# mountain/qingdai

Hardware: AMD Instinct MI355X
Metric: simulated planet-days/sec at 721x1440 f64 (higher is better)
Workload: dtype f64; 1 GPU; 721x1440 seed-42 planet, dt=300 s: forcing + time_step(Teq, dt, albedo) with QD_ENERGY_W=1 QD_CLOUD_COUPLE=1 + slab-ocean coupling + driver-side precipitation/cloud/albedo diagnostics (run_simulation.py:1766-1934,2063-2146) (BASELINE configs[2]; loop order of benchmark_jax.py:124-158); ocean_n_sub=13, parallelism=lat-bands x1

## Files before the change

qingdai_amd/csrc/qd_atmos.hip:

```cpp
#include "qd_internal.h"
#include "qd_pointwise.h"
#include "qd_device.h"
#include "qd_saf.h"

#include "qd_fluxes.h"
#include "qd_fused.h"

struct QdColPtrs {
    const double *u, *v, *Teq, *isr, *albedo, *csmap;
    double *h, *Ts, *q, *cloud, *hice;
    double *E, *Pcond, *LH, *LHrel, *olr, *cloud_eff;
    const uint8_t* land;
    const double* pref;
    unsigned long long* npos;
};

struct QdColIn { double cloud, isr, albedo, teq; };

template <int PHASE, bool HAS_ALB>
__device__ __forceinline__ void qd_column_cell(const QdColP& P, const QdColPtrs& A, size_t o, const QdColIn* IN, int i, int nlat) {
    const double u = A.u[o], v = A.v[o], h = A.h[o], Ts = A.Ts[o];
    const double hice = A.hice[o];
    const bool land = (A.land[o] == 1);
    const bool ocean = !land;
    const double T_a = 288.0 + P.ga * h;
    const double qsat_air = qd_qsat(T_a, P.p0);

    const QdHum Hm = qd_humidity_column(P, u, v, Ts, A.q[o], qsat_air, land, hice);
    const double q = Hm.q, E = Hm.E, Pc = Hm.Pc, LH = Hm.LH, LHrel = Hm.LHrel;
    if (PHASE == 1) { A.Pcond[o] = Pc; return; }
    A.q[o] = q; A.LH[o] = LH;
    if (PHASE != 2) A.Pcond[o] = Pc;
    if (P.write_diag) { A.E[o] = E; A.LHrel[o] = LHrel; }

    const double Teq = IN ? IN->teq : A.Teq[o];
    const double olr_old = P.sigma * qd_pow4(Ts);
    const double net_old = P.sigma * qd_pow4(Teq) + P.gfs * qd_pow4(T_a) - olr_old;
    const double Ts_newton = Ts + (net_old / P.c_sfc_safe) * P.dt;

    double Ts_new, h_new = h;
    QdFlux F;
    if (HAS_ALB) {
        const double cloud = IN ? IN->cloud : A.cloud[o];
        double cloud_eff;
        if (P.couple) {
            const double RH = qd_clip(q / qd_max(1e-12, qsat_air), 0.0, 1.5);
            const double rh_excess = qd_max(0.0, RH - P.rh0);
            const double P_ref = *A.pref;
            const double p_term = qd_tanh(P_ref > 0 ? Pc / P_ref : 0.0);
            cloud_eff = qd_clip(cloud + P.k_q * rh_excess + P.k_p * p_term, 0.0, 1.0);
        } else cloud_eff = cloud;
        A.cloud_eff[o] = cloud_eff;
        F = qd_surface_fluxes(P, IN ? IN->isr : A.isr[o], IN ? IN->albedo : A.albedo[o], cloud_eff, Ts, T_a, u, v, land, hice);
        double Ts_energy;
        if (P.seaice) {
            double Q = F.SW_sfc - F.LW_sfc - F.SH - LH;
            double Tn = Ts, hi = hice;
            if (hi > 0.0 && ocean && Q > 0.0) {
                const double dh_melt = (Q * P.dt) / P.rhoiLf;
                const double dh_cap = qd_min(dh_melt, hi);
                hi -= dh_cap;
                Q = Q - (dh_cap * P.rho_i * P.L_f) / P.dt;
            }
            if (ocean && Q < 0.0 && Tn <= (P.t_freeze + 0.5)) {
                hi += (-Q * P.dt) / P.rhoiLf;
                Q = 0.0;
                Tn = qd_min(Tn, P.t_freeze);
            }
            double Cs = land ? P.Cs_land : (hi > 0.0 ? P.Cs_ice : P.Cs_ocean);
            Cs = (isfinite(Cs) && Cs > 1e3) ? Cs : 1e3;
            Tn = Tn + (Q / Cs) * P.dt;
            if ((i == 0 && P.fix_s) || (i == nlat - 1 && P.fix_n)) {
                if (ocean && Q < 0.0 && Tn > P.t_freeze) Tn = P.t_freeze;
            }
            if (hi > 0.0 && ocean) Tn = qd_min(Tn, P.t_freeze);
            Tn = qd_max(P.t_floor, Tn);
            Ts_energy = qd_nn(Tn);
            { const double hn_ = qd_nn(hi); if (__double_as_longlong(hn_) != __double_as_longlong(hice)) A.hice[o] = hn_; }
        } else {
            const double net = F.SW_sfc - F.LW_sfc - F.SH - LH;
            double Cs;
            if (P.has_csmap) { const double cm = A.csmap[o]; Cs = (isfinite(cm) && cm > 1e3) ? cm : 1e3; }
            else Cs = P.c_sfc_safe;
            Ts_energy = qd_nn(qd_max(P.t_floor, Ts + (net / Cs) * P.dt));
        }
        if (P.write_diag) A.olr[o] = F.OLR;
        Ts_new = (1.0 - P.w_energy) * Ts_newton + P.w_energy * Ts_energy;
    } else {
        if (P.write_diag) A.olr[o] = olr_old;
        Ts_new = Ts_newton;
    }
    A.Ts[o] = Ts_new;

    const double h_eq = P.h_eq_fac * Teq;
    h_new = h + ((h_eq - h) / P.tau_rad) * P.dt;
    if (HAS_ALB && P.atm_couple) {
        const double F_atm = F.SW_atm + F.LW_atm + F.SH + LHrel;
        h_new = qd_nn(h_new + P.atm_w * (F_atm / P.atm_denom) * P.dt);
    }
    A.h[o] = h_new;
}

template <int PHASE, bool HAS_ALB>
__global__ void __launch_bounds__(QD_BLOCK)
k_column(QdGeom G, QdColP P, QdColPtrs A) {
    const QdTile tl = qd_tile();
    const int j = tl.seg * QD_BLOCK + threadIdx.x;
    if (j >= G.nlon) return;
    const int i = G.row0 + tl.row;
    qd_column_cell<PHASE, HAS_ALB>(P, A, (size_t)qd_lrow(G, i) * G.nlon + j, nullptr, i, G.nlat);
}

__global__ void __launch_bounds__(QD_BLOCK)
k_saf_column2(QdSafArgs K, QdColP P, QdColPtrs A) {
    const QdTile tl = qd_tile();
    const int j = tl.seg * QD_BLOCK + threadIdx.x;
    if (j >= K.G.nlon) return;
    const int i = K.G.row0 + tl.row;
    const size_t o = (size_t)qd_lrow(K.G, i) * K.G.nlon + j;
    const QdSafOut s = qd_saf_cell(K, i, j, o, K.write_diag != 0);
    const QdColIn in{s.cloud, s.isr, s.albedo, s.teq};
    qd_column_cell<2, true>(P, A, o, &in, i, K.G.nlat);
}

struct QdMomP { double g, a, dt, dlat, dlon, f_min; int primitive; };

__global__ void __launch_bounds__(QD_BLOCK)
k_momentum(QdGeom G, QdTabs T, QdMomP P, const double* __restrict__ h, const double* __restrict__ fric,
           double* __restrict__ u, double* __restrict__ v) {
    const QdTile tl = qd_tile();
    const int j = tl.seg * QD_BLOCK + threadIdx.x;
    if (j >= G.nlon) return;
    const int i = G.row0 + tl.row;
    const int n = G.nlat, m = G.nlon;
    const size_t b = (size_t)qd_lrow(G, i) * m;
    const size_t o = b + j;
    double dh_dlon;
    if (j == 0) dh_dlon = (h[b + 1] - h[b]) / P.dlon;
    else if (j == m - 1) dh_dlon = (h[b + m - 1] - h[b + m - 2]) / P.dlon;
    else dh_dlon = (h[b + j + 1] - h[b + j - 1]) / (2.0 * P.dlon);
    double dh_dlat;
    if (i == 0) dh_dlat = (h[(size_t)qd_lrow(G, 1) * m + j] - h[o]) / P.dlat;
    else if (i == n - 1) dh_dlat = (h[o] - h[(size_t)qd_lrow(G, n - 2) * m + j]) / P.dlat;
    else dh_dlat = (h[(size_t)qd_lrow(G, i + 1) * m + j] - h[(size_t)qd_lrow(G, i - 1) * m + j]) / (2.0 * P.dlat);
    const double cosc = T.cos6[i];
    const double f = T.fcor[i];
    const double r = fric[o];
    const double u0 = u[o], v0 = v[o];
    if (P.primitive) {
        const double PGF_x = -(P.g / (P.a * cosc)) * dh_dlon;
        const double PGF_y = -(P.g / P.a) * dh_dlat;
        const double du = (PGF_x + f * v0 - r * u0) * P.dt;
        const double dv = (PGF_y - f * u0 - r * v0) * P.dt;
        u[o] = qd_clip(u0 + du, -200.0, 200.0);
        v[o] = qd_clip(v0 + dv, -200.0, 200.0);
    } else {
        const double sgn = (f >= 0.0) ? 1.0 : -1.0;
        const double f_safe = (fabs(f) < P.f_min) ? sgn * P.f_min : f;
        const double u_g = qd_clip(-(P.g / (f_safe * P.a * cosc)) * dh_dlat, -200.0, 200.0);
        const double v_g = qd_clip((P.g / (f_safe * P.a)) * dh_dlon, -200.0, 200.0);
        double un = u0 * 0.8 + u_g * 0.2;
        double vn = v0 * 0.8 + v_g * 0.2;
        un = un + (-r * un) * P.dt;
        vn = vn + (-r * vn) * P.dt;
        u[o] = un; v[o] = vn;
    }
}

__global__ void __launch_bounds__(QD_BLOCK)
k_final(QdGeom G, const double* __restrict__ cosl, double dt, double a, double dlat, double dlon,
        double* __restrict__ u, double* __restrict__ v, double* __restrict__ h, double* __restrict__ Ts,
        double* __restrict__ q, const double* __restrict__ cloud_in, double* __restrict__ cloud_out,
        double decay, double dfac) {
    const QdTile tl = qd_tile();
    const int j = tl.seg * QD_BLOCK + threadIdx.x;
    if (j >= G.nlon) return;
    const int i = G.row0 + tl.row;
    const size_t o = (size_t)qd_lrow(G, i) * G.nlon + j;
    const double uu = u[o], vv = v[o];
    const QdBilin b = qd_departure(G, i, j, uu, vv, dt, a, cosl[i], dlat, dlon);
    double c = qd_gather(cloud_in, G, b);
    c = c * decay;
    cloud_out[o] = qd_nn(c * dfac);
    u[o] = qd_nn(uu * dfac);
    v[o] = qd_nn(vv * dfac);
    h[o] = qd_nn(h[o] * dfac);
    q[o] = qd_nn(q[o] * dfac);
    Ts[o] = qd_nn(Ts[o]);
}

__global__ void __launch_bounds__(QD_BLOCK)
k_forcing(QdGeom G, QdTabs T, QdForcingP P, double* __restrict__ isrA, double* __restrict__ isrB, double* __restrict__ isr,
          const double* __restrict__ albedo, double* __restrict__ Teq, double* __restrict__ eday, double eday_dt) {
    const QdTile tl = qd_tile();
    const int j = tl.seg * QD_BLOCK + threadIdx.x;
    if (j >= G.nlon) return;
    const int i = G.row0 + tl.row;
    const size_t o = (size_t)qd_lrow(G, i) * G.nlon + j;
    qd_forcing_cell(T, P, i, j, o, P.with_teq ? albedo[o] : 0.0, isrA, isrB, isr, Teq, eday, eday_dt);
}

int qd_forcing_impl(qd_ctx* c, const double* sa, const double* sb, double theta, int with_teq) {
    QdScope sc(c, "forcing");
    QdStar A{sa[0], std::sin(sa[1]), std::cos(sa[1]), sa[2]};
    QdStar B{sb[0], std::sin(sb[1]), std::cos(sb[1]), sb[2]};
    const int m = with_teq ? qd_plan(c, {QD_IN(c->f[QD_F_ALBEDO], 0)}) : c->geo.halo;
    if (m < 0) return -1;
    const QdForcingP FP{A, B, theta, 5.670374e-8, with_teq};
    QD_ROWS(c, m, G, hipLaunchKernelGGL(k_forcing, qd_grid2d(G), dim3(QD_BLOCK), 0, c->stream, G, c->tabs, FP,
                                        c->f[QD_F_ISR_A], c->f[QD_F_ISR_B], c->f[QD_F_ISR],
                                        c->f[QD_F_ALBEDO], c->f[QD_F_TEQ], c->eco.eday_dt > 0 ? c->f[QD_F_ECO_EDAY] : (double*)nullptr,
                                        c->eco.eday_dt));
    c->eco.eday_dt = 0;
    qd_mark(c, {c->f[QD_F_ISR_A], c->f[QD_F_ISR_B], c->f[QD_F_ISR]}, m);
    if (with_teq) qd_mark(c, {c->f[QD_F_TEQ]}, m);
    return 0;
}

__global__ void __launch_bounds__(QD_BLOCK)
k_simple_albedo(QdGeom G, const uint8_t* __restrict__ land, const double* __restrict__ base, double ocean_albedo,
                double* __restrict__ albedo) {
    const QdTile tl = qd_tile();
    const int j = tl.seg * QD_BLOCK + threadIdx.x;
    if (j >= G.nlon) return;
    const size_t o = (size_t)qd_lrow(G, G.row0 + tl.row) * G.nlon + j;
    albedo[o] = (land[o] == 0) ? ocean_albedo : base[o];
}

int qd_simple_albedo_impl(qd_ctx* c, double ocean_albedo) {
    const int m = c->geo.full ? 0 : c->geo.halo;
    QD_ROWS(c, m, G, hipLaunchKernelGGL(k_simple_albedo, qd_grid2d(G), dim3(QD_BLOCK), 0, c->stream, G, c->land,
                                        c->f[QD_F_BASE_ALBEDO], ocean_albedo, c->f[QD_F_ALBEDO]));
    qd_mark(c, {c->f[QD_F_ALBEDO]}, m);
    return 0;
}

static inline bool qd_isset(double x) { return !(x != x); }

QdColP qd_make_colp(const qd_ctx* c, double dt) {
    const qd_params& p = c->p;
    QdColP P;
    P.ga = p.g / 1004.0;
    P.M_col = std::max(1e-6, p.rho_a * p.h_mbl);
    P.tau_c = std::max(1e-6, p.tau_cond);
    P.L_v = p.L_v; P.p0 = p.p0; P.rhoCE = p.rho_a * p.C_E;
    P.s_ocean = p.ocean_evap_scale; P.s_land = p.land_evap_scale; P.s_ice = p.ice_evap_scale;
    P.sigma = 5.670374e-8;
    P.gfs = p.greenhouse_factor * P.sigma;
    P.c_sfc_safe = std::max(1e-12, p.c_sfc);
    P.dt = dt;
    P.rh0 = p.rh0; P.k_q = p.k_q; P.k_p = p.k_p;
    P.sw_a0 = p.sw_a0; P.sw_kc = p.sw_kc; P.lw_eps0 = p.lw_eps0; P.lw_kc = p.lw_kc;
    P.eps_clear = std::min(std::max(p.lw_eps0, 0.0), 1.0);
    P.tau0 = p.lw_tau0; P.k_tau = p.lw_ktau;
    P.hice_ref_safe = std::max(1e-6, p.hice_ref);
    P.eps_ocean = p.eps_ocean; P.eps_land = p.eps_land; P.eps_ice = p.eps_ice; P.eps_default = p.eps_default;
    P.g_lw = p.gh_factor_lw;
    P.rhocpch = p.rho_a * p.cp_a * p.ch;
    P.t_freeze = p.t_freeze; P.rho_i = p.rho_i; P.L_f = p.L_f; P.rhoiLf = p.rho_i * p.L_f;
    P.Cs_ocean = p.Cs_ocean; P.Cs_land = p.Cs_land; P.Cs_ice = p.Cs_ice; P.t_floor = p.t_floor;
    P.w_energy = std::min(1.0, std::max(0.0, p.energy_w));
    P.h_eq_fac = 287.0 / p.g;
    P.tau_rad = p.tau_rad;
    const double H_atm = qd_isset(p.atm_h) ? p.atm_h : p.h_mbl;
    P.atm_denom = std::max(1e-6, p.rho_a) * std::max(1.0, H_atm) * p.g;
    P.atm_w = p.energy_w;
    P.atm_couple = (p.energy_w > 0.0) ? 1 : 0;
    P.couple = p.cloud_couple; P.lw_v2 = p.lw_v2; P.gh_lock = p.gh_lock; P.seaice = p.seaice_enabled;
    P.fix_s = p.polar_freeze_fix_s; P.fix_n = p.polar_freeze_fix_n; P.has_csmap = p.has_csmap;
    P.write_diag = c->diag_write;
    return P;
}

__global__ void k_set_scalar(double* p, double v) { if (threadIdx.x == 0 && blockIdx.x == 0) *p = v; }
__global__ void k_zero_count(unsigned long long* p) { if (threadIdx.x == 0 && blockIdx.x == 0) *p = 0ull; }

static QdColPtrs qd_col_ptrs(qd_ctx* c) {
    double** F = c->f;
    QdColPtrs A;
    A.u = F[QD_F_U]; A.v = F[QD_F_V]; A.Teq = F[QD_F_TEQ]; A.isr = F[QD_F_ISR];
    A.albedo = F[QD_F_ALBEDO]; A.csmap = F[QD_F_CSMAP];
    A.h = F[QD_F_H]; A.Ts = F[QD_F_TS]; A.q = F[QD_F_Q]; A.cloud = F[QD_F_CLOUD]; A.hice = F[QD_F_HICE];
    A.E = F[QD_F_EFLUX]; A.Pcond = F[QD_F_PCOND]; A.LH = F[QD_F_LH]; A.LHrel = F[QD_F_LHREL];
    A.olr = F[QD_F_OLR]; A.cloud_eff = F[QD_F_CLOUD_EFF];
    A.land = c->land; A.pref = c->dscal + QD_S_PREF; A.npos = c->dcount;
    return A;
}

int qd_pcond_phase1(qd_ctx* c, double dt) {
    hipLaunchKernelGGL((k_column<1, true>), qd_grid2d(c->geo), dim3(QD_BLOCK), 0, c->stream, c->geo, qd_make_colp(c, dt), qd_col_ptrs(c));
    return 0;
}
int qd_pcond_median_side(qd_ctx* c, double dt) {
    QD_HIP(c, hipEventRecord(c->med_fork, c->stream));
    QD_HIP(c, hipStreamWaitEvent(c->side_stream, c->med_fork, 0));
    std::swap(c->stream, c->side_stream);
    c->med_side_active = true;
    const QdColP P = qd_make_colp(c, dt);
    const QdColPtrs A = qd_col_ptrs(c);
    hipLaunchKernelGGL((k_column<1, true>), qd_grid2d(c->geo), dim3(QD_BLOCK), 0, c->stream, c->geo, P, A);
    const int r = qd_median_positive_dev(c, c->f[QD_F_PCOND], 1e-6, QD_S_PREF, 0, 0.0, 1);
    c->med_side_active = false;
    std::swap(c->stream, c->side_stream);
    if (r) return -1;
    QD_HIP(c, hipEventRecord(c->med_done, c->side_stream));
    c->pcond_ahead = 2;
    return 0;
}

int qd_atmos_step_impl(qd_ctx* c, double dt, int has_albedo) {
    const qd_params& p = c->p;
    const QdGeom& G0 = c->geo;
    const dim3 blk(QD_BLOCK);
    double** F = c->f;
    QdColP P = qd_make_colp(c, dt);
    const int R = qd_adv_reach(c, dt, 250.0);

    if (c->saf_pending && !(has_albedo && p.cloud_couple && !qd_isset(p.pcond_ref) && c->pcond_ahead == 3) && qd_saf_flush(c)) return -1;
    {
        QdScope sc(c, "column");
        int m = has_albedo
            ? qd_plan(c, {QD_IN(F[QD_F_U], 0), QD_IN(F[QD_F_V], 0), QD_IN(F[QD_F_H], 0), QD_IN(F[QD_F_TS], 0), QD_IN(F[QD_F_Q], 0),
                          QD_IN(F[QD_F_CLOUD], 0), QD_IN(F[QD_F_HICE], 0), QD_IN(F[QD_F_TEQ], 0), QD_IN(F[QD_F_ISR], 0),
                          QD_IN(F[QD_F_ALBEDO], 0)})
            : qd_plan(c, {QD_IN(F[QD_F_U], 0), QD_IN(F[QD_F_V], 0), QD_IN(F[QD_F_H], 0), QD_IN(F[QD_F_TS], 0), QD_IN(F[QD_F_Q], 0),
                          QD_IN(F[QD_F_HICE], 0), QD_IN(F[QD_F_TEQ], 0)});
        if (m < 0) return -1;
        QdColPtrs A;
        A.u = F[QD_F_U]; A.v = F[QD_F_V]; A.Teq = F[QD_F_TEQ]; A.isr = F[QD_F_ISR];
        A.albedo = F[QD_F_ALBEDO]; A.csmap = F[QD_F_CSMAP];
        A.h = F[QD_F_H]; A.Ts = F[QD_F_TS]; A.q = F[QD_F_Q]; A.cloud = F[QD_F_CLOUD]; A.hice = F[QD_F_HICE];
        A.E = F[QD_F_EFLUX]; A.Pcond = F[QD_F_PCOND]; A.LH = F[QD_F_LH]; A.LHrel = F[QD_F_LHREL];
        A.olr = F[QD_F_OLR]; A.cloud_eff = F[QD_F_CLOUD_EFF];
        A.land = c->land; A.pref = c->dscal + QD_S_PREF; A.npos = c->dcount;
        if (!has_albedo) {
            QD_ROWS(c, m, G, hipLaunchKernelGGL((k_column<0, false>), qd_grid2d(G), blk, 0, c->stream, G, P, A));
        } else if (!p.cloud_couple || qd_isset(p.pcond_ref)) {
            hipLaunchKernelGGL(k_set_scalar, dim3(1), dim3(1), 0, c->stream, c->dscal + QD_S_PREF,
                               qd_isset(p.pcond_ref) ? p.pcond_ref : 1e-6);
            QD_ROWS(c, m, G, hipLaunchKernelGGL((k_column<0, true>), qd_grid2d(G), blk, 0, c->stream, G, P, A));
        } else {
            const int ahead = c->pcond_ahead;
            c->pcond_ahead = 0;
            if (!ahead) QD_ROWS(c, m, G, hipLaunchKernelGGL((k_column<1, true>), qd_grid2d(G), blk, 0, c->stream, G, P, A));
            if (ahead == 2) QD_HIP(c, hipStreamWaitEvent(c->stream, c->med_done, 0));
            else if (ahead != 3 && qd_median_positive_dev(c, F[QD_F_PCOND], 1e-6, QD_S_PREF, 0, 0.0, 1)) return -1;
            if (c->saf_pending && ahead == 3 && c->geo.full) {
                QdSafArgs* K = (QdSafArgs*)c->saf_pending;
                c->saf_pending = nullptr;
                hipLaunchKernelGGL(k_saf_column2, qd_grid2d(K->G), blk, 0, c->stream, *K, P, A);
                delete K;
            } else {
                if (qd_saf_flush(c)) return -1;
                QD_ROWS(c, m, G, hipLaunchKernelGGL((k_column<2, true>), qd_grid2d(G), blk, 0, c->stream, G, P, A));
            }
        }
        qd_mark(c, {F[QD_F_H], F[QD_F_TS], F[QD_F_Q], F[QD_F_EFLUX], F[QD_F_PCOND], F[QD_F_LH], F[QD_F_LHREL], F[QD_F_OLR]}, m);
        if (has_albedo) { qd_mark(c, {F[QD_F_HICE], F[QD_F_CLOUD_EFF]}, m); c->cloud_eff_valid = 1; }
    }
    c->atm_counter += 1;
    const int64_t sc_ = c->atm_counter;

    {
        QdScope sc(c, "advect_tsq");
        const int m = qd_plan(c, {QD_IN(F[QD_F_TS], R), QD_IN(F[QD_F_Q], R), QD_IN(F[QD_F_U], 0), QD_IN(F[QD_F_V], 0)});
        if (m < 0) return -1;
        double* oT = qd_scratch(c, 0); double* oq = qd_scratch(c, 1);
        qd_launch_advect(c, F[QD_F_U], F[QD_F_V], c->tabs.cos6, dt, F[QD_F_TS], oT, F[QD_F_Q], oq, 0.2, 1, m);
        qd_swap(c, QD_F_TS, 0); qd_swap(c, QD_F_Q, 1);
    }
    const int ft = p.filter_type;
    const bool do_diff = p.diff_enable && (ft == 0 || ft == 1) && (sc_ % std::max(1, p.diff_every) == 0);
    const double f_min = 2.0 * p.omega * std::sin(5.0 * (M_PI / 180.0));
    if (do_diff) { int rc = qd_build_k4_tables(c, dt, false, 0.0); if (rc) return rc; }
    const double ov[5] = {p.k4_u, p.k4_v, p.k4_h, p.k4_q, p.k4_cloud};
    if (do_diff && c->use_fused && p.k4_nsub == 1) {
        const int m = qd_plan(c, {QD_IN(F[QD_F_H], 5), QD_IN(F[QD_F_U], 4), QD_IN(F[QD_F_V], 4), QD_IN(F[QD_F_FRICTION], 4),
                                  QD_IN(F[QD_F_Q], 4), QD_IN(F[QD_F_CLOUD], 4)});
        if (m < 0) return -1;
        QdDynArgs D;
        D.u = F[QD_F_U]; D.v = F[QD_F_V]; D.h = F[QD_F_H]; D.fric = F[QD_F_FRICTION];
        D.q = F[QD_F_Q]; D.cloud = F[QD_F_CLOUD];
        D.uo = qd_scratch(c, 0); D.vo = qd_scratch(c, 1); D.ho = qd_scratch(c, 2); D.qo = qd_scratch(c, 3); D.co = qd_scratch(c, 4);
        for (int f = 0; f < 5; ++f) {
            const bool sc1 = qd_isset(ov[f]);
            D.k4row[f] = sc1 ? nullptr : c->k4_atm + (size_t)f * G0.nlat;
            D.k4s[f] = sc1 ? ov[f] : 0.0;
            D.skip[f] = c->k4_atm_skip[f];
        }
        D.g = p.g; D.a = p.a; D.dt = dt; D.dlat = c->dlat; D.dlon = c->dlon; D.f_min = f_min; D.primitive = p.mom_scheme == 1;
        D.inv_dlon = 1.0 / c->dlon; D.inv_2dlon = 1.0 / (2.0 * c->dlon); D.inv_dlat = 1.0 / c->dlat; D.inv_2dlat = 1.0 / (2.0 * c->dlat);
        D.pgf_y = -(p.g / p.a);
        if (qd_launch_dyn_hyper(c, D, m)) return -1;
        qd_mark(c, {D.uo, D.vo, D.ho, D.qo, D.co}, m);
        qd_swap(c, QD_F_U, 0); qd_swap(c, QD_F_V, 1); qd_swap(c, QD_F_H, 2); qd_swap(c, QD_F_Q, 3); qd_swap(c, QD_F_CLOUD, 4);
    } else {
        {
            QdScope sc(c, "momentum");
            const int m = qd_plan(c, {QD_IN(F[QD_F_H], 1), QD_IN(F[QD_F_U], 0), QD_IN(F[QD_F_V], 0), QD_IN(F[QD_F_FRICTION], 0)});
            if (m < 0) return -1;
            QdMomP M;
            M.g = p.g; M.a = p.a; M.dt = dt; M.dlat = c->dlat; M.dlon = c->dlon; M.f_min = f_min;
            M.primitive = p.mom_scheme == 1;
            QD_ROWS(c, m, G, hipLaunchKernelGGL(k_momentum, qd_grid2d(G), blk, 0, c->stream, G, c->tabs, M, F[QD_F_H],
                                                F[QD_F_FRICTION], F[QD_F_U], F[QD_F_V]));
            qd_mark(c, {F[QD_F_U], F[QD_F_V]}, m);
        }
        if (do_diff) {
            QdScope sc(c, "hyperdiffusion");
            const int ns = std::max(1, p.k4_nsub);
            const int m3 = qd_plan(c, {QD_IN(F[QD_F_U], 4 * ns), QD_IN(F[QD_F_V], 4 * ns), QD_IN(F[QD_F_H], 4 * ns)});
            const int m2 = qd_plan(c, {QD_IN(F[QD_F_Q], 4), QD_IN(F[QD_F_CLOUD], 4)});
            if (m3 < 0 || m2 < 0) return -1;
            double* fl[5] = {F[QD_F_U], F[QD_F_V], F[QD_F_H], F[QD_F_Q], F[QD_F_CLOUD]};
            int skip3[5] = {c->k4_atm_skip[0], c->k4_atm_skip[1], c->k4_atm_skip[2], 1, 1};
            int skip2[5] = {1, 1, 1, c->k4_atm_skip[3], c->k4_atm_skip[4]};
            qd_hyperdiffuse_fields(c, fl, 5, c->k4_atm, skip3, ov, dt, ns, c->tabs.cos02, m3);
            qd_hyperdiffuse_fields(c, fl, 5, c->k4_atm, skip2, ov, dt, 1, c->tabs.cos02, m2);
            F[QD_F_U] = fl[0]; F[QD_F_V] = fl[1]; F[QD_F_H] = fl[2]; F[QD_F_Q] = fl[3]; F[QD_F_CLOUD] = fl[4];
        }
    }
    if ((ft == 0 || ft == 1 || ft == 2) && p.shapiro_every > 0 && (sc_ % p.shapiro_every == 0)) {
        QdScope sc(c, "shapiro");
        const int np_ = std::max(1, p.shapiro_n);
        const int m = qd_plan(c, {QD_IN(F[QD_F_U], np_), QD_IN(F[QD_F_V], np_), QD_IN(F[QD_F_H], np_)});
        if (m < 0) return -1;
        double* fl[3] = {F[QD_F_U], F[QD_F_V], F[QD_F_H]};
        qd_shapiro_fields(c, fl, 3, np_, m);
        F[QD_F_U] = fl[0]; F[QD_F_V] = fl[1]; F[QD_F_H] = fl[2];
        const int n1 = std::max(1, p.shapiro_n - 1);
        if (p.diff_q) {
            const int mq = qd_plan(c, {QD_IN(F[QD_F_Q], n1)}); if (mq < 0) return -1;
            double* g1[1] = {F[QD_F_Q]}; qd_shapiro_fields(c, g1, 1, n1, mq); F[QD_F_Q] = g1[0];
        }
        if (p.diff_cloud) {
            const int mc = qd_plan(c, {QD_IN(F[QD_F_CLOUD], n1)}); if (mc < 0) return -1;
            double* g1[1] = {F[QD_F_CLOUD]}; qd_shapiro_fields(c, g1, 1, n1, mc); F[QD_F_CLOUD] = g1[0];
        }
    }
    if ((ft == 0 || ft == 3) && p.spec_every > 0 && (sc_ % p.spec_every == 0)) {
        QdScope sc(c, "zonal_filter");
        const int m = qd_plan(c, {QD_IN(F[QD_F_U], 0), QD_IN(F[QD_F_V], 0), QD_IN(F[QD_F_H], 0)});
        if (m < 0) return -1;
        double* fl[3] = {F[QD_F_U], F[QD_F_V], F[QD_F_H]};
        if (qd_zonal_filter_fields(c, fl, 3, p.spec_cutoff, p.spec_damp, m)) return -1;
    }
    {
        QdScope sc(c, "final");
        const int m = qd_plan(c, {QD_IN(F[QD_F_CLOUD], R), QD_IN(F[QD_F_U], 0), QD_IN(F[QD_F_V], 0), QD_IN(F[QD_F_H], 0),
                                  QD_IN(F[QD_F_TS], 0), QD_IN(F[QD_F_Q], 0)});
        if (m < 0) return -1;
        const double decay = 1 - dt / (2.0 * 24 * 3600);
        if (c->defer_final && c->geo.full) {
            c->final_pending.on = 1; c->final_pending.dt = dt; c->final_pending.decay = decay; c->final_pending.dfac = p.diff_factor;
            return 0;
        }
        double* oc = qd_scratch(c, 0);
        QD_ROWS(c, m, G, hipLaunchKernelGGL(k_final, qd_grid2d(G), blk, 0, c->stream, G, c->tabs.cos6, dt, p.a, c->dlat, c->dlon,
                                            F[QD_F_U], F[QD_F_V], F[QD_F_H], F[QD_F_TS], F[QD_F_Q], F[QD_F_CLOUD], oc, decay,
                                            p.diff_factor));
        qd_mark(c, {F[QD_F_U], F[QD_F_V], F[QD_F_H], F[QD_F_TS], F[QD_F_Q], oc}, m);
        qd_swap(c, QD_F_CLOUD, 0);
    }
    return 0;
}
```

qingdai_amd/csrc/qd_ocean.hip:

```cpp
#include <cstdlib>
#include <atomic>
#include <chrono>
#include "qd_internal.h"
#include "qd_device.h"
#include "qd_wave.h"

#include "qd_fluxes.h"
#include "qd_fused.h"
#include "qd_ocntail.h"
#include "qd_band.h"
#include "qd_blockred.h"

QdColP qd_make_colp(const qd_ctx* c, double dt);

__global__ void __launch_bounds__(QD_BLOCK)
k_qnet(QdGeom G, QdColP P, const double* __restrict__ isr, const double* __restrict__ albedo,
       const double* __restrict__ cloud, const double* __restrict__ Ts, const double* __restrict__ h,
       const double* __restrict__ u, const double* __restrict__ v, const uint8_t* __restrict__ land,
       const double* __restrict__ hice, const double* __restrict__ LH, double* __restrict__ qnet,
       uint8_t* __restrict__ icemask) {
    const QdTile tl = qd_tile();
    const int j = tl.seg * QD_BLOCK + threadIdx.x;
    if (j >= G.nlon) return;
    const size_t o = (size_t)qd_lrow(G, G.row0 + tl.row) * G.nlon + j;
// ... 225 lines not shown
    const double du = (f * v0 - P.g * gx + taux[o] / P.rhoH - P.r_bot * u0);
    const double dv = (-f * u0 - P.g * gy + tauy[o] / P.rhoH - P.r_bot * v0);
    double un = u0 + P.sub_dt * du;
    double vn = v0 + P.sub_dt * dv;
    if (land[o] == 1) { un = 0.0; vn = 0.0; }
    const double rx = T.r_extra[i];
    un = un - P.sub_dt * rx * un;
    vn = vn - P.sub_dt * rx * vn;
    uo[o] = un; vo[o] = vn;
}

__global__ void __launch_bounds__(QD_BLOCK)
k_continuity(QdGeom G, QdTabs T, double a, double dlat, double dlon, double msdtH, const double* __restrict__ uo,
             const double* __restrict__ vo, const uint8_t* __restrict__ land, double* __restrict__ eta,
             double* __restrict__ partial) {
    __shared__ double sm[QD_BLOCK / 64];
    const int i = G.row0 + blockIdx.y;
    const size_t b = (size_t)qd_lrow(G, i) * G.nlon;
    const double w = T.warea[i];
    double acc = 0.0;
    for (int j = threadIdx.x; j < G.nlon; j += QD_BLOCK) {
        const size_t o = b + j;
        const double div = qd_divvort_point(G, T, uo, vo, i, j, a, dlat, dlon, 0);
        double e = eta[o] + msdtH * div;
        const bool island = land[o] == 1;
        if (island) e = 0.0;
        eta[o] = e;
        acc += e * (island ? 0.0 : w);
    }
    acc = qd_wave_sum(acc);
    const int lane = threadIdx.x & 63, wv = threadIdx.x >> 6;
    if (lane == 0) sm[wv] = acc;
    __syncthreads();
    if (threadIdx.x == 0) {
        double r = sm[0];
        for (int k = 1; k < QD_BLOCK / 64; ++k) r += sm[k];
        partial[blockIdx.y] = r;
    }
}

__global__ void __launch_bounds__(QD_BLOCK)
k_eta_mean(const double* __restrict__ partial, int n, double wsum, double* __restrict__ out, double seq = 0.0) {
    __shared__ double sm[QD_BLOCK / 64];
    double acc = 0.0;
    for (int k = threadIdx.x; k < n; k += QD_BLOCK) acc += partial[k];
    acc = qd_wave_sum(acc);
    const int lane = threadIdx.x & 63, wv = threadIdx.x >> 6;
    if (lane == 0) sm[wv] = acc;
    __syncthreads();
    if (threadIdx.x == 0) {
        double r = sm[0];
        for (int k = 1; k < QD_BLOCK / 64; ++k) r += sm[k];
        *out = (wsum < 0.0) ? r : r / (wsum + 1e-15);
        if (seq != 0.0) __hip_atomic_store(&out[1], seq, __ATOMIC_RELEASE, __HIP_MEMORY_SCOPE_SYSTEM);
    }
}

__global__ void __launch_bounds__(QD_BLOCK)
k_cont_sstadv(QdGeom G, QdTabs T, double a, double dlat, double dlon, double msdtH, double sub_dt, double alpha,
              const double* __restrict__ uo, const double* __restrict__ vo, const uint8_t* __restrict__ land,
              double* __restrict__ eta, const double* __restrict__ Ts, double* __restrict__ Ts_out,
              int own0, int own1, double* __restrict__ partial, unsigned long long* ticket, double wsum,
              double* __restrict__ eta_mean) {
    __shared__ double sm[QD_BLOCK / 64];
    __shared__ int s_last;
    const int i = G.row0 + blockIdx.y;
    const size_t b = (size_t)qd_lrow(G, i) * G.nlon;
    const double w = (i >= own0 && i < own1) ? T.warea[i] : 0.0;
    const double cosl = T.cos05[i];
    const int pidx = blockIdx.y * gridDim.x + blockIdx.x, pcount = gridDim.x * gridDim.y;
    double acc = 0.0;
    for (int j = blockIdx.x * QD_BLOCK + threadIdx.x; j < G.nlon; j += gridDim.x * QD_BLOCK) {
        const size_t o = b + j;
        const double div = qd_divvort_point(G, T, uo, vo, i, j, a, dlat, dlon, 0);
        double e = eta[o] + msdtH * div;
        const bool island = land[o] == 1;
        if (island) e = 0.0;
        eta[o] = e;
        acc += e * (island ? 0.0 : w);
        const QdBilin bl = qd_departure(G, i, j, uo[o], vo[o], sub_dt, a, cosl, dlat, dlon);
        Ts_out[o] = (1.0 - alpha) * Ts[o] + alpha * qd_gather(Ts, G, bl);
    }
    acc = qd_wave_sum(acc);
    const int lane = threadIdx.x & 63, wv = threadIdx.x >> 6;
    if (lane == 0) sm[wv] = acc;
    __syncthreads();
    if (threadIdx.x == 0) {
        double r = sm[0];
        for (int k = 1; k < QD_BLOCK / 64; ++k) r += sm[k];
        if (!ticket) partial[pidx] = r;
        else {
            __hip_atomic_store(&partial[pidx], r, __ATOMIC_RELAXED, __HIP_MEMORY_SCOPE_AGENT);
            asm volatile("s_waitcnt vmcnt(0)" ::: "memory");
            const unsigned long long t = atomicAdd(ticket, 1ull);
            s_last = (t == (unsigned long long)pcount - 1ull) ? 1 : 0;
        }
    }
    if (!ticket) return;
    __syncthreads();
    if (!s_last) return;
    double a2 = 0.0;
    for (int k = threadIdx.x; k < pcount; k += QD_BLOCK)
        a2 += __hip_atomic_load(&partial[k], __ATOMIC_RELAXED, __HIP_MEMORY_SCOPE_AGENT);
    a2 = qd_wave_sum(a2);
    __syncthreads();
    if (lane == 0) sm[wv] = a2;
    __syncthreads();
    if (threadIdx.x == 0) {
        double r = sm[0];
        for (int k = 1; k < QD_BLOCK / 64; ++k) r += sm[k];
        *eta_mean = r / (wsum + 1e-15);
        __hip_atomic_store(ticket, 0ull, __ATOMIC_RELAXED, __HIP_MEMORY_SCOPE_AGENT);
    }
}

__global__ void __launch_bounds__(QD_BLOCK)
k_sst_advect(QdGeom G, const double* __restrict__ cos05, double sub_dt, double a, double dlat, double dlon,
             const double* __restrict__ uo, const double* __restrict__ vo, const double* __restrict__ Ts,
             double* __restrict__ Ts_out, double alpha, double* __restrict__ eta, const double* __restrict__ eta_mean,
             int has_ocean) {
    const QdTile tl = qd_tile();
    const int j = tl.seg * QD_BLOCK + threadIdx.x;
    if (j >= G.nlon) return;
    const int i = G.row0 + tl.row;
    const size_t o = (size_t)qd_lrow(G, i) * G.nlon + j;
    if (has_ocean) eta[o] = eta[o] - *eta_mean;
    const QdBilin b = qd_departure(G, i, j, uo[o], vo[o], sub_dt, a, cos05[i], dlat, dlon);
    const double adv = qd_gather(Ts, G, b);
    Ts_out[o] = (1.0 - alpha) * Ts[o] + alpha * adv;
}

struct QdHeatP { double sub_dt, K_h, rcH, ice_qfac; int use_q, has_ice; };

__global__ void __launch_bounds__(QD_BLOCK)
k_sst_diffuse_heat(QdGeom G, const double* __restrict__ cos05, double dlat, double dlon, double a, QdHeatP P,
                   const double* __restrict__ Ts1, double* __restrict__ Ts_out, const double* __restrict__ qnet,
                   const uint8_t* __restrict__ land, const uint8_t* __restrict__ ice) {
    const QdTile tl = qd_tile();
    const int j = tl.seg * QD_BLOCK + threadIdx.x;
    if (j >= G.nlon) return;
    const int i = G.row0 + tl.row;
    const size_t o = (size_t)qd_lrow(G, i) * G.nlon + j;
    double T = Ts1[o];
    if (P.K_h > 0.0) T = qd_nn(T) + P.sub_dt * P.K_h * qd_lap_point<true>(Ts1, G, cos05, i, j, dlat, dlon, a);
    if (P.use_q) {
        const double heat = qnet[o] / P.rcH;
        const bool ocean = land[o] == 0;
        if (P.has_ice) {
            const bool ic = ice[o] != 0;
            if (ocean && !ic) T = T + P.sub_dt * heat;
            if (P.ice_qfac > 0.0 && ocean && ic) T = T + P.sub_dt * P.ice_qfac * heat;
        } else if (ocean) T = T + P.sub_dt * heat;
    }
    Ts_out[o] = qd_nn(T);
}

__global__ void __launch_bounds__(QD_BLOCK)
k_outlier(QdGeom G, const double* __restrict__ uo, const double* __restrict__ vo, double* __restrict__ uo_out,
          double* __restrict__ vo_out, double* __restrict__ eta, double cap, double eta_cap, int mean4) {
    const QdTile tl = qd_tile();
    const int j = tl.seg * QD_BLOCK + threadIdx.x;
    if (j >= G.nlon) return;
    const int i = G.row0 + tl.row;
    const size_t b = (size_t)qd_lrow(G, i) * G.nlon;
    const size_t o = b + j;
    double u = qd_nn(uo[o]), v = qd_nn(vo[o]);
    const double speed = sqrt(u * u + v * v);
    if (mean4) {
        if (speed > cap) {
            const size_t bn = (size_t)qd_lrow(G, i + 1) * G.nlon, bs = (size_t)qd_lrow(G, i - 1) * G.nlon;
            const int je = qd_wrapc(j + 1, G.nlon), jw = qd_wrapc(j - 1, G.nlon);
            u = 0.25 * (qd_nn(uo[bn + j]) + qd_nn(uo[bs + j]) + qd_nn(uo[b + je]) + qd_nn(uo[b + jw]));
            v = 0.25 * (qd_nn(vo[bn + j]) + qd_nn(vo[bs + j]) + qd_nn(vo[b + je]) + qd_nn(vo[b + jw]));
        }
        const double sp2 = sqrt(u * u + v * v);
        const double sc2 = (sp2 > cap) ? cap / (sp2 + 1e-12) : 1.0;
        u = u * sc2; v = v * sc2;
    } else {
        const double sc = (speed > cap) ? cap / (speed + 1e-12) : 1.0;
        u = u * sc; v = v * sc;
    }
    uo_out[o] = u; vo_out[o] = v;
    eta[o] = qd_clip(qd_nn(eta[o]), -eta_cap, eta_cap);
}

__global__ void __launch_bounds__(QD_BLOCK)
k_sst_outlier_fused(QdGeom G, QdTabs T, double dlat, double dlon, double a, QdHeatP P,
                    const double* __restrict__ Ts1, double* __restrict__ Ts_out, const double* __restrict__ qnet,
                    const uint8_t* __restrict__ land, const uint8_t* __restrict__ ice,
                    const double* __restrict__ uo, const double* __restrict__ vo, double* __restrict__ uo_out,
                    double* __restrict__ vo_out, double* __restrict__ eta, double cap, double eta_cap, int mean4,
                    const double* __restrict__ eta_mean, const double* __restrict__ partial, int pcount, double wsum,
                    double* __restrict__ mean_out) {
    if (mean_out && blockIdx.x == 0 && blockIdx.y == 0) {
        __shared__ double smm[QD_BLOCK / 64];
        double acc = 0.0;
        for (int k = threadIdx.x; k < pcount; k += QD_BLOCK) acc += partial[k];
        acc = qd_wave_sum(acc);
        if ((threadIdx.x & 63) == 0) smm[threadIdx.x >> 6] = acc;
        __syncthreads();
        if (threadIdx.x == 0) {
            double r = smm[0];
            for (int k = 1; k < QD_BLOCK / 64; ++k) r += smm[k];
            *mean_out = r / (wsum + 1e-15);
        }
    }
    const QdTile tl = qd_tile();
    const int j = tl.seg * QD_BLOCK + threadIdx.x;
    if (j >= G.nlon) return;
    const int i = G.row0 + tl.row;
    const size_t b = (size_t)qd_lrow(G, i) * G.nlon;
    const size_t o = b + j;
    double Tv = Ts1[o];
    if (P.K_h > 0.0) Tv = qd_nn(Tv) + P.sub_dt * P.K_h * qd_lap_point_fast<true>(Ts1, G, T, 1, i, j, dlat, dlon, a);
    if (P.use_q) {
        const double heat = qnet[o] / P.rcH;
        const bool ocean = land[o] == 0;
        if (P.has_ice) {
            const bool ic = ice[o] != 0;
            if (ocean && !ic) Tv = Tv + P.sub_dt * heat;
            if (P.ice_qfac > 0.0 && ocean && ic) Tv = Tv + P.sub_dt * P.ice_qfac * heat;
        } else if (ocean) Tv = Tv + P.sub_dt * heat;
    }
    Ts_out[o] = qd_nn(Tv);
    double u = qd_nn(uo[o]), v = qd_nn(vo[o]);
    const double speed = sqrt(u * u + v * v);
    if (mean4) {
        if (speed > cap) {
            const size_t bn = (size_t)qd_lrow(G, i + 1) * G.nlon, bs = (size_t)qd_lrow(G, i - 1) * G.nlon;
            const int je = qd_wrapc(j + 1, G.nlon), jw = qd_wrapc(j - 1, G.nlon);
            u = 0.25 * (qd_nn(uo[bn + j]) + qd_nn(uo[bs + j]) + qd_nn(uo[b + je]) + qd_nn(uo[b + jw]));
            v = 0.25 * (qd_nn(vo[bn + j]) + qd_nn(vo[bs + j]) + qd_nn(vo[b + je]) + qd_nn(vo[b + jw]));
        }
        const double sp2 = sqrt(u * u + v * v);
        const double sc2 = (sp2 > cap) ? cap / (sp2 + 1e-12) : 1.0;
        u = u * sc2; v = v * sc2;
    } else {
        const double sc = (speed > cap) ? cap / (speed + 1e-12) : 1.0;
        u = u * sc; v = v * sc;
    }
    uo_out[o] = u; vo_out[o] = v;
    if (mean_out) return;
    const double e = eta_mean ? eta[o] - (pcount < 0 ? *eta_mean / (wsum + 1e-15) : *eta_mean) : eta[o];
    eta[o] = qd_clip(qd_nn(e), -eta_cap, eta_cap);
}


__device__ __forceinline__ double qd_block_sum_ocn(double x, double* sm) {
    x = qd_wave_sum(x);
    const int lane = threadIdx.x & 63, wv = threadIdx.x >> 6;
    __syncthreads();
    if (lane == 0) sm[wv] = x;
    __syncthreads();
    double r = sm[0];
    for (int k = 1; k < QD_BLOCK / 64; ++k) r += sm[k];
    return r;
}

__device__ __forceinline__ void qd_polar_fill_row(const QdGeom& G, const QdTabs& T, const uint8_t* __restrict__ land, double* __restrict__ Ts,
                                                  double* __restrict__ uo, double* __restrict__ vo, bool north, double* sm) {
    const int i = north ? G.nlat - 1 : 0;
    const size_t b = (size_t)qd_lrow(G, i) * G.nlon;
    double cnt = 0, sT = 0, s0 = 0, s1 = 0;
    for (int j = threadIdx.x; j < G.nlon; j += QD_BLOCK) {
        if (land[b + j] != 0) continue;
        cnt += 1.0;
        sT += Ts[b + j];
        const double sl = T.sin_lon[j], cl = T.cos_lon[j];
        const double u = uo[b + j], v = vo[b + j];
        const double nx = north ? -cl : cl, ny = north ? -sl : sl;
        s0 += (-sl) * u + nx * v;
        s1 += cl * u + ny * v;
    }
    cnt = qd_block_sum_ocn(cnt, sm);
    sT = qd_block_sum_ocn(sT, sm);
    s0 = qd_block_sum_ocn(s0, sm);
    s1 = qd_block_sum_ocn(s1, sm);
    if (cnt <= 0.0) return;
    const double mT = sT / cnt, m0 = s0 / cnt, m1 = s1 / cnt;
    for (int j = threadIdx.x; j < G.nlon; j += QD_BLOCK) {
        if (land[b + j] != 0) continue;
        const double sl = T.sin_lon[j], cl = T.cos_lon[j];
        const double nx = north ? -cl : cl, ny = north ? -sl : sl;
        Ts[b + j] = mT;
        uo[b + j] = (-sl) * m0 + cl * m1;
        vo[b + j] = nx * m0 + ny * m1;
    }
}

__global__ void __launch_bounds__(QD_BLOCK)
k_polar_fill(QdGeom G, QdTabs T, const uint8_t* __restrict__ land, double* __restrict__ Ts, double* __restrict__ uo,
             double* __restrict__ vo) {
    __shared__ double sm[QD_BLOCK / 64];
    const bool north = blockIdx.x == 1;
    const int i = north ? G.nlat - 1 : 0;
    if (i < G.row0 || i >= G.row0 + G.nrows) return;
    qd_polar_fill_row(G, T, land, Ts, uo, vo, north, sm);
}

__device__ __forceinline__ void qd_sst_clamp_cell(size_t o, double* __restrict__ sst, double tmin, double tmax, int inject,
                                                  const uint8_t* __restrict__ land, const uint8_t* __restrict__ ice, int has_ice,
                                                  double* __restrict__ Ts_atm, double* __restrict__ eta, const double* __restrict__ eta_mean,
                                                  double eta_cap) {
    if (eta) eta[o] = qd_clip(qd_nn(eta[o] - *eta_mean), -eta_cap, eta_cap);
    const double t0 = sst[o];
    const double t = qd_clip(t0, tmin, tmax);
    if (__double_as_longlong(t) != __double_as_longlong(t0)) sst[o] = t;
    if (inject && land[o] == 0 && !(has_ice && ice[o] != 0)) Ts_atm[o] = t;
}

__global__ void __launch_bounds__(QD_BLOCK)
k_sst_clamp_inject(QdGeom G, double* __restrict__ sst, double tmin, double tmax, int inject,
                   const uint8_t* __restrict__ land, const uint8_t* __restrict__ ice, int has_ice,
                   double* __restrict__ Ts_atm, double* __restrict__ eta, const double* __restrict__ eta_mean, double eta_cap) {
    const QdTile tl = qd_tile();
    const int j = tl.seg * QD_BLOCK + threadIdx.x;
    if (j >= G.nlon) return;
    const size_t o = (size_t)qd_lrow(G, G.row0 + tl.row) * G.nlon + j;
    qd_sst_clamp_cell(o, sst, tmin, tmax, inject, land, ice, has_ice, Ts_atm, eta, eta_mean, eta_cap);
}

#define QD_PF_CH 6
__global__ void __launch_bounds__(QD_BLOCK)
k_polar_clamp_inject(QdGeom G, QdTabs T, double* __restrict__ sst, double* __restrict__ uo, double* __restrict__ vo, double tmin, double tmax,
                     int inject, const uint8_t* __restrict__ land, const uint8_t* __restrict__ ice, int has_ice,
                     double* __restrict__ Ts_atm, double* __restrict__ eta, const double* __restrict__ eta_mean, double eta_cap) {
    __shared__ double sm[4][QD_BLOCK / 64];
    const QdTile tl = qd_tile();
    const int i = G.row0 + tl.row;
    if (i == 0 || i == G.nlat - 1) {
        if (tl.seg != 0) return;
        const bool north = i != 0;
        const size_t b = (size_t)qd_lrow(G, i) * G.nlon;
        if (G.nlon > QD_PF_CH * QD_BLOCK) {
            qd_polar_fill_row(G, T, land, sst, uo, vo, north, &sm[0][0]);
            __syncthreads();
            for (int j = threadIdx.x; j < G.nlon; j += QD_BLOCK)
                qd_sst_clamp_cell(b + j, sst, tmin, tmax, inject, land, ice, has_ice, Ts_atm, eta, eta_mean, eta_cap);
            return;
        }
        double t_[QD_PF_CH], u_[QD_PF_CH], v_[QD_PF_CH], sl_[QD_PF_CH], cl_[QD_PF_CH]; int ld_[QD_PF_CH];
#pragma unroll
        for (int k = 0; k < QD_PF_CH; ++k) {
            const int j = threadIdx.x + k * QD_BLOCK;
            const int jj = j < G.nlon ? j : G.nlon - 1;
            ld_[k] = j < G.nlon ? (int)land[b + jj] : 1;
            t_[k] = sst[b + jj]; u_[k] = uo[b + jj]; v_[k] = vo[b + jj]; sl_[k] = T.sin_lon[jj]; cl_[k] = T.cos_lon[jj];
        }
        double cnt = 0, sT = 0, s0 = 0, s1 = 0;
#pragma unroll
        for (int k = 0; k < QD_PF_CH; ++k) {
            if (ld_[k] != 0) continue;
            cnt += 1.0;
            sT += t_[k];
            const double nx = north ? -cl_[k] : cl_[k], ny = north ? -sl_[k] : sl_[k];
            s0 += (-sl_[k]) * u_[k] + nx * v_[k];
            s1 += cl_[k] * u_[k] + ny * v_[k];
        }
        cnt = qd_wave_sum(cnt); sT = qd_wave_sum(sT); s0 = qd_wave_sum(s0); s1 = qd_wave_sum(s1);
        const int lane = threadIdx.x & 63, wv = threadIdx.x >> 6;
        if (lane == 0) { sm[0][wv] = cnt; sm[1][wv] = sT; sm[2][wv] = s0; sm[3][wv] = s1; }
        __syncthreads();
        cnt = sm[0][0]; sT = sm[1][0]; s0 = sm[2][0]; s1 = sm[3][0];
        for (int k = 1; k < QD_BLOCK / 64; ++k) { cnt += sm[0][k]; sT += sm[1][k]; s0 += sm[2][k]; s1 += sm[3][k]; }
        const bool any = cnt > 0.0;
        const double mT = sT / cnt, m0 = s0 / cnt, m1 = s1 / cnt;
#pragma unroll
        for (int k = 0; k < QD_PF_CH; ++k) {
            const int j = threadIdx.x + k * QD_BLOCK;
            if (j >= G.nlon) continue;
            const size_t o = b + j;
            double tv = t_[k];
            if (any && ld_[k] == 0) {
                const double nx = north ? -cl_[k] : cl_[k], ny = north ? -sl_[k] : sl_[k];
                tv = mT;
                uo[o] = (-sl_[k]) * m0 + cl_[k] * m1;
                vo[o] = nx * m0 + ny * m1;
            }
            if (eta) eta[o] = qd_clip(qd_nn(eta[o] - *eta_mean), -eta_cap, eta_cap);
            const double t = qd_clip(tv, tmin, tmax);
            sst[o] = t;
            if (inject && ld_[k] == 0 && !(has_ice && ice[o] != 0)) Ts_atm[o] = t;
        }
        return;
    }
    const int j = tl.seg * QD_BLOCK + threadIdx.x;
    if (j >= G.nlon) return;
    qd_sst_clamp_cell((size_t)qd_lrow(G, i) * G.nlon + j, sst, tmin, tmax, inject, land, ice, has_ice, Ts_atm, eta, eta_mean, eta_cap);
}

__global__ void __launch_bounds__(256) k_eta_mean_tail(const double* __restrict__ partial, int n, double wsum, double* __restrict__ out) {
    __shared__ double sm[4];
    double a = 0.0;
    for (int k = threadIdx.x; k < n; k += 256) a += partial[k];
#pragma unroll
    for (int o = 32; o > 0; o >>= 1) a += __shfl_down(a, o, 64);
    if ((threadIdx.x & 63) == 0) sm[threadIdx.x >> 6] = a;
    __syncthreads();
    if (threadIdx.x == 0) *out = (((sm[0] + sm[1]) + sm[2]) + sm[3]) / (wsum + 1e-15);
}

__global__ void k_eta_mean_post(double* s, double wsum) { if (threadIdx.x == 0 && blockIdx.x == 0) *s = *s / (wsum + 1e-15); }

__global__ void k_host_flag(double* flag, double seq) {
    if (threadIdx.x == 0 && blockIdx.x == 0) __hip_atomic_store(flag, seq, __ATOMIC_RELEASE, __HIP_MEMORY_SCOPE_SYSTEM);
}
int qd_ocean_step_impl(qd_ctx* c, double dt, int compute_qnet, int use_ice_mask, int inject_sst) {
    const qd_params& p = c->p;
    const QdGeom& G0 = c->geo;
    const dim3 blk(QD_BLOCK);
    double** F = c->f;
    const bool band = !G0.full;
    c->ocn_counter += 1;
    const int64_t step = c->ocn_counter;
    const double H = p.H_ocean;
    const QdGeom Gown = qd_segments(c, 0).g[0];
    const dim3 rows(1, Gown.nrows);

    auto launch_qnet = [&]() -> int {
        QdScope sc(c, "ocean_qnet");
        QdColP P = qd_make_colp_driver(c, dt);
        double*& cl = c->cloud_eff_valid ? F[QD_F_CLOUD_EFF] : F[QD_F_CLOUD];
        const int m = qd_plan(c, {QD_IN(F[QD_F_ISR], 0), QD_IN(F[QD_F_ALBEDO], 0), QD_IN(cl, 0), QD_IN(F[QD_F_TS], 0),
                                  QD_IN(F[QD_F_H], 0), QD_IN(F[QD_F_U], 0), QD_IN(F[QD_F_V], 0), QD_IN(F[QD_F_HICE], 0),
                                  QD_IN(F[QD_F_LH], 0)});
        if (m < 0) return -1;
        QD_ROWS(c, m, G, hipLaunchKernelGGL(k_qnet, qd_grid2d(G), blk, 0, c->stream, G, P, F[QD_F_ISR], F[QD_F_ALBEDO], cl,
                                            F[QD_F_TS], F[QD_F_H], F[QD_F_U], F[QD_F_V], c->land, F[QD_F_HICE], F[QD_F_LH],
                                            F[QD_F_QNET], c->icemask));
        qd_mark(c, {F[QD_F_QNET], c->icemask}, m);
        use_ice_mask = 1;
        return 0;
    };
    if (compute_qnet && band && launch_qnet()) return -1;
    double*& taux = c->scratch[14];
    double*& tauy = c->scratch[15];
    int n_sub;
    bool band_fix_stats = false;
    {
        QdScope sc(c, "ocean_stress");
        const int m = qd_plan(c, {QD_IN(F[QD_F_U], 0), QD_IN(F[QD_F_V], 0), QD_IN(F[QD_F_UO], 0), QD_IN(F[QD_F_VO], 0)});
        if (m < 0) return -1;
        QdSegs S = qd_segments(c, m);
        double maxVa = 0.0, maxUo = 0.0;
        if (!band) {
            const QdGeom& G = S.g[0];
            c->eta_seq += 1.0;
            bool merged_final = false;
            if (c->final_pending.on) {
                if (!compute_qnet) return qd_fail(c, "ocean step: a deferred k_final needs compute_qnet");
                c->final_pending.on = 0;
                QdFqsArgs A;
                A.cosl = c->tabs.cos6; A.dt = c->final_pending.dt; A.a = p.a; A.dlat = c->dlat; A.dlon = c->dlon;
                A.decay = c->final_pending.decay; A.dfac = c->final_pending.dfac;
                A.u = F[QD_F_U]; A.v = F[QD_F_V]; A.h = F[QD_F_H]; A.Ts = F[QD_F_TS]; A.q = F[QD_F_Q];
                A.cloud_in = F[QD_F_CLOUD]; A.cloud_out = qd_scratch(c, 0);
                A.isr = F[QD_F_ISR]; A.albedo = F[QD_F_ALBEDO]; A.cloud_eff = c->cloud_eff_valid ? F[QD_F_CLOUD_EFF] : nullptr;
                A.hice = F[QD_F_HICE]; A.LH = F[QD_F_LH]; A.land = c->land; A.qnet = F[QD_F_QNET]; A.icemask = c->icemask;
                A.uo = F[QD_F_UO]; A.vo = F[QD_F_VO]; A.vcap = p.vcap; A.rhoCD = p.rho_a_ocean * p.CD; A.tau_scale = p.tau_scale;
                A.taux = taux; A.tauy = tauy;
                A.dev_wg = c->wgmax; A.n_wg = c->n_wgmax;
                merged_final = true;
                hipLaunchKernelGGL(k_final_qnet_stress, qd_grid2d(G), blk, 0, c->stream, G, qd_make_colp_driver(c, dt), A);
                hipLaunchKernelGGL(k_max2_publish, dim3(1), dim3(1024), 0, c->stream, c->wgmax, c->n_wgmax, c->hpin + 58, c->fix_count);
                qd_swap(c, QD_F_CLOUD, 0);
                use_ice_mask = 1;
            } else {
            hipLaunchKernelGGL(k_stress_max, dim3(1, G.nrows), blk, 0, c->stream, G, F[QD_F_U], F[QD_F_V], F[QD_F_UO],
                               F[QD_F_VO], p.vcap, p.rho_a_ocean * p.CD, p.tau_scale, taux, tauy, c->hpin_rows,
                               c->hpin_rows + (size_t)2 * G0.lrows(), c->eta_seq);
            qd_mark(c, {taux, tauy}, m);
            if (compute_qnet && launch_qnet()) return -1;
            }
            if (c->before_cfl_wait) {
                std::function<int()> fn = std::move(c->before_cfl_wait);
                c->before_cfl_wait = nullptr;
                if (c->side_stream_on && c->timing != 1 && !c->ocn_fused) {
                    QD_HIP(c, hipEventRecord(c->side_fork, c->stream));
                    QD_HIP(c, hipStreamWaitEvent(c->side_stream, c->side_fork, 0));
                    std::swap(c->stream, c->side_stream);
                    const int r = fn();
                    std::swap(c->stream, c->side_stream);
                    if (r) return -1;
                    QD_HIP(c, hipEventRecord(c->side_done, c->side_stream));
                    c->side_pending = true;
                } else if (fn()) return -1;
            }
            if (merged_final) {
                if (qd_wait_host_nonneg(c, c->hpin + 58, &maxVa, "ocean step: the CFL maxima never arrived") ||
                    qd_wait_host_nonneg(c, c->hpin + 59, &maxUo, "ocean step: the CFL maxima never arrived")) return -1;
                { const double avg = c->hpin[57]; c->hpin[57] = -1.0; if (avg >= 0.0) c->fix_avg = avg; }
            } else {
            for (int k = 0; k < G.nrows; ++k)
                if (qd_wait_host_flag(c, c->hpin_rows + (size_t)2 * G0.lrows() + k, c->eta_seq, "ocean step: the CFL maxima never arrived")) return -1;
            for (int k = 0; k < G.nrows; ++k) { maxVa = std::max(maxVa, c->hpin_rows[k]); maxUo = std::max(maxUo, c->hpin_rows[G.nrows + k]); }
            }
        } else {
        const bool hooked = qd_peer_hooks(c) && !qd_has_host_ring(c) && S.n <= 3;
        for (int k = 0; k < S.n; ++k) {
            const QdGeom& G = S.g[k];
            hipLaunchKernelGGL(k_stress_max, dim3(1, G.nrows), blk, 0, c->stream, G, F[QD_F_U], F[QD_F_V], F[QD_F_UO],
                               F[QD_F_VO], p.vcap, p.rho_a_ocean * p.CD, p.tau_scale, taux, tauy,
                               c->red_partial + (size_t)k * 2 * G0.lrows(), (double*)nullptr, 0.0);
            if (!hooked)
            hipLaunchKernelGGL(k_max2_finish, dim3(1), blk, 0, c->stream, c->red_partial + (size_t)k * 2 * G0.lrows(), G.nrows,
                               c->dscal + QD_S_TMP0 + 2 * k, k == S.n - 1 ? 2 * (3 - S.n) : 0);
        }
        qd_mark(c, {taux, tauy}, m);
        if (hooked) {
            QdPeerHook H; H.pre = 3; H.partial = c->red_partial; H.pstride = (size_t)2 * G0.lrows(); H.nseg = S.n;
            for (int k = 0; k < S.n; ++k) H.nsegrows[k] = S.g[k].nrows;
            c->allreduces++;
            c->pub_seq += 1.0;
            H.fixstat = (c->tail_fix && c->fix_count) ? c->fix_count : nullptr;
            if (qd_peer_allreduce_hooked(c, c->dscal + QD_S_TMP0, H.fixstat ? 7 : 6, 1, H, c->hpin, c->pub_seq)) return -1;
            if (qd_wait_host_flag(c, c->hpin + 61, c->pub_seq, "reduced scalars never reached the host")) return -1;
            if (c->hpin[60] != 0.0) return qd_fail(c, "peer exchange: a rank did not arrive within the deadline");
            if (H.fixstat && c->hpin[6] >= 0.0) c->fix_avg = c->hpin[6];
            band_fix_stats = H.fixstat != nullptr;
        } else if (qd_has_host_ring(c)) {
            QD_HIP(c, hipMemcpyAsync(c->hpin, c->dscal + QD_S_TMP0, 6 * sizeof(double), hipMemcpyDeviceToHost, c->stream));
            QD_HIP(c, hipStreamSynchronize(c->stream));
            if (qd_host_allreduce(c, c->hpin, 6, 1)) return -1;
        } else {
        if (qd_allreduce_fetch(c, c->dscal + QD_S_TMP0, 6, 1, c->hpin)) return -1;
        }
        for (int k = 0; k < 3; ++k) { maxVa = std::max(maxVa, c->hpin[2 * k]); maxUo = std::max(maxUo, c->hpin[2 * k + 1]); }
        }
        const double dx_lat = p.a * c->dlat;
        const double min_cos = 0.5;
        const double dx_lon_min = p.a * c->dlon * std::max(1e-3, min_cos);
        const double dx_min = std::min(dx_lat, dx_lon_min);
        const double cg = std::sqrt(p.g_ocean * H);
        double uadv = std::max(maxUo, maxVa);
        const double target = std::max(1e-3, p.ocean_cfl);
        const double v = std::ceil(std::max(cg, uadv) * (dt / std::max(1e-12, dx_min)) / target);
        n_sub = (v != v) ? 1 : (v > 500.0 ? 500 : (v < 1.0 ? 1 : (int)v));
        c->last_nsub = n_sub;
        c->form_note(QD_SF_LAST_NSUB, n_sub); c->form_note(QD_SF_LAST_TAIL_KERNEL, 0); c->form_note(QD_SF_LAST_OCN_FORM, 0);
    }
    bool fix_now = c->tail_fix && c->fix_count && (!band || band_fix_stats);
    if (fix_now) {
        if (c->fix_avg <= c->fix_dense) c->fix_probe_every = 32;
        else if (step >= c->fix_probe_at) {
            c->fix_probe_at = step + c->fix_probe_every;
            c->fix_probe_every = std::min(256, c->fix_probe_every * 2);
        } else fix_now = false;
    }
    const double sub_dt = dt / n_sub;
    QdOcnP OP{p.a, p.g_ocean, c->dlat, c->dlon, sub_dt, p.rho_w * H, p.r_bot};
    QdHeatP HP{sub_dt, p.K_h, p.rho_w * p.cp_w * H, p.ocean_ice_qfac, p.ocean_use_qnet ? 1 : 0, use_ice_mask ? 1 : 0};
    const bool do_diff = (p.ocean_diff_every > 0) && (step % p.ocean_diff_every == 0);
    const bool do_shap = (p.ocean_shapiro_n > 0) && (p.ocean_shapiro_every > 0) && (step % p.ocean_shapiro_every == 0);
    if (do_diff) { int rc = qd_build_k4_tables(c, dt, true, sub_dt); if (rc) return rc; }
    const double ov[3] = {p.ocean_k4_u, p.ocean_k4_v, p.ocean_k4_eta};
    const int Ro = qd_adv_reach(c, sub_dt, 4.0);

    const bool can_defer = do_diff && c->use_fused && p.ocean_k4_nsub == 1 && !do_shap && c->wsum_ocean > 0.0;
    const bool band_defer = band && can_defer && qd_has_host_ring(c);
    const bool band_tail = band && can_defer && !band_defer && c->ocn_tail == 1 && c->tail_acc && c->band_tail && G0.nlon >= 64 &&
                           G0.halo >= std::max(7, Ro + 2);
    const bool defer_eta = (!band && can_defer) || band_defer || band_tail;
    double* const mean_ptr = band_defer ? c->hpin + 42 : c->dscal + QD_S_ETA_MEAN;
    struct CoRefresh { qd_ctx* c; ~CoRefresh() { c->corefresh.clear(); } } corefresh_guard{c};
    if (band) c->corefresh = {QD_IN(F[QD_F_UO], 0), QD_IN(F[QD_F_VO], 0), QD_IN(F[QD_F_ETA], 0), QD_IN(F[QD_F_SST], 0), QD_IN(taux, 0),
                              QD_IN(tauy, 0), QD_IN(F[QD_F_QNET], 0), QD_IN8(c->icemask, 0)};
    const bool use_tail = c->use_fused && (!band || band_tail) && defer_eta && qd_ocn_tail_ok(G0) && c->ocn_tail;
    const bool tail_acc = use_tail && c->tail_acc;
    const bool use_fused1 = use_tail && !band && c->ocn_fused && c->ocn_tail == 1 && tail_acc && c->fused_fast == 1 && do_diff &&
                            p.ocean_k4_nsub == 1 && !do_shap && HP.use_q && HP.K_h > 0.0 && qd_ocn_fused_ok(c) &&
                            !c->k4_ocn_skip[0] && !c->k4_ocn_skip[1] && !c->k4_ocn_skip[2];
    const bool mean_form_ok = c->mean_in_momentum && !band && G0.full && tail_acc && !use_fused1 && do_diff && c->use_fused && n_sub > 1 &&
                              p.ocean_k4_nsub == 1 && !do_shap && qd_ocn_tail_is_fast(c) && qd_ocn_stream_ok(c, 0);
    if (mean_form_ok) fix_now = false;
    const bool mean_next_ok = mean_form_ok;
    c->form_note(QD_SF_LAST_USE_TAIL, use_tail); c->form_note(QD_SF_LAST_TAIL_ACC, tail_acc); c->form_note(QD_SF_LAST_USE_FUSED1, use_fused1);
    c->form_note(QD_SF_LAST_MEAN_FORM, mean_form_ok); c->form_note(QD_SF_LAST_FIX_NOW, fix_now);
    unsigned long long* acc_pending = nullptr;
    for (int s = 0; s < n_sub; ++s) {
        if (use_fused1) {
            QdOcnArgs O;
            O.uo = F[QD_F_UO]; O.vo = F[QD_F_VO]; O.eta = F[QD_F_ETA]; O.taux = taux; O.tauy = tauy; O.land = c->land;
            O.uo_out = qd_scratch(c, 0); O.vo_out = qd_scratch(c, 1); O.eta_out = qd_scratch(c, 6);
            for (int f = 0; f < 3; ++f) {
                const bool sc1 = !(ov[f] != ov[f]);
                O.k4row[f] = sc1 ? nullptr : c->k4_ocn + (size_t)f * G0.nlat;
                O.k4s[f] = sc1 ? ov[f] : 0.0;
                O.skip[f] = c->k4_ocn_skip[f];
            }
            O.a = p.a; O.g = p.g_ocean; O.dlat = c->dlat; O.dlon = c->dlon; O.sub_dt = sub_dt; O.rhoH = p.rho_w * H; O.r_bot = p.r_bot;
            O.inv_2dlon = 1.0 / (2.0 * c->dlon); O.inv_2dlat = 1.0 / (2.0 * c->dlat); O.inv_a = 1.0 / p.a; O.inv_rhoH = 1.0 / (p.rho_w * H);
            O.eta_mean = s > 0 ? mean_ptr : nullptr;
            O.eta_cap = p.eta_cap;
            QdTailArgs A;
            A.uo = O.uo_out; A.vo = O.vo_out; A.eta_in = O.eta_out; A.Ts = F[QD_F_SST]; A.qnet = F[QD_F_QNET]; A.land = c->land; A.ice = c->icemask;
            A.eta = qd_scratch(c, 2); A.Ts_out = qd_scratch(c, 3); A.uo_out = qd_scratch(c, 12); A.vo_out = qd_scratch(c, 13); A.partial = c->red_partial;
            A.a = p.a; A.dlat = c->dlat; A.dlon = c->dlon; A.sub_dt = sub_dt; A.msdtH = -sub_dt * H; A.alpha = p.ocean_adv_alpha;
            A.K_h = HP.K_h; A.rcH = HP.rcH; A.ice_qfac = HP.ice_qfac; A.cap = p.ocean_max_u;
            A.use_q = HP.use_q; A.has_ice = HP.has_ice; A.mean4 = p.ocean_outlier == 0 ? 1 : 0;
            A.r_a = 1.0 / p.a; A.r_dlon = 1.0 / c->dlon; A.r_dlat = 1.0 / c->dlat; A.r_2dlon = 1.0 / (2 * c->dlon); A.r_2dlat = 1.0 / (2 * c->dlat);
            A.r_rcH = 1.0 / HP.rcH;
            A.acc = c->eta_acc; A.mean_out = c->dscal + QD_S_ETA_MEAN; A.wsum = c->wsum_ocean;
            if (qd_launch_ocn_fused(c, O, A)) return -1;
            qd_swap(c, QD_F_UO, 12); qd_swap(c, QD_F_VO, 13); qd_swap(c, QD_F_ETA, 2); qd_swap(c, QD_F_SST, 3);
            continue;
        }
        if (do_diff && c->use_fused && p.ocean_k4_nsub == 1) {
            const QdUse narrow[5] = {QD_IN(F[QD_F_ETA], 5), QD_IN(F[QD_F_UO], 4), QD_IN(F[QD_F_VO], 4), QD_IN(taux, 4), QD_IN(tauy, 4)};
            bool pending = false;
            int m_old = 0;
            if (band_tail) {
                const QdUse wide[8] = {QD_IN(F[QD_F_ETA], 7), QD_IN(F[QD_F_UO], 6), QD_IN(F[QD_F_VO], 6), QD_IN(taux, 6), QD_IN(tauy, 6),
                                       QD_IN(F[QD_F_SST], Ro + 2), QD_IN(F[QD_F_QNET], 0), QD_IN8(c->icemask, 0)};
                if (qd_plan_begin(c, wide, 8, &pending) < 0) return -1;
                if (pending) m_old = qd_plan_peek(c, narrow, 5);
            }
            QdOcnArgs O;
            O.uo = F[QD_F_UO]; O.vo = F[QD_F_VO]; O.eta = F[QD_F_ETA]; O.taux = taux; O.tauy = tauy; O.land = c->land;
            O.uo_out = qd_scratch(c, 0); O.vo_out = qd_scratch(c, 1); O.eta_out = qd_scratch(c, 2);
            for (int f = 0; f < 3; ++f) {
                const bool sc1 = !(ov[f] != ov[f]);
                O.k4row[f] = sc1 ? nullptr : c->k4_ocn + (size_t)f * G0.nlat;
                O.k4s[f] = sc1 ? ov[f] : 0.0;
                O.skip[f] = c->k4_ocn_skip[f];
            }
            O.a = p.a; O.g = p.g_ocean; O.dlat = c->dlat; O.dlon = c->dlon; O.sub_dt = sub_dt; O.rhoH = p.rho_w * H; O.r_bot = p.r_bot;
            O.inv_2dlon = 1.0 / (2.0 * c->dlon); O.inv_2dlat = 1.0 / (2.0 * c->dlat); O.inv_a = 1.0 / p.a; O.inv_rhoH = 1.0 / (p.rho_w * H);
            O.eta_mean = (defer_eta && s > 0) ? mean_ptr : nullptr;
            O.eta_cap = p.eta_cap;
            if (acc_pending) { O.acc_read = acc_pending; O.acc_partial = c->red_partial; O.acc_n = qd_ocn_tail_tiles(c, Gown); O.acc_wsum = c->wsum_ocean; }
            int m_int = 0;
            bool split = false;
            if (pending) {
                m_int = m_old >= 0 ? m_old : -12;
                const QdSegList Si = qd_segments_rows(c, c->own_row0 - m_int, c->own_nrows + 2 * m_int);
                if (c->own_nrows + 2 * m_int >= 12 && qd_ocn_stream_ok_list(c, Si)) {
                    if (qd_launch_ocn_stream_list(c, O, Si)) return -1;
                    split = true;
                    c->form_count(QD_SF_CNT_SPLIT);
                }
                if (qd_plan_end(c)) return -1;
            }
            const int m = qd_plan(c, narrow, 5);
            if (m < 0) return -1;
            if (qd_allreduce_flush(c)) return -1;
            if (split && m > m_int) {
                QdSegList Sb = qd_segments_rows(c, c->own_row0 - m, m - m_int);
                Sb = qd_segments_rows(c, c->own_row0 + c->own_nrows + m_int, m - m_int, Sb);
                if (!qd_ocn_stream_ok_list(c, Sb)) {
                    c->form_count(QD_SF_CNT_SPLIT_REDO);
                    if (qd_launch_ocn_hyper(c, O, m)) return -1;
                } else if (qd_launch_ocn_stream_list(c, O, Sb)) return -1;
            } else if (!split) {
                if (qd_launch_ocn_hyper(c, O, m)) return -1;
            }
            qd_mark(c, {O.uo_out, O.vo_out, O.eta_out}, m);
            qd_swap(c, QD_F_UO, 0); qd_swap(c, QD_F_VO, 1); qd_swap(c, QD_F_ETA, 2);
        } else {
            {
                QdScope sc(c, "ocean_momentum");
                const int m = qd_plan(c, {QD_IN(F[QD_F_ETA], 1), QD_IN(F[QD_F_UO], 0), QD_IN(F[QD_F_VO], 0), QD_IN(taux, 0),
                                          QD_IN(tauy, 0)});
                if (m < 0) return -1;
                QD_ROWS(c, m, G, hipLaunchKernelGGL(k_ocean_momentum, qd_grid2d(G), blk, 0, c->stream, G, c->tabs, OP,
                                                    F[QD_F_ETA], taux, tauy, c->land, F[QD_F_UO], F[QD_F_VO]));
                qd_mark(c, {F[QD_F_UO], F[QD_F_VO]}, m);
            }
            if (do_diff) {
                QdScope sc(c, "ocean_hyperdiffusion");
                const int ns = std::max(1, p.ocean_k4_nsub);
                const int m = qd_plan(c, {QD_IN(F[QD_F_UO], 4 * ns), QD_IN(F[QD_F_VO], 4 * ns), QD_IN(F[QD_F_ETA], 4 * ns)});
                if (m < 0) return -1;
                double* fl[3] = {F[QD_F_UO], F[QD_F_VO], F[QD_F_ETA]};
                c->lap_tag = "ocean_k_laplacian"; c->hyp_tag = "ocean_k_hyper_apply";
                qd_hyperdiffuse_fields(c, fl, 3, c->k4_ocn, c->k4_ocn_skip, ov, sub_dt, ns, c->tabs.cos05, m);
                c->lap_tag = "k_laplacian"; c->hyp_tag = "k_hyper_apply";
                F[QD_F_UO] = fl[0]; F[QD_F_VO] = fl[1]; F[QD_F_ETA] = fl[2];
            }
        }
        if (do_shap) {
            const int np_ = p.ocean_shapiro_n;
            const int m = qd_plan(c, {QD_IN(F[QD_F_UO], np_), QD_IN(F[QD_F_VO], np_), QD_IN(F[QD_F_ETA], np_)});
            if (m < 0) return -1;
            double* fl[3] = {F[QD_F_UO], F[QD_F_VO], F[QD_F_ETA]};
            qd_shapiro_fields(c, fl, 3, np_, m);
// ... 201 lines not shown
```

qingdai_amd/csrc/qd_physics.hip:

```cpp
#include "qd_internal.h"
#include "qd_band.h"
#include "qd_pointwise.h"
#include "qd_device.h"
#include "qd_saf.h"
#include "qd_fluxes.h"
#include "qd_blockred.h"
QdColP qd_make_colp(const qd_ctx* c, double dt);


template <bool SLAB>
__global__ void __launch_bounds__(QD_BLOCK)
k_precip_raw(QdGeom G, QdTabs T, const double* __restrict__ u, const double* __restrict__ v,
             const double* __restrict__ pcond, double a, double dlat, double dlon, double D_crit, double beta,
             const double* __restrict__ scale_p, const unsigned long long* __restrict__ sel_state,
             double* __restrict__ praw, double* __restrict__ pos_out, double* __restrict__ partial,
             const double* __restrict__ orog) {
    __shared__ double sm[2][QD_BLOCK / 64];
    const int i = G.row0 + blockIdx.y;
    const size_t b = (size_t)qd_lrow(G, i) * G.nlon;
    const double w = T.warea[i];
    const bool anypos = sel_state[0] > 0;
    const double scale = qd_max(*scale_p, 1e-12);
    double s_num = 0.0, s_den = 0.0;
    for (int j = threadIdx.x; j < G.nlon; j += QD_BLOCK) {
        const double div = SLAB ? u[b + j] : qd_divvort_point(G, T, u, v, i, j, a, dlat, dlon, 0);
        const double pos = qd_max(0.0, -(div - D_crit));
        const double F_div = anypos ? qd_clip(pos / scale, 0.0, 5.0) : 0.0;
        const double Pq = qd_max(0.0, pcond[b + j]);
        const double F_orog = orog ? qd_clip(orog[b + j], 1.0, 3.0) : 1.0;
        const double F = (1.0 + beta * F_div) * F_orog;
        const double pr = Pq * F;
        praw[b + j] = pr;
        if (!SLAB) pos_out[b + j] = pos;
        s_num += Pq * w;
        s_den += pr * w;
    }
    s_num = qd_wave_sum(s_num); s_den = qd_wave_sum(s_den);
    const int lane = threadIdx.x & 63, wv = threadIdx.x >> 6;
    if (lane == 0) { sm[0][wv] = s_num; sm[1][wv] = s_den; }
    __syncthreads();
    if (threadIdx.x == 0) {
        for (int k = 1; k < QD_BLOCK / 64; ++k) { s_num += sm[0][k]; s_den += sm[1][k]; }
        partial[blockIdx.y] = s_num;
        partial[gridDim.y + blockIdx.y] = s_den;
    }
}

__global__ void __launch_bounds__(QD_BLOCK)
k_orog_factor(QdGeom G, QdTabs T, const double* __restrict__ elev, const double* __restrict__ u, const double* __restrict__ v,
              double a, double dlat, double dlon, double k_orog, double cap, double* __restrict__ out) {
    const QdTile tl = qd_tile();
    const int j = tl.seg * QD_BLOCK + threadIdx.x;
    if (j >= G.nlon) return;
    const int i = G.row0 + tl.row, n = G.nlat;
    const size_t b = (size_t)qd_lrow(G, i) * G.nlon;
    const int jp = qd_wrapc(j + 1, G.nlon), jm = qd_wrapc(j - 1, G.nlon);
    const double dx = a * T.cos6[i] * dlon, dy = a * dlat;
    const double dHdx = (elev[b + jp] - elev[b + jm]) / (2.0 * dx);
    double dHdy = 0.0;
    if (i != 0 && i != n - 1)
        dHdy = (elev[(size_t)qd_lrow(G, i + 1) * G.nlon + j] - elev[(size_t)qd_lrow(G, i - 1) * G.nlon + j]) / (2.0 * dy);
    const double gn = sqrt(dHdx * dHdx + dHdy * dHdy);
    const double nxh = gn > 1e-12 ? dHdx / (gn + 1e-12) : 0.0;
    const double nyh = gn > 1e-12 ? dHdy / (gn + 1e-12) : 0.0;
    out[b + j] = qd_clip(1.0 + k_orog * qd_max(0.0, u[b + j] * nxh + v[b + j] * nyh), 1.0, cap);
}

__global__ void __launch_bounds__(QD_BLOCK)
k_precip_scalars(const double* __restrict__ partial, int n, double wsum, double pq_min, double p_blend, int use_fb,
                 double* __restrict__ out) {
    qd_precip_scalars_wg(partial, n, wsum, pq_min, p_blend, use_fb, out);
}

__global__ void __launch_bounds__(QD_BLOCK)
k_scale_field(QdGeom G, const double* __restrict__ in, const double* __restrict__ s, double k, double* __restrict__ out) {
    const QdTile tl = qd_tile();
    const int j = tl.seg * QD_BLOCK + threadIdx.x;
    if (j >= G.nlon) return;
    const size_t o = (size_t)qd_lrow(G, G.row0 + tl.row) * G.nlon + j;
    out[o] = s ? in[o] * (*s) : k * in[o];
}

__global__ void __launch_bounds__(QD_BLOCK)
k_precip_blend(QdGeom G, const double* __restrict__ P, const double* __restrict__ Pdyn, const double* __restrict__ sc,
               double* __restrict__ out) {
    const QdTile tl = qd_tile();
    const int j = tl.seg * QD_BLOCK + threadIdx.x;
    if (j >= G.nlon) return;
    const size_t o = (size_t)qd_lrow(G, G.row0 + tl.row) * G.nlon + j;
    const double al = sc[1];
    double p = P[o];
    if (al != 0.0) p = (1.0 - al) * p + al * Pdyn[o];
    out[o] = qd_max(p, 0.0);
}

__global__ void __launch_bounds__(QD_BLOCK)
k_cloud_from_p(QdGeom G, const double* __restrict__ precip, const double* __restrict__ pref, double cmax,
               double* __restrict__ out) {
    const QdTile tl = qd_tile();
    const int j = tl.seg * QD_BLOCK + threadIdx.x;
    if (j >= G.nlon) return;
    const size_t o = (size_t)qd_lrow(G, G.row0 + tl.row) * G.nlon + j;
    out[o] = cmax * qd_tanh(precip[o] / (*pref + 1e-12));
}


__device__ __forceinline__ double qd_tanh01(double x) {
    double t = 0.0;
    if (!(x <= 0.0)) t = qd_tanh_nonneg(x);
    return qd_clip(t, 0.0, 1.0);
}

__device__ __forceinline__ double qd_cloud_source_cell(const QdGeom& G, const QdTabs& T, const double* __restrict__ u, const double* __restrict__ v,
                                                       const double* __restrict__ Ts, double a, double dlat, double dlon, int i, int j);

__global__ void __launch_bounds__(QD_BLOCK)
k_cloud_source(QdGeom G, QdTabs T, const double* __restrict__ u, const double* __restrict__ v,
               const double* __restrict__ Ts, double a, double dlat, double dlon, double* __restrict__ out) {
    const QdTile tl = qd_tile();
    const int j = tl.seg * QD_BLOCK + threadIdx.x;
    if (j >= G.nlon) return;
    const int i = G.row0 + tl.row;
    out[(size_t)qd_lrow(G, i) * G.nlon + j] = qd_cloud_source_cell(G, T, u, v, Ts, a, dlat, dlon, i, j);
}

__global__ void __launch_bounds__(QD_BLOCK)
k_cloud_fromp_source(QdGeom G, QdTabs T, const double* __restrict__ precip, const double* __restrict__ pref, double cmax,
                     const double* __restrict__ u, const double* __restrict__ v, const double* __restrict__ Ts, double a, double dlat,
                     double dlon, double* __restrict__ cfp, double* __restrict__ src) {
    const QdTile tl = qd_tile();
    const int j = tl.seg * QD_BLOCK + threadIdx.x;
    if (j >= G.nlon) return;
    const int i = G.row0 + tl.row;
    const size_t o = (size_t)qd_lrow(G, i) * G.nlon + j;
    cfp[o] = cmax * qd_tanh(precip[o] / (*pref + 1e-12));
    src[o] = qd_cloud_source_cell(G, T, u, v, Ts, a, dlat, dlon, i, j);
}

__device__ __forceinline__ double qd_cloud_source_cell(const QdGeom& G, const QdTabs& T, const double* __restrict__ u, const double* __restrict__ v,
                                                       const double* __restrict__ Ts, double a, double dlat, double dlon, int i, int j) {
    const size_t b = (size_t)qd_lrow(G, i) * G.nlon;
    const size_t o = b + j;
    const double T0 = Ts[o];
    double src = 0.0;
    src = src + 0.5 * qd_tanh01((T0 - 285.0) / 12.0);
    const double vort = qd_divvort_point(G, T, v, u, i, j, a, dlat, dlon, 1);
    const double rel = vort / (T.fcor[i] + 1e-12);
    src = src + 0.4 * qd_tanh01((rel - 0.5) / 2.0);
    const double dx = dlon * a * T.cos6[i];
    const double dy = dlat * a;
    const int jp = qd_wrapc(j + 1, G.nlon), jm = qd_wrapc(j - 1, G.nlon);
    const double gx = (Ts[b + jp] - Ts[b + jm]) / (2 * dx);
    const double gy = (Ts[(size_t)qd_lrow(G, i + 1) * G.nlon + j] - Ts[(size_t)qd_lrow(G, i - 1) * G.nlon + j]) / (2 * dy);
    const double tadv = -(u[o] * gx + v[o] * gy);
    src = src + 0.3 * qd_tanh01(fabs(tadv) / 2e-5);
    return src;
}

struct QdBlendP { double w_mem, w_p, w_src, tend, c_floor; };

__global__ void __launch_bounds__(QD_BLOCK)
k_cloud_blend(QdGeom G, QdBlendP P, const double* __restrict__ cfp, const double* __restrict__ src,
              double* __restrict__ cloud) {
    const QdTile tl = qd_tile();
    const int j = tl.seg * QD_BLOCK + threadIdx.x;
    if (j >= G.nlon) return;
    const size_t o = (size_t)qd_lrow(G, G.row0 + tl.row) * G.nlon + j;
    const double c0 = cloud[o], cp = cfp[o];
    const double tendency = src[o] * P.tend;
    double c = (P.w_mem * c0 + P.w_p * cp + P.w_src * qd_clip(c0 + tendency, 0.0, 1.0));
    if (P.c_floor > 0.0) c = qd_max(c, qd_clip(P.c_floor * cp, 0.0, 1.0));
    cloud[o] = qd_clip(c, 0.0, 1.0);
}

__global__ void __launch_bounds__(QD_BLOCK)
k_cloud_albedo(QdGeom G, QdAlbP P, const double* __restrict__ adv, double* __restrict__ cloud,
               const double* __restrict__ cloud_eff, const double* __restrict__ hice,
               const double* __restrict__ base, const uint8_t* __restrict__ land, const double* __restrict__ csnow,
               const double* __restrict__ eco_alpha, const double* __restrict__ glacier, const double* __restrict__ banded,
               const double* __restrict__ water, double* __restrict__ albedo) {
    const QdTile tl = qd_tile();
    const int j = tl.seg * QD_BLOCK + threadIdx.x;
    if (j >= G.nlon) return;
    const size_t o = (size_t)qd_lrow(G, G.row0 + tl.row) * G.nlon + j;
    double c = cloud[o];
    if (P.do_adv) { c = qd_clip((1.0 - P.alpha) * c + P.alpha * adv[o], 0.0, 1.0); cloud[o] = c; }
    const int landv = land[o];
    const double cs = (P.snow && landv == 1) ? csnow[o] : 0.0;
    const double gl = (P.eco && landv == 1) ? glacier[o] : 0.0;
    albedo[o] = qd_albedo_cell(P, o, c, cloud_eff, hice, base, landv, cs, gl, eco_alpha, banded, water);
}

__global__ void k_precip_scalars_post(const double* raw, double wsum, double pq_min, double p_blend, int use_fb, double* out) {
    if (threadIdx.x == 0 && blockIdx.x == 0) {
        const double a = raw[0], b = raw[1];
        const double den = b + 1e-20;
        out[0] = den > 0 ? a / den : 1.0;
        const double pq_mean = a / (wsum + 1e-15);
        out[1] = (use_fb && pq_mean < pq_min) ? p_blend : 0.0;
    }
}
__global__ void __launch_bounds__(QD_BLOCK)
k_precip_rawsums(const double* __restrict__ partial, int n, double* __restrict__ out) {
    __shared__ double sm[2][QD_BLOCK / 64];
    double a = 0.0, b = 0.0;
    for (int k = threadIdx.x; k < n; k += QD_BLOCK) { a += partial[k]; b += partial[n + k]; }
    a = qd_wave_sum(a); b = qd_wave_sum(b);
    const int lane = threadIdx.x & 63, wv = threadIdx.x >> 6;
    if (lane == 0) { sm[0][wv] = a; sm[1][wv] = b; }
    __syncthreads();
    if (threadIdx.x == 0) {
        for (int k = 1; k < QD_BLOCK / 64; ++k) { a += sm[0][k]; b += sm[1][k]; }
        out[0] = a; out[1] = b;
    }
}

__global__ void __launch_bounds__(QD_BLOCK)
k_snow_provisional(QdGeom G, QdTabs T, QdSnowP P, const double* __restrict__ precip, const double* __restrict__ h,
                   const double* __restrict__ S_snow, const double* __restrict__ elev, const uint8_t* __restrict__ land,
                   double* __restrict__ P_rain, double* __restrict__ S_next, double* __restrict__ melt,
                   double* __restrict__ C_snow, double* __restrict__ glacier) {
    const QdTile tl = qd_tile();
    const int j = tl.seg * QD_BLOCK + threadIdx.x;
    if (j >= G.nlon) return;
    const int i = G.row0 + tl.row;
    const size_t o = (size_t)qd_lrow(G, i) * G.nlon + j;
    const QdSnowOut r = qd_snow_cell(T, P, i, land[o] == 1, h[o], S_snow[o], elev[o], precip[o]);
    P_rain[o] = r.Pr; S_next[o] = r.Sn; melt[o] = r.melt; C_snow[o] = r.Cs; glacier[o] = r.gl;
}

__global__ void __launch_bounds__(QD_BLOCK)
k_snow_albedo_forcing(QdSafArgs K) {
    const QdTile tl = qd_tile();
    const int j = tl.seg * QD_BLOCK + threadIdx.x;
    if (j >= K.G.nlon) return;
    const int i = K.G.row0 + tl.row;
    qd_saf_cell(K, i, j, (size_t)qd_lrow(K.G, i) * K.G.nlon + j, true);
}
int qd_saf_launch(qd_ctx* c, const QdSafArgs& K) {
    hipLaunchKernelGGL(k_snow_albedo_forcing, qd_grid2d(K.G), dim3(QD_BLOCK), 0, c->stream, K);
    return 0;
}
void qd_saf_drop(qd_ctx* c) { delete (QdSafArgs*)c->saf_pending; c->saf_pending = nullptr; }
int qd_saf_flush(qd_ctx* c) {
    if (!c->saf_pending) return 0;
    QdSafArgs* K = (QdSafArgs*)c->saf_pending;
    c->saf_pending = nullptr;
    const int r = qd_saf_launch(c, *K);
    delete K;
    return r;
}

struct QdBucketP { double dt, tau_s, cap; };

__global__ void __launch_bounds__(QD_BLOCK)
k_hydro_commit(QdGeom G, QdBucketP P, const double* __restrict__ P_rain, const double* __restrict__ melt,
               const double* __restrict__ glacier, const double* __restrict__ E, const uint8_t* __restrict__ land,
               const double* __restrict__ S_next, double* __restrict__ S_snow, double* __restrict__ W_land,
               double* __restrict__ runoff) {
    const QdTile tl = qd_tile();
    const int j = tl.seg * QD_BLOCK + threadIdx.x;
    if (j >= G.nlon) return;
    const size_t o = (size_t)qd_lrow(G, G.row0 + tl.row) * G.nlon + j;
    const double L = land[o] == 1 ? 1.0 : 0.0;
    const double gl = glacier[o];
    const double non_gl = (L != 0.0 && gl == 0.0) ? 1.0 : 0.0;
    const double ml = melt[o];
    const double P_in = (P_rain[o] * L + ml) * non_gl;
    const double E_l = (E[o] * L) * non_gl;
    const double W = W_land[o];
    const double R_base = W / P.tau_s;
    double Wn = qd_max(0.0, W + (P_in - E_l - R_base) * P.dt);
    double R_fast = 0.0;
    if (P.cap > 0.0) {
        const double over = qd_max(0.0, Wn - P.cap);
        Wn = Wn - over;
        R_fast = (P.dt > 0) ? over / P.dt : 0.0;
    }
    W_land[o] = qd_nn(Wn);
    runoff[o] = qd_nn(R_base + R_fast) + ml * gl;
    S_snow[o] = S_next[o];
}

int qd_hydrology_commit_impl(qd_ctx* c, double dt) {
    const qd_params& p = c->p;
    double** F = c->f;
    QdScope sc(c, "hydrology");
    const int m = qd_plan(c, {QD_IN(F[QD_F_P_RAIN], 0), QD_IN(F[QD_F_MELT], 0), QD_IN(F[QD_F_GLACIER], 0), QD_IN(F[QD_F_EFLUX], 0),
                              QD_IN(F[QD_F_S_SNOW_NEXT], 0), QD_IN(F[QD_F_W_LAND], 0)});
    if (m < 0) return -1;
    QdBucketP B{dt, std::max(1.0, p.runoff_tau_days * 86400.0), (p.wland_cap_mm == p.wland_cap_mm && p.wland_cap_mm > 0) ? p.wland_cap_mm : -1.0};
    QD_ROWS(c, m, G, hipLaunchKernelGGL(k_hydro_commit, qd_grid2d(G), dim3(QD_BLOCK), 0, c->stream, G, B, F[QD_F_P_RAIN], F[QD_F_MELT],
                                        F[QD_F_GLACIER], F[QD_F_EFLUX], c->land, F[QD_F_S_SNOW_NEXT], F[QD_F_S_SNOW], F[QD_F_W_LAND],
                                        F[QD_F_RUNOFF]));
    qd_mark(c, {F[QD_F_S_SNOW], F[QD_F_W_LAND], F[QD_F_RUNOFF]}, m);
    return 0;
}

int qd_driver_physics_impl(qd_ctx* c, double dt, const QdForcingCall* fc, int part) {
    const qd_params& p = c->p;
    const QdGeom& G0 = c->geo;
    const dim3 blk(QD_BLOCK);
    double** F = c->f;
    const bool band = !G0.full;
    const QdGeom Gown = qd_segments(c, 0).g[0];
    auto isset = [](double x) { return !(x != x); };
    double*& praw = c->scratch[4];
    double*& pos = c->scratch[5];
    double*& tmp = c->scratch[6];
    double*& pdyn = c->scratch[7];
    const int R1 = qd_gauss_radius(1.0);
    const int Rc = qd_adv_reach(c, dt, 250.0);
    double* const rp = (c->side_stream_on && c->red_partial_b) ? c->red_partial_b : c->red_partial;
    if (part == 2 && qd_side_join(c)) return -1;
    const bool pcond_side = part != 1 && c->want_pcond_ahead && c->med_side && c->side_stream && c->geo.full && p.cloud_couple && !isset(p.pcond_ref) &&
                            c->timing != 1;
    if (pcond_side && qd_pcond_median_side(c, dt)) return -1;
    const bool pcond_pair = part != 1 && !pcond_side && c->want_pcond_ahead && c->med_pair && c->hist_b && c->geo.full && p.cloud_couple &&
                            !isset(p.pcond_ref) && !(isset(p.pref) && p.pref != 0.0);
    if (part != 2) {
        QdScope sc(c, "phys_precip");
        int m = qd_plan(c, {QD_IN(F[QD_F_U], 1), QD_IN(F[QD_F_V], 1), QD_IN(F[QD_F_PCOND], 0)});
        if (m < 0) return -1;
        qd_launch_divvort(c, F[QD_F_U], F[QD_F_V], tmp, 0, m);
        if (qd_median_positive_dev(c, tmp, 1e-12, QD_S_PSCALE, 1, p.D_crit, 2)) return -1;
        const double* orog = nullptr;
        if (p.orog_enable && c->has_elevation) {
            double*& of = c->scratch[8];
            const int mo = qd_plan(c, {QD_IN(F[QD_F_U], 0), QD_IN(F[QD_F_V], 0), QD_IN(F[QD_F_ELEVATION], 1)});
            if (mo < 0) return -1;
            QD_ROWS(c, mo, G, hipLaunchKernelGGL(k_orog_factor, qd_grid2d(G), blk, 0, c->stream, G, c->tabs, F[QD_F_ELEVATION],
                                                 F[QD_F_U], F[QD_F_V], p.a, c->dlat, c->dlon, p.orog_k, 2.0, of));
            qd_mark(c, {of}, mo);
            const int mb = qd_plan(c, {QD_IN(of, R1)});
            if (mb < 0) return -1;
            if (qd_gaussian_swap(c, of, tmp, 1.0, 0, mb)) return -1;
            orog = of;
            m = qd_plan(c, {QD_IN(F[QD_F_U], 1), QD_IN(F[QD_F_V], 1), QD_IN(F[QD_F_PCOND], 0), QD_IN(c->scratch[8], 0)});
            if (m < 0) return -1;
        }
        if (band && m > 0) {
            QdSegs S = qd_segments(c, m);
            const int own0 = c->own_row0, own1 = c->own_row0 + c->own_nrows;
            for (int k = 0; k < S.n; ++k) {
                const QdGeom& G = S.g[k];
                auto run = [&](int r0, int r1) {
                    if (r1 <= r0) return;
                    QdGeom g2 = G; g2.row0 = r0; g2.nrows = r1 - r0;
                    hipLaunchKernelGGL(k_precip_raw<false>, dim3(1, g2.nrows), blk, 0, c->stream, g2, c->tabs, F[QD_F_U], F[QD_F_V],
                                       F[QD_F_PCOND], p.a, c->dlat, c->dlon, p.D_crit, p.p_betadiv, c->dscal + QD_S_PSCALE,
                                       c->dcount, praw, pos, rp + (size_t)2 * G0.lrows(), orog);
                };
                const int a0 = G.row0, a1 = G.row0 + G.nrows;
                if (a1 <= own0 || a0 >= own1) run(a0, a1);
                else { run(a0, std::max(a0, own0)); run(std::min(a1, own1), a1); }
            }
        }
        const bool fold = !band && !orog && qd_gauss_pair_ok(c, 1.0);
        if (fold)
            hipLaunchKernelGGL(k_precip_raw<true>, dim3(1, Gown.nrows), blk, 0, c->stream, Gown, c->tabs, tmp, (const double*)nullptr,
                               F[QD_F_PCOND], p.a, c->dlat, c->dlon, p.D_crit, p.p_betadiv, c->dscal + QD_S_PSCALE, c->dcount, praw,
                               (double*)nullptr, rp, orog);
        else
        hipLaunchKernelGGL(k_precip_raw<false>, dim3(1, Gown.nrows), blk, 0, c->stream, Gown, c->tabs, F[QD_F_U], F[QD_F_V],
                           F[QD_F_PCOND], p.a, c->dlat, c->dlon, p.D_crit, p.p_betadiv, c->dscal + QD_S_PSCALE, c->dcount, praw,
                           pos, rp, orog);
        if (fold) qd_mark(c, {praw}, m); else qd_mark(c, {praw, pos}, m);
        if (band && qd_peer_hooks(c)) {
            QdPeerHook H; H.pre = 2; H.partial = rp; H.n = Gown.nrows;
            H.post = 1; H.wsum = c->wsum_all; H.pq_min = p.pq_min; H.p_blend = p.p_blend; H.use_fb = p.p_hybrid_fallback; H.out = c->dscal + QD_S_RENORM;
            c->allreduces++;
            if (qd_peer_allreduce_hooked(c, c->dscal + QD_S_TMP0, 2, 0, H)) return -1;
        } else if (band) {
            hipLaunchKernelGGL(k_precip_rawsums, dim3(1), blk, 0, c->stream, rp, Gown.nrows, c->dscal + QD_S_TMP0);
            if (qd_allreduce_f64(c, c->dscal + QD_S_TMP0, 2, 0)) return -1;
            hipLaunchKernelGGL(k_precip_scalars_post, dim3(1), dim3(64), 0, c->stream, c->dscal + QD_S_TMP0, c->wsum_all, p.pq_min,
                               p.p_blend, p.p_hybrid_fallback, c->dscal + QD_S_RENORM);
        } else if (!fold) {
            hipLaunchKernelGGL(k_precip_scalars, dim3(1), blk, 0, c->stream, rp, Gown.nrows, c->wsum_all, p.pq_min,
                               p.p_blend, p.p_hybrid_fallback, c->dscal + QD_S_RENORM);
        }
        if (fold) {
            const int mg = qd_plan(c, {QD_IN(praw, R1), QD_IN(tmp, R1)});
            if (mg < 0) return -1;
            const QdPrecipFold PF{rp, Gown.nrows, c->wsum_all, p.pq_min, p.p_blend, p.p_hybrid_fallback, p.D_crit, c->dscal + QD_S_RENORM};
            if (qd_gaussian_pair(c, praw, tmp, 1.0, 0, nullptr, 1.0, p.k_precip, nullptr, 1, nullptr, nullptr, nullptr,
                                 F[QD_F_PRECIP], mg, &PF)) return -1;
            qd_mark(c, {F[QD_F_PRECIP]}, mg);
        } else if (qd_gauss_pair_ok(c, 1.0)) {
            const int mg = qd_plan(c, {QD_IN(praw, R1), QD_IN(pos, R1)});
            if (mg < 0) return -1;
            if (qd_gaussian_pair(c, praw, pos, 1.0, 0, c->dscal + QD_S_RENORM, 1.0, p.k_precip, c->dscal + QD_S_RENORM, 1, nullptr,
                                 nullptr, nullptr, F[QD_F_PRECIP], mg)) return -1;
            qd_mark(c, {F[QD_F_PRECIP]}, mg);
        } else if (qd_gauss_can_fuse(c, 1.0)) {
            const int mg = qd_plan(c, {QD_IN(praw, R1), QD_IN(pos, R1)});
            if (mg < 0) return -1;
            if (qd_gaussian_swap(c, praw, tmp, 1.0, 0, mg, 0, c->dscal + QD_S_RENORM)) return -1;
            if (qd_gaussian(c, pos, pdyn, nullptr, 1.0, 0, mg, 0, nullptr, p.k_precip)) return -1;
            QD_ROWS(c, mg, G, hipLaunchKernelGGL(k_precip_blend, qd_grid2d(G), blk, 0, c->stream, G, praw, pdyn,
                                                 c->dscal + QD_S_RENORM, F[QD_F_PRECIP]));
            qd_mark(c, {F[QD_F_PRECIP]}, mg);
        } else {
        QD_ROWS(c, m, G, hipLaunchKernelGGL(k_scale_field, qd_grid2d(G), blk, 0, c->stream, G, praw, c->dscal + QD_S_RENORM, 0.0, praw));
        QD_ROWS(c, m, G, hipLaunchKernelGGL(k_scale_field, qd_grid2d(G), blk, 0, c->stream, G, pos, (const double*)nullptr,
                                            p.k_precip, pdyn));
        qd_mark(c, {pdyn}, m);
        const int mg = qd_plan(c, {QD_IN(praw, R1), QD_IN(pdyn, R1)});
        if (mg < 0) return -1;
        if (qd_gaussian_swap(c, praw, tmp, 1.0, 0, mg)) return -1;
        if (qd_gaussian_swap(c, pdyn, tmp, 1.0, 0, mg)) return -1;
        QD_ROWS(c, mg, G, hipLaunchKernelGGL(k_precip_blend, qd_grid2d(G), blk, 0, c->stream, G, praw, pdyn,
                                             c->dscal + QD_S_RENORM, F[QD_F_PRECIP]));
        qd_mark(c, {F[QD_F_PRECIP]}, mg);
        }
    }
    if (part == 1) return 0;
    {
        QdScope sc(c, "phys_cloud");
        if (isset(p.pref) && p.pref != 0.0) {
            hipMemcpyAsync(c->dscal + QD_S_MED_OUT, &p.pref, sizeof(double), hipMemcpyHostToDevice, c->stream);
        } else if (pcond_pair) {
            if (c->med_fold && qd_median_pair_ready(c, 3, 1)) {
                if (qd_median_pair_pcond_dev(c, F[QD_F_PRECIP], 1e-6, QD_S_MED_OUT, 0, 0.0, 3, qd_make_colp(c, dt), 1e-6, QD_S_PREF, 1)) return -1;
            } else {
                if (qd_pcond_phase1(c, dt)) return -1;
                if (qd_median_pair_dev(c, F[QD_F_PRECIP], 1e-6, QD_S_MED_OUT, 0, 0.0, 3, F[QD_F_PCOND], 1e-6, QD_S_PREF, 0, 0.0, 1)) return -1;
            }
            c->pcond_ahead = 3;
        } else {
            if (qd_median_positive_dev(c, F[QD_F_PRECIP], 1e-6, QD_S_MED_OUT, 0, 0.0, 3)) return -1;
        }
        double*& cfp = F[QD_F_CLOUD_FROM_P];
        double*& src = F[QD_F_CLOUD_SRC];
        int m = qd_plan(c, {QD_IN(F[QD_F_PRECIP], 0)});
        if (m < 0) return -1;
        int ms = qd_plan(c, {QD_IN(F[QD_F_U], 1), QD_IN(F[QD_F_V], 1), QD_IN(F[QD_F_TS], 1)});
        if (ms < 0) return -1;
        if (c->merge_pointwise) {
            m = ms = std::min(m, ms);
            QD_ROWS(c, m, G, hipLaunchKernelGGL(k_cloud_fromp_source, qd_grid2d(G), blk, 0, c->stream, G, c->tabs, F[QD_F_PRECIP],
                                                c->dscal + QD_S_MED_OUT, p.cmax, F[QD_F_U], F[QD_F_V], F[QD_F_TS], p.a, c->dlat, c->dlon, cfp, src));
        } else {
        QD_ROWS(c, m, G, hipLaunchKernelGGL(k_cloud_from_p, qd_grid2d(G), blk, 0, c->stream, G, F[QD_F_PRECIP],
                                            c->dscal + QD_S_MED_OUT, p.cmax, cfp));
        QD_ROWS(c, ms, G, hipLaunchKernelGGL(k_cloud_source, qd_grid2d(G), blk, 0, c->stream, G, c->tabs, F[QD_F_U], F[QD_F_V],
                                             F[QD_F_TS], p.a, c->dlat, c->dlon, src));
        }
        qd_mark(c, {cfp}, m);
        qd_mark(c, {src}, ms);
        const int mg = qd_plan(c, {QD_IN(cfp, R1), QD_IN(src, R1), QD_IN(F[QD_F_CLOUD], 0)});
        if (mg < 0) return -1;
        double wm = p.w_mem, wp = p.w_p, ws = p.w_src, wsum = wm + wp + ws;
        if (wsum <= 0) { wm = 0.5; wp = 0.4; ws = 0.1; wsum = 1.0; }
        wm /= wsum; wp /= wsum; ws /= wsum;
        QdBlendP B{wm, wp, ws, dt / (6 * 3600), p.cloud_from_p_floor};
        if (qd_gauss_pair_ok(c, 1.0)) {
            double*& oa = c->scratch[6]; double*& ob = c->scratch[7];
            const double b5[5] = {B.w_mem, B.w_p, B.w_src, B.tend, B.c_floor};
            if (qd_gaussian_pair(c, cfp, src, 1.0, 0, nullptr, 1.0, 1.0, nullptr, 2, b5, oa, ob, F[QD_F_CLOUD], mg)) return -1;
            std::swap(cfp, oa); std::swap(src, ob);
            qd_mark(c, {cfp, src, F[QD_F_CLOUD]}, mg);
        } else {
        if (qd_gaussian_swap(c, cfp, tmp, 1.0, 0, mg, 1)) return -1;
        if (qd_gaussian_swap(c, src, tmp, 1.0, 0, mg, 1)) return -1;
        QD_ROWS(c, mg, G, hipLaunchKernelGGL(k_cloud_blend, qd_grid2d(G), blk, 0, c->stream, G, B, cfp, src, F[QD_F_CLOUD]));
        qd_mark(c, {F[QD_F_CLOUD]}, mg);
        }
    }
    {
        QdScope sc(c, "phys_albedo");
        double*& adv = c->scratch[7];
        int m;
        if (p.cloud_advect) {
            const int ma = qd_plan(c, {QD_IN(F[QD_F_CLOUD], Rc), QD_IN(F[QD_F_U], 0), QD_IN(F[QD_F_V], 0)});
            if (ma < 0) return -1;
            qd_launch_advect(c, F[QD_F_U], F[QD_F_V], c->tabs.cos05, dt, F[QD_F_CLOUD], adv, nullptr, nullptr, 1.0, 0, ma);
            if (p.cloud_smooth_sigma > 0.0) {
                const int rs = qd_gauss_radius(p.cloud_smooth_sigma);
                const int mb = qd_plan(c, {QD_IN(adv, rs)});
                if (mb < 0) return -1;
                if (qd_gaussian_swap(c, adv, tmp, p.cloud_smooth_sigma, 1, mb)) return -1;
            }
            m = qd_plan(c, {QD_IN(adv, 0), QD_IN(F[QD_F_CLOUD], 0), QD_IN(F[QD_F_HICE], 0)});
        } else {
            m = qd_plan(c, {QD_IN(F[QD_F_CLOUD], 0), QD_IN(F[QD_F_HICE], 0)});
        }
        if (m < 0) return -1;
        if (c->cloud_eff_valid) { const int me = qd_plan(c, {QD_IN(F[QD_F_CLOUD_EFF], 0)}); if (me < 0) return -1; m = std::min(m, me); }
        const QdEco& E = c->eco;
        QdAlbP A{p.cloud_adv_alpha, std::max(1e-6, p.hice_ref), p.alpha_ice, p.alpha_cloud, p.alpha_water, p.snow_albedo_fresh, E.p.w_lai,
                 p.cloud_advect ? 1 : 0, p.use_topo_albedo ? 1 : 0, p.swe_enable ? 1 : 0,
                 (E.configured && E.p.albedo_couple && E.alpha_valid) ? 1 : 0, (E.configured && E.p.bands_couple && E.banded_valid) ? 1 : 0,
                 ((E.configured && E.p.water_couple && E.water_valid) || qd_phyto_daily_couples(c)) ? 1 : 0,
                 (E.configured && E.p.map_f32) ? 1 : 0};
        if (A.eco) { const int me = qd_plan(c, {QD_IN(F[QD_F_ECO_ALPHA], 0)}); if (me < 0) return -1; m = std::min(m, me); }
        if (A.banded) { const int me = qd_plan(c, {QD_IN(F[QD_F_ECO_ALPHA_BANDED], 0)}); if (me < 0) return -1; m = std::min(m, me); }
        if (A.water) { const int me = qd_plan(c, {QD_IN(F[QD_F_WATER_ALPHA], 0)}); if (me < 0) return -1; m = std::min(m, me); }
        {
            const int msn = qd_plan(c, {QD_IN(F[QD_F_PRECIP], 0), QD_IN(F[QD_F_H], 0), QD_IN(F[QD_F_S_SNOW], 0), QD_IN(F[QD_F_ELEVATION], 0)});
            if (msn < 0) return -1;
            QdSnowP S;
            S.dt = dt; S.ga = 9.81 / 1004.0; S.rho_snow_safe = std::max(p.rho_snow, 1e-6); S.polar_lat = p.polar_lat_thresh;
            S.ice_max = p.polar_ice_thick_max_m; S.elev_max = p.land_elev_max_m; S.gamma = p.lapse_k_kpm; S.lapse = p.lapse_enable;
            S.t_thresh = p.snow_thresh_K; S.dT = std::max(1e-6, p.snow_t_band_K); S.mode = p.snow_melt_mode;
            S.ddf_s = p.snow_ddf_mm_per_k_day / 86400.0; S.tref = p.snow_melt_tref_K; S.rate_s = p.snow_melt_rate_mm_day / 86400.0;
            S.swe_max = (p.swe_max_mm == p.swe_max_mm && p.swe_max_mm > 0) ? p.swe_max_mm : -1.0;
            S.swe_ref_safe = std::max(1e-6, p.swe_ref_mm); S.gl_frac = p.glacier_frac; S.gl_swe = p.glacier_swe_mm; S.swe = p.swe_enable;
            if (fc) {
                const QdForcingP Fo{QdStar{fc->sa[0], std::sin(fc->sa[1]), std::cos(fc->sa[1]), fc->sa[2]},
                                    QdStar{fc->sb[0], std::sin(fc->sb[1]), std::cos(fc->sb[1]), fc->sb[2]}, fc->theta, 5.670374e-8, 1};
                const int mm = std::min(m, msn);
                QdSafArgs K;
                K.T = c->tabs; K.S = S; K.A = A; K.Fo = Fo;
                K.precip = F[QD_F_PRECIP]; K.h = F[QD_F_H]; K.S_snow = F[QD_F_S_SNOW]; K.elev = F[QD_F_ELEVATION]; K.land = c->land;
                K.P_rain = F[QD_F_P_RAIN]; K.S_next = F[QD_F_S_SNOW_NEXT]; K.melt = F[QD_F_MELT]; K.C_snow = F[QD_F_C_SNOW]; K.glacier = F[QD_F_GLACIER];
                K.adv = adv; K.cloud = F[QD_F_CLOUD]; K.cloud_eff = c->cloud_eff_valid ? F[QD_F_CLOUD_EFF] : (const double*)nullptr;
                K.hice = F[QD_F_HICE]; K.base = F[QD_F_BASE_ALBEDO]; K.eco_alpha = F[QD_F_ECO_ALPHA]; K.banded = F[QD_F_ECO_ALPHA_BANDED];
                K.water = F[QD_F_WATER_ALPHA]; K.albedo = F[QD_F_ALBEDO]; K.isrA = F[QD_F_ISR_A]; K.isrB = F[QD_F_ISR_B]; K.isr = F[QD_F_ISR];
                K.Teq = F[QD_F_TEQ]; K.eday = c->eco.eday_dt > 0 ? F[QD_F_ECO_EDAY] : (double*)nullptr; K.eday_dt = c->eco.eday_dt;
                K.write_diag = c->diag_write;
                K.col1 = (c->want_pcond_ahead && !pcond_side && !pcond_pair && c->geo.full && p.cloud_couple && !isset(p.pcond_ref)) ? 1 : 0;
                K.P = qd_make_colp(c, dt);
                K.u = F[QD_F_U]; K.v = F[QD_F_V]; K.Ts = F[QD_F_TS]; K.q = F[QD_F_Q]; K.Pcond = F[QD_F_PCOND];
                if (pcond_pair && c->merge_saf && c->pcond_ahead == 3 && c->geo.full) {
                    K.G = c->geo;
                    delete (QdSafArgs*)c->saf_pending;
                    c->saf_pending = new QdSafArgs(K);
                } else
                QD_ROWS(c, mm, G, K.G = G; hipLaunchKernelGGL(k_snow_albedo_forcing, qd_grid2d(G), blk, 0, c->stream, K));
                c->eco.eday_dt = 0;
                if (K.col1) c->pcond_ahead = 1;
                qd_mark(c, {F[QD_F_P_RAIN], F[QD_F_S_SNOW_NEXT], F[QD_F_MELT], F[QD_F_C_SNOW], F[QD_F_GLACIER]}, mm);
                qd_mark(c, {F[QD_F_CLOUD], F[QD_F_ALBEDO], F[QD_F_ISR_A], F[QD_F_ISR_B], F[QD_F_ISR], F[QD_F_TEQ]}, mm);
                return 0;
            }
            QD_ROWS(c, msn, G, hipLaunchKernelGGL(k_snow_provisional, qd_grid2d(G), blk, 0, c->stream, G, c->tabs, S, F[QD_F_PRECIP],
                                                  F[QD_F_H], F[QD_F_S_SNOW], F[QD_F_ELEVATION], c->land, F[QD_F_P_RAIN],
                                                  F[QD_F_S_SNOW_NEXT], F[QD_F_MELT], F[QD_F_C_SNOW], F[QD_F_GLACIER]));
            qd_mark(c, {F[QD_F_P_RAIN], F[QD_F_S_SNOW_NEXT], F[QD_F_MELT], F[QD_F_C_SNOW], F[QD_F_GLACIER]}, msn);
// ... 67 lines not shown
```

qingdai_amd/csrc/qd_pointwise.h:

```cpp
#pragma once
#include "qd_internal.h"

struct QdSnowP {
    double dt, ga, rho_snow_safe, polar_lat, ice_max, elev_max, gamma, t_thresh, dT, ddf_s, tref, rate_s, swe_max, swe_ref_safe,
           gl_frac, gl_swe;
    int lapse, mode, swe;
};
struct QdSnowOut { double Pr, Sn, melt, Cs, gl; };

__device__ __forceinline__ QdSnowOut qd_snow_cell(const QdTabs& T, const QdSnowP& P, int i, bool is_land, double hval, double S0, double elev,
                                                  double Pf) {
    QdSnowOut r;
    const double T_a = 288.0 + P.ga * hval;
    const double h_snow = is_land ? qd_max(S0, 0.0) / P.rho_snow_safe : 0.0;
    const bool polar = fabs(T.lat_deg[i]) >= P.polar_lat;
    const double h_ice_eff = polar ? qd_min(h_snow, P.ice_max) : h_snow;
    const double H_eff = qd_min(elev + h_ice_eff, P.elev_max);
    const double T_hat = P.lapse ? T_a - P.gamma * (H_eff / 1000.0) : T_a;
    double f_snow = 1.0 / (1.0 + exp((T_hat - P.t_thresh) / P.dT));
    f_snow = qd_clip(f_snow, 0.0, 1.0);
    const double Ps = qd_nn(f_snow * Pf);
    const double Pr = qd_nn((1.0 - f_snow) * Pf);
    r.Pr = Pr;
    if (!P.swe) { r.Sn = S0; r.melt = 0.0; r.Cs = 0.0; r.gl = 0.0; return r; }
    const double Ps_land = Ps * (is_land ? 1.0 : 0.0);
    double melt_flux;
    if (P.mode == 0) melt_flux = P.ddf_s * qd_max(T_hat - P.tref, 0.0);
    else melt_flux = (T_hat >= P.t_thresh) ? P.rate_s : 0.0;
    const double actual = qd_min(qd_max(S0, 0.0), melt_flux * P.dt);
    double Sn = S0 + Ps_land * P.dt - actual;
    if (P.swe_max > 0.0) Sn = qd_min(Sn, P.swe_max);
    Sn = qd_max(0.0, Sn);
    const double melt_out = (P.dt > 0) ? actual / P.dt : 0.0;
    const double Cs = qd_clip(1.0 - exp(-qd_max(Sn, 0.0) / P.swe_ref_safe), 0.0, 1.0);
    Sn = qd_nn(Sn);
    const bool gl = is_land && ((Cs >= P.gl_frac) || (Sn >= P.gl_swe));
    const double Pr_gl = (Pr * (is_land ? 1.0 : 0.0)) * (gl ? 1.0 : 0.0);
    if (Pr_gl != 0.0) Sn = Sn + Pr_gl * P.dt;
    r.Sn = Sn; r.melt = qd_nn(melt_out); r.Cs = Cs; r.gl = gl ? 1.0 : 0.0;
    return r;
}

struct QdAlbP { double alpha, hice_ref_safe, alpha_ice, alpha_cloud, alpha_water, alpha_snow, w_lai; int do_adv, use_topo, snow, eco, banded, water, eco_f32; };

__device__ __forceinline__ double qd_albedo_cell(const QdAlbP& P, size_t o, double c, const double* __restrict__ cloud_eff,
                                                 const double* __restrict__ hice, const double* __restrict__ base, int landv, double cs, double gl,
                                                 const double* __restrict__ eco_alpha, const double* __restrict__ banded,
                                                 const double* __restrict__ water) {
    const double crad = cloud_eff ? cloud_eff[o] : c;
    const double C = qd_clip(crad, 0.0, 1.0);
    const double ice_frac = 1.0 - exp(-qd_max(hice[o], 0.0) / P.hice_ref_safe);
    double fi = qd_clip(ice_frac, 0.0, 1.0);
    fi = fi * ((landv == 0) ? 1.0 : 0.0);
    double b0 = P.use_topo ? base[o] : P.alpha_water;
    if (P.eco && landv == 1 && gl == 0.0) {
        const double ae = P.eco_f32 ? (double)reinterpret_cast<const float*>(eco_alpha)[o] : eco_alpha[o];
        if (fabs(ae) <= DBL_MAX) b0 = (1.0 - P.w_lai) * b0 + P.w_lai * ae;
    }
    if (P.banded && landv == 1) {
        const double ab = P.eco_f32 ? (double)reinterpret_cast<const float*>(banded)[o] : banded[o];
        if (fabs(ab) <= DBL_MAX) b0 = qd_clip(ab, 0.0, 1.0);
    }
    if (P.water && landv == 0) {
        const double aw = water[o];
        if (fabs(aw) <= DBL_MAX) b0 = qd_clip(aw, 0.0, 1.0);
    }
    if (P.snow && landv == 1) b0 = qd_clip((1.0 - cs) * b0 + cs * P.alpha_snow, 0.0, 1.0);
    const double surf = b0 * (1.0 - fi) + P.alpha_ice * fi;
    return qd_clip(surf * (1.0 - C) + P.alpha_cloud * C, 0.0, 1.0);
}

struct QdStar { double flux, sin_d, cos_d, alpha; };
struct QdForcingP { QdStar A, B; double theta, sigma; int with_teq; };

__device__ __forceinline__ void qd_star_insolation(const QdTabs& T, const QdStar& A, const QdStar& B, double theta, int i, int j,
                                                   double& a_, double& b_) {
    const double sl = T.sin_raw[i], cl = T.cos_raw[i], lon = T.lon_rad[j];
    const double hA = theta + lon - A.alpha;
    const double hB = theta + lon - B.alpha;
    const double czA = qd_max(0.0, sl * A.sin_d + cl * A.cos_d * cos(hA));
    const double czB = qd_max(0.0, sl * B.sin_d + cl * B.cos_d * cos(hB));
    a_ = A.flux * czA; b_ = B.flux * czB;
}

struct QdForcingOut { double tot, teq; };
__device__ __forceinline__ QdForcingOut qd_forcing_cell(const QdTabs& T, const QdForcingP& P, int i, int j, size_t o, double alb,
                                                        double* __restrict__ isrA, double* __restrict__ isrB, double* __restrict__ isr,
                                                        double* __restrict__ Teq, double* __restrict__ eday, double eday_dt) {
    double a_, b_;
    qd_star_insolation(T, P.A, P.B, P.theta, i, j, a_, b_);
    const double tot = a_ + b_;
    if (isrA) { isrA[o] = a_; isrB[o] = b_; }
    isr[o] = tot;
    if (eday) eday[o] += qd_nn(tot) * eday_dt;
    QdForcingOut r{tot, 0.0};
    if (P.with_teq) {
        double num = tot * (1 - alb);
        if (num < 0) num = 0;
        r.teq = sqrt(sqrt(num / P.sigma));
        if (Teq) Teq[o] = r.teq;
    }
    return r;
}
```

qingdai_amd/csrc/qd_saf.h:

```cpp
#pragma once
#include "qd_internal.h"
#include "qd_pointwise.h"
#include "qd_fluxes.h"

struct QdSafArgs {
    QdGeom G; QdTabs T; QdSnowP S; QdAlbP A; QdForcingP Fo;
    const double *precip, *h, *S_snow, *elev; const uint8_t* land;
    double *P_rain, *S_next, *melt, *C_snow, *glacier;
    const double* adv; double* cloud; const double *cloud_eff, *hice, *base, *eco_alpha, *banded, *water;
    double *albedo, *isrA, *isrB, *isr, *Teq, *eday; double eday_dt;
    int write_diag, col1; QdColP P; const double *u, *v, *Ts, *q; double* Pcond;
};
struct QdSafOut { double cloud, albedo, isr, teq; };

__device__ __forceinline__ QdSafOut qd_saf_cell(const QdSafArgs& K, int i, int j, size_t o, bool store_teq) {
    const int landv = K.land[o];
    const double hh = K.h[o];
    if (K.col1) {
        const double hi = K.hice[o];
        const double qsat_air = qd_qsat(288.0 + K.P.ga * hh, K.P.p0);
        K.Pcond[o] = qd_humidity_column(K.P, K.u[o], K.v[o], K.Ts[o], K.q[o], qsat_air, landv == 1, hi).Pc;
    }
    const QdSnowOut r = qd_snow_cell(K.T, K.S, i, landv == 1, hh, K.S_snow[o], K.elev[o], K.precip[o]);
    if (K.write_diag) { K.P_rain[o] = r.Pr; K.S_next[o] = r.Sn; K.melt[o] = r.melt; K.C_snow[o] = r.Cs; K.glacier[o] = r.gl; }
    double c = K.cloud[o];
    if (K.A.do_adv) { c = qd_clip((1.0 - K.A.alpha) * c + K.A.alpha * K.adv[o], 0.0, 1.0); K.cloud[o] = c; }
    const double alb = qd_albedo_cell(K.A, o, c, K.cloud_eff, K.hice, K.base, landv, r.Cs, r.gl, K.eco_alpha, K.banded, K.water);
    K.albedo[o] = alb;
    const QdForcingOut f = qd_forcing_cell(K.T, K.Fo, i, j, o, alb, K.write_diag ? K.isrA : nullptr, K.isrB, K.isr, store_teq ? K.Teq : nullptr,
                                           K.eday, K.eday_dt);
    return QdSafOut{c, alb, f.tot, f.teq};
}
```

qingdai_amd/csrc/qd_stencil.hip:

```cpp
#include "qd_internal.h"
#include "qd_device.h"
#include "qd_wave.h"
#include "qd_blockred.h"
#include <cstdlib>

__global__ void __launch_bounds__(QD_BLOCK)
k_laplacian(QdGeom G, QdFieldList fl, const double* __restrict__ cosf, double dphi, double dlam, double a) {
    const QdTile tl = qd_tile();
    const int j = tl.seg * QD_BLOCK + threadIdx.x;
    if (j >= G.nlon) return;
    const int i = G.row0 + tl.row;
    const int f = tl.fld;
    const size_t o = (size_t)qd_lrow(G, i) * G.nlon + j;
    fl.out[f][o] = qd_lap_point<true>(fl.in[f], G, cosf, i, j, dphi, dlam, a);
}

__global__ void __launch_bounds__(QD_BLOCK)
k_hyper_apply(QdGeom G, QdFieldList fl, const double* __restrict__ cosf, double dphi, double dlam, double a,
              double sub_dt) {
    const QdTile tl = qd_tile();
    const int j = tl.seg * QD_BLOCK + threadIdx.x;
    if (j >= G.nlon) return;
    const int i = G.row0 + tl.row;
    const int f = tl.fld;
// ... 98 lines not shown
    const int lane = threadIdx.x & 63, n = G.nlat;
    const int jraw = cs * W - NP + lane;
    const int j = jraw < 0 ? jraw + G.nlon : (jraw >= G.nlon ? jraw - G.nlon : jraw);
    const bool own = lane >= NP && lane < 64 - NP && jraw < G.nlon;
    const unsigned vo = (unsigned)j * 8u, vs = own ? (unsigned)jraw * 8u : QD_BUF_OOB;
    const unsigned slab = (unsigned)(G.lrows_ + QD_PAD_ROWS) * (unsigned)G.nlon * 8u;
    const qd_rsrc src = qd_buf(fl.in[blockIdx.y], slab), dst = qd_buf(fl.out[blockIdx.y], slab);
    int a[NP + 1], b[NP + 1];
    a[NP] = G.row0 + rs * R; b[NP] = min(a[NP] + R, G.row0 + G.nrows) - 1;
#pragma unroll
    for (int p = NP; p > 0; --p) { a[p - 1] = max(0, a[p] - 1); b[p - 1] = min(n - 1, b[p] + 1); }
    const int t0 = a[0], t1 = b[NP] + NP;
    auto row_off = [&](int g) { return (unsigned)min(qd_lrow(G, min(g, n - 1)), G.lrows_ - 1) * (unsigned)G.nlon; };
    double pf[QD_SH_PF], h1[NP], h2[NP];
#pragma unroll
    for (int k = 0; k < QD_SH_PF; ++k) pf[k] = qd_buf_ld(src, row_off(t0 + k), vo);
#pragma unroll
    for (int p = 0; p < NP; ++p) h1[p] = h2[p] = 0.0;
    int t_lo = t0, t_hi = t1;
#pragma unroll
    for (int p = 1; p <= NP; ++p) { t_lo = max(t_lo, a[p] + p); t_hi = min(t_hi, min(min(b[p] + 1, b[p - 1]), n - 1) + (p - 1)); }
    auto tick = [&](int t, double cur) {
        if (t > t1) return;
        if (scrub) cur = qd_nn(cur);
        bool live = false;
#pragma unroll
        for (int p = 1; p <= NP; ++p) {
            const int rp = t - (p - 1);
            live = false;
            if (rp < a[p - 1] || rp > b[p - 1] + (b[p - 1] == n - 1 ? 1 : 0)) continue;
            const double l = rp <= n - 1 ? (qd_west(cur) * 0.25 + cur * 0.5) + qd_east(cur) * 0.25 : h1[p - 1];
            if (rp == a[p - 1]) { h1[p - 1] = l; h2[p - 1] = l; continue; }
            const double o = (h2[p - 1] * 0.25 + h1[p - 1] * 0.5) + l * 0.25;
            h2[p - 1] = h1[p - 1]; h1[p - 1] = l;
            live = rp - 1 >= a[p] && rp - 1 <= b[p];
            if (live) cur = o;
        }
        if (live) qd_buf_st(dst, row_off(t - NP), vs, cur);
    };
    auto tick_all = [&](int t, double cur) {
        cur = scrub ? qd_nn(cur) : cur;
#pragma unroll
        for (int p = 0; p < NP; ++p) {
            const double l = (qd_west(cur) * 0.25 + cur * 0.5) + qd_east(cur) * 0.25;
            const double o = (h2[p] * 0.25 + h1[p] * 0.5) + l * 0.25;
            h2[p] = h1[p]; h1[p] = l;
            cur = o;
        }
        qd_buf_st(dst, row_off(t - NP), vs, cur);
    };
    static_assert(QD_SH_PF == 8, "the tick loop is written as two half-rings of four");
    for (int tb = t0; tb <= t1; tb += QD_SH_PF) {
        if (tb >= t_lo && tb + 3 <= t_hi) {
#pragma unroll
            for (int k = 0; k < 4; ++k) { const double cur = pf[k]; pf[k] = qd_buf_ld(src, row_off(tb + k + QD_SH_PF), vo); tick_all(tb + k, cur); }
        } else {
#pragma unroll
            for (int k = 0; k < 4; ++k) { const double cur = pf[k]; pf[k] = qd_buf_ld(src, row_off(tb + k + QD_SH_PF), vo); tick(tb + k, cur); }
        }
        if (tb + 4 >= t_lo && tb + 7 <= t_hi) {
#pragma unroll
            for (int k = 4; k < 8; ++k) { const double cur = pf[k]; pf[k] = qd_buf_ld(src, row_off(tb + k + QD_SH_PF), vo); tick_all(tb + k, cur); }
        } else {
#pragma unroll
            for (int k = 4; k < 8; ++k) { const double cur = pf[k]; pf[k] = qd_buf_ld(src, row_off(tb + k + QD_SH_PF), vo); tick(tb + k, cur); }
        }
    }
}

static int qd_shapiro_rows(const qd_ctx* c) { return c->tune.shapiro_r > 0 ? c->tune.shapiro_r : 12; }

int qd_shapiro_fields(qd_ctx* c, double** fields, int n, int npass, int m_out) {
    if (npass < 1) npass = 1;
    QdFieldList a; a.n = n;
    if (npass <= 3 && c->geo.nlon >= 64 && c->shapiro_stream) {
        QdScope sc(c, "k_shapiro_stream");
        for (int k = 0; k < n; ++k) { a.in[k] = fields[k]; a.out[k] = qd_scratch(c, k); a.aux[k] = nullptr; a.k4row[k] = nullptr; a.k4s[k] = 0; }
        const int R = qd_shapiro_rows(c), W = 64 - 2 * npass, ntc = (c->geo.nlon + W - 1) / W;
        QD_ROWS(c, m_out, G, {
            const int ns = ((G.nrows + R - 1) / R) * ntc;
            const dim3 grid((ns + QD_SH_WAVES - 1) / QD_SH_WAVES, n), blk(64 * QD_SH_WAVES);
            if (npass == 1) hipLaunchKernelGGL(k_shapiro_stream<1>, grid, blk, 0, c->stream, G, a, 1, R, ntc, ns);
            else if (npass == 2) hipLaunchKernelGGL(k_shapiro_stream<2>, grid, blk, 0, c->stream, G, a, 1, R, ntc, ns);
            else hipLaunchKernelGGL(k_shapiro_stream<3>, grid, blk, 0, c->stream, G, a, 1, R, ntc, ns);
        });
        for (int k = 0; k < n; ++k) { double* t = fields[k]; fields[k] = c->scratch[k]; c->scratch[k] = t; qd_mark(c, {fields[k]}, m_out); }
        return 0;
    }
    QdScope sc(c, "k_shapiro_pass");
    for (int p = 0; p < npass; ++p) {
        for (int k = 0; k < n; ++k) { a.in[k] = fields[k]; a.out[k] = qd_scratch(c, k); a.aux[k] = nullptr; a.k4row[k] = nullptr; a.k4s[k] = 0; }
        const int m = m_out + (npass - 1 - p);
        qd_launch_shapiro_pass(c, a, p == 0, m);
        for (int k = 0; k < n; ++k) { double* t = fields[k]; fields[k] = c->scratch[k]; c->scratch[k] = t; qd_mark(c, {fields[k]}, m); }
    }
    return 0;
}

__global__ void __launch_bounds__(QD_BLOCK)
k_advect(QdGeom G, const double* __restrict__ u, const double* __restrict__ v, const double* __restrict__ cosl,
         double dt, double a, double dlat, double dlon,
         const double* __restrict__ f0, double* __restrict__ o0,
         const double* __restrict__ f1, double* __restrict__ o1, double alpha, int clipq) {
    const QdTile tl = qd_tile();
    const int j = tl.seg * QD_BLOCK + threadIdx.x;
    if (j >= G.nlon) return;
    const int i = G.row0 + tl.row;
    const size_t o = (size_t)qd_lrow(G, i) * G.nlon + j;
    const QdBilin b = qd_departure(G, i, j, u[o], v[o], dt, a, cosl[i], dlat, dlon);
    const bool blend = (alpha != 1.0);
    {
        const double adv = qd_gather(f0, G, b);
        o0[o] = blend ? (1.0 - alpha) * f0[o] + alpha * adv : adv;
    }
    if (f1) {
        const double adv = qd_gather(f1, G, b);
        double x = blend ? (1.0 - alpha) * f1[o] + alpha * adv : adv;
        if (clipq) x = qd_clip(qd_nn(x), 0.0, 0.5);
        o1[o] = x;
    }
}

void qd_launch_advect(qd_ctx* c, const double* u, const double* v, const double* coslat, double dt,
                      const double* f0, double* o0, const double* f1, double* o1, double alpha, int clipq, int m) {
    QD_ROWS(c, m, G, hipLaunchKernelGGL(k_advect, qd_grid2d(G), dim3(QD_BLOCK), 0, c->stream, G, u, v, coslat, dt,
                                        c->p.a, c->dlat, c->dlon, f0, o0, f1, o1, alpha, clipq));
    qd_mark(c, {o0, o1}, m);
}

__global__ void __launch_bounds__(QD_BLOCK)
k_divvort(QdGeom G, QdTabs T, const double* __restrict__ u, const double* __restrict__ v, double* __restrict__ out,
          double a, double dlat, double dlon, int vort) {
    const QdTile tl = qd_tile();
    const int j = tl.seg * QD_BLOCK + threadIdx.x;
    if (j >= G.nlon) return;
    const int i = G.row0 + tl.row;
    out[(size_t)qd_lrow(G, i) * G.nlon + j] =
        vort ? qd_divvort_point(G, T, v, u, i, j, a, dlat, dlon, 1) : qd_divvort_point(G, T, u, v, i, j, a, dlat, dlon, 0);
}

void qd_launch_divvort(qd_ctx* c, const double* u, const double* v, double* out, int vort, int m) {
    QD_ROWS(c, m, G, hipLaunchKernelGGL(k_divvort, qd_grid2d(G), dim3(QD_BLOCK), 0, c->stream, G, c->tabs, u, v, out,
                                        c->p.a, c->dlat, c->dlon, vort));
    qd_mark(c, {out}, m);
}

#define QD_GAUSS_MAXR 24
struct QdGaussW { double w[QD_GAUSS_MAXR + 1]; int r; };

__device__ __forceinline__ int qd_ext(int i, int n, int mode_wrap) {
    if (mode_wrap) { i %= n; return i < 0 ? i + n : i; }
    const int p = 2 * n;
    i %= p; if (i < 0) i += p;
    return i >= n ? p - 1 - i : i;
}

__global__ void __launch_bounds__(QD_BLOCK)
k_gauss_axis(QdGeom G, const double* __restrict__ in, double* __restrict__ out, QdGaussW W, int axis, int mode_wrap) {
    const QdTile tl = qd_tile();
    const int j = tl.seg * QD_BLOCK + threadIdx.x;
    if (j >= G.nlon) return;
    const int i = G.row0 + tl.row;
    const size_t o = (size_t)qd_lrow(G, i) * G.nlon + j;
    double tmp = in[o] * W.w[0];
    if (axis == 0) {
        for (int k = W.r; k >= 1; --k) {
            const double lo = in[(size_t)qd_lrow(G, qd_ext(i - k, G.nlat, mode_wrap)) * G.nlon + j];
            const double hi = in[(size_t)qd_lrow(G, qd_ext(i + k, G.nlat, mode_wrap)) * G.nlon + j];
            tmp += (lo + hi) * W.w[k];
        }
    } else {
        const size_t b = (size_t)qd_lrow(G, i) * G.nlon;
        for (int k = W.r; k >= 1; --k) {
            const double lo = in[b + qd_ext(j - k, G.nlon, mode_wrap)];
            const double hi = in[b + qd_ext(j + k, G.nlon, mode_wrap)];
            tmp += (lo + hi) * W.w[k];
        }
    }
    out[o] = tmp;
}

__global__ void __launch_bounds__(QD_BLOCK) k_clip01_field(QdGeom G, double* __restrict__ x) {
    const QdTile tl = qd_tile();
    const int j = tl.seg * QD_BLOCK + threadIdx.x;
    if (j >= G.nlon) return;
    const size_t o = (size_t)qd_lrow(G, G.row0 + tl.row) * G.nlon + j;
    x[o] = qd_clip(x[o], 0.0, 1.0);
}

__global__ void __launch_bounds__(QD_BLOCK)
k_gauss_fused(QdGeom G, const double* __restrict__ in, double* __restrict__ out, QdGaussW W, int mode_wrap, int clip01,
              const double* __restrict__ scale_p, double scale_k) {
    __shared__ double sm[QD_BLOCK + 2 * QD_GAUSS_MAXR];
    const QdTile tl = qd_tile();
    const int i = G.row0 + tl.row;
    const int jbase = tl.seg * QD_BLOCK;
    const int r = W.r;
    for (int s = threadIdx.x; s < QD_BLOCK + 2 * r; s += QD_BLOCK) {
        const int jj = jbase - r + s;
        if (jj >= G.nlon + r) break;
        const int j = qd_ext(jj, G.nlon, mode_wrap);
        const double sc = scale_p ? *scale_p : scale_k;
        double tmp = (in[(size_t)qd_lrow(G, i) * G.nlon + j] * sc) * W.w[0];
        for (int k = r; k >= 1; --k) {
            const double lo = in[(size_t)qd_lrow(G, qd_ext(i - k, G.nlat, mode_wrap)) * G.nlon + j] * sc;
            const double hi = in[(size_t)qd_lrow(G, qd_ext(i + k, G.nlat, mode_wrap)) * G.nlon + j] * sc;
            tmp += (lo + hi) * W.w[k];
        }
        sm[s] = tmp;
    }
    __syncthreads();
    const int j = jbase + threadIdx.x;
    if (j >= G.nlon) return;
    const int c0 = threadIdx.x + r;
    double acc = sm[c0] * W.w[0];
    for (int k = r; k >= 1; --k) acc += (sm[c0 - k] + sm[c0 + k]) * W.w[k];
    if (clip01) acc = qd_clip(acc, 0.0, 1.0);
    out[(size_t)qd_lrow(G, i) * G.nlon + j] = acc;
}

#define QD_GB 8
template <int RR>
__global__ void __launch_bounds__(QD_BLOCK)
k_gauss_rows(QdGeom G, const double* __restrict__ in, double* __restrict__ out, QdGaussW W, int mode_wrap, int clip01,
             const double* __restrict__ scale_p, double scale_k) {
    constexpr int OWN = QD_BLOCK - 2 * RR;
    __shared__ double sm[QD_GB][QD_BLOCK];
    const int i0 = G.row0 + (int)blockIdx.y * QD_GB;
    const int nvalid = min(QD_GB, G.row0 + G.nrows - i0);
    const int jbase = (int)blockIdx.x * OWN;
    const double sc = scale_p ? *scale_p : scale_k;
    double w[RR + 1];
#pragma unroll
    for (int k = 0; k <= RR; ++k) w[k] = W.w[k];
    {
        const int s = threadIdx.x;
        const int jj = jbase - RR + s;
        if (jj < G.nlon + RR) {
            const int j = qd_ext(jj, G.nlon, mode_wrap);
            double x[QD_GB + 2 * RR];
#pragma unroll
            for (int q = 0; q < QD_GB + 2 * RR; ++q) {
                const int qq = q < nvalid + 2 * RR ? q : nvalid + 2 * RR - 1;
                x[q] = in[(size_t)qd_lrow(G, qd_ext(i0 - RR + qq, G.nlat, mode_wrap)) * G.nlon + j] * sc;
            }
#pragma unroll
            for (int k = 0; k < QD_GB; ++k) {
                double tmp = x[k + RR] * w[0];
#pragma unroll
                for (int q = RR; q >= 1; --q) tmp += (x[k + RR - q] + x[k + RR + q]) * w[q];
                sm[k][s] = tmp;
            }
        }
    }
    __syncthreads();
    const int c0 = threadIdx.x;
    const int j = jbase + c0 - RR;
    if (c0 < RR || c0 >= QD_BLOCK - RR || j >= G.nlon) return;
#pragma unroll
    for (int k = 0; k < QD_GB; ++k) {
        if (k >= nvalid) break;
        double acc = sm[k][c0] * w[0];
#pragma unroll
        for (int q = RR; q >= 1; --q) acc += (sm[k][c0 - q] + sm[k][c0 + q]) * w[q];
        if (clip01) acc = qd_clip(acc, 0.0, 1.0);
        out[(size_t)qd_lrow(G, i0 + k) * G.nlon + j] = acc;
    }
}

template <int RR>
static void qd_launch_gauss_rows(qd_ctx* c, const double* in, double* out, const QdGaussW& W, int mode_wrap, int clip01,
                                 const double* scale_p, double scale_k, int m_out) {
    constexpr int OWN = QD_BLOCK - 2 * RR;
    QD_ROWS(c, m_out, G, hipLaunchKernelGGL(k_gauss_rows<RR>, dim3((G.nlon + OWN - 1) / OWN, (G.nrows + QD_GB - 1) / QD_GB),
                                            dim3(QD_BLOCK), 0, c->stream, G, in, out, W, mode_wrap, clip01, scale_p, scale_k));
}

static bool qd_gauss_weights(double sigma, QdGaussW& W) {
    const int r = (int)(4.0 * sigma + 0.5);
    if (r > QD_GAUSS_MAXR) return false;
    W.r = r;
    std::vector<double> phi(2 * r + 1);
    const double s2 = sigma * sigma;
    for (int x = -r; x <= r; ++x) phi[x + r] = std::exp(-0.5 / s2 * (double)(x * x));
    double tot;
    const int m = 2 * r + 1;
    if (m < 8) { tot = 0.0; for (int k = 0; k < m; ++k) tot += phi[k]; }
    else {
        double acc[8];
        for (int k = 0; k < 8; ++k) acc[k] = phi[k];
        int k = 8;
        for (; k < m - (m % 8); k += 8) for (int t = 0; t < 8; ++t) acc[t] += phi[k + t];
        tot = ((acc[0] + acc[1]) + (acc[2] + acc[3])) + ((acc[4] + acc[5]) + (acc[6] + acc[7]));
        for (; k < m; ++k) tot += phi[k];
    }
    for (int k = 0; k <= r; ++k) W.w[k] = phi[r + k] / tot;
    return true;
}

struct QdGaussPairP {
    int op; double w_mem, w_p, w_src, tend, c_floor;
    int fold, fold_n, use_fb; const double* partial; double wsum, pq_min, p_blend, dcrit; double* scal_out;
};
template <int RR, bool POS>
__device__ __forceinline__ void qd_gauss_rows_pass(const QdGeom& G, const double* __restrict__ in, double sc, const double (&w)[RR + 1],
                                                   int mode_wrap, int i0, int nvalid, int jbase, double (*sm)[QD_BLOCK], double (&acc)[QD_GB],
                                                   double dcrit = 0.0) {
    {
        const int s = threadIdx.x;
        const int jj = jbase - RR + s;
        if (jj < G.nlon + RR) {
            const int j = qd_ext(jj, G.nlon, mode_wrap);
            double x[QD_GB + 2 * RR];
#pragma unroll
            for (int q = 0; q < QD_GB + 2 * RR; ++q) {
                const int qq = q < nvalid + 2 * RR ? q : nvalid + 2 * RR - 1;
                const double v = in[(size_t)qd_lrow(G, qd_ext(i0 - RR + qq, G.nlat, mode_wrap)) * G.nlon + j];
                x[q] = (POS ? qd_max(0.0, -(v - dcrit)) : v) * sc;
            }
#pragma unroll
            for (int k = 0; k < QD_GB; ++k) {
                double tmp = x[k + RR] * w[0];
#pragma unroll
                for (int q = RR; q >= 1; --q) tmp += (x[k + RR - q] + x[k + RR + q]) * w[q];
                sm[k][s] = tmp;
            }
        }
    }
    __syncthreads();
    const int c0 = threadIdx.x;
    if (c0 >= RR && c0 < QD_BLOCK - RR) {
#pragma unroll
        for (int k = 0; k < QD_GB; ++k) {
            double a = sm[k][c0] * w[0];
#pragma unroll
            for (int q = RR; q >= 1; --q) a += (sm[k][c0 - q] + sm[k][c0 + q]) * w[q];
            acc[k] = a;
        }
    }
    __syncthreads();
}

template <int RR>
__global__ void __launch_bounds__(QD_BLOCK)
k_gauss_pair(QdGeom G, const double* __restrict__ inA, const double* __restrict__ inB, QdGaussW W, int mode_wrap,
             const double* __restrict__ scA_p, double scA_k, double scB_k, const double* __restrict__ sc, QdGaussPairP P,
             double* __restrict__ outA, double* __restrict__ outB, double* __restrict__ out0) {
    constexpr int OWN = QD_BLOCK - 2 * RR;
    __shared__ double sm[QD_GB][QD_BLOCK];
    const int i0 = G.row0 + (int)blockIdx.y * QD_GB;
    const int nvalid = min(QD_GB, G.row0 + G.nrows - i0);
    const int jbase = (int)blockIdx.x * OWN;
    double w[RR + 1];
#pragma unroll
    for (int k = 0; k <= RR; ++k) w[k] = W.w[k];
    double scA, al;
    if (P.fold) {
        __shared__ double s_sc[2];
        qd_precip_scalars_wg(P.partial, P.fold_n, P.wsum, P.pq_min, P.p_blend, P.use_fb, s_sc);
        if (threadIdx.x == 0 && blockIdx.x == 0 && blockIdx.y == 0) { P.scal_out[0] = s_sc[0]; P.scal_out[1] = s_sc[1]; }
        scA = s_sc[0]; al = s_sc[1];
    } else {
        scA = scA_p ? *scA_p : scA_k;
        al = (P.op == 1) ? sc[1] : 0.0;
    }
    double a[QD_GB], b[QD_GB];
#pragma unroll
    for (int k = 0; k < QD_GB; ++k) { a[k] = 0.0; b[k] = 0.0; }
    qd_gauss_rows_pass<RR, false>(G, inA, scA, w, mode_wrap, i0, nvalid, jbase, sm, a);
    if (P.fold) { if (al != 0.0) qd_gauss_rows_pass<RR, true>(G, inB, scB_k, w, mode_wrap, i0, nvalid, jbase, sm, b, P.dcrit); }
    else if (P.op != 1 || al != 0.0) qd_gauss_rows_pass<RR, false>(G, inB, scB_k, w, mode_wrap, i0, nvalid, jbase, sm, b);
    const int c0 = threadIdx.x;
    const int j = jbase + c0 - RR;
    if (c0 < RR || c0 >= QD_BLOCK - RR || j >= G.nlon) return;
#pragma unroll
    for (int k = 0; k < QD_GB; ++k) {
        if (k >= nvalid) break;
        const size_t o = (size_t)qd_lrow(G, i0 + k) * G.nlon + j;
        if (P.op == 1) {
            double p = a[k];
            if (al != 0.0) p = (1.0 - al) * p + al * b[k];
            out0[o] = qd_max(p, 0.0);
        } else {
            const double cp = qd_clip(a[k], 0.0, 1.0), sr = qd_clip(b[k], 0.0, 1.0);
            outA[o] = cp; outB[o] = sr;
            const double c0v = out0[o];
            const double tendency = sr * P.tend;
            double c = (P.w_mem * c0v + P.w_p * cp + P.w_src * qd_clip(c0v + tendency, 0.0, 1.0));
            if (P.c_floor > 0.0) c = qd_max(c, qd_clip(P.c_floor * cp, 0.0, 1.0));
            out0[o] = qd_clip(c, 0.0, 1.0);
        }
    }
}

bool qd_gauss_pair_ok(const qd_ctx* c, double sigma) {
    const int r = qd_gauss_radius(sigma);
    return c->use_fused && c->merge_pointwise && sigma > 1e-15 && c->geo.nlon > 2 * r && (r == 1 || r == 2 || r == 4);
}
int qd_gaussian_pair(qd_ctx* c, const double* inA, const double* inB, double sigma, int mode_wrap, const double* scA_p, double scA_k,
                     double scB_k, const double* sc, int op, const double* blend5, double* outA, double* outB, double* out0, int m_out,
                     const QdPrecipFold* fold) {
    QdGaussW W;
    if (!qd_gauss_weights(sigma, W)) return qd_fail(c, "gaussian radius too large");
    QdGaussPairP P{op, 0, 0, 0, 0, 0, 0, 0, 0, nullptr, 0, 0, 0, 0, nullptr};
    if (blend5) { P.w_mem = blend5[0]; P.w_p = blend5[1]; P.w_src = blend5[2]; P.tend = blend5[3]; P.c_floor = blend5[4]; }
    if (fold) {
        if (op != 1 || !c->geo.full) return qd_fail(c, "qd_gaussian_pair: the folded scalars belong to the precipitation blend of a whole-globe handle");
        P.fold = 1; P.fold_n = fold->n; P.use_fb = fold->use_fb; P.partial = fold->partial; P.wsum = fold->wsum; P.pq_min = fold->pq_min;
        P.p_blend = fold->p_blend; P.dcrit = fold->dcrit; P.scal_out = fold->out;
    }
    const int r = W.r;
    QD_ROWS(c, m_out, G,
        const dim3 grid((G.nlon + (QD_BLOCK - 2 * r) - 1) / (QD_BLOCK - 2 * r), (G.nrows + QD_GB - 1) / QD_GB);
        if (r == 1) hipLaunchKernelGGL(k_gauss_pair<1>, grid, dim3(QD_BLOCK), 0, c->stream, G, inA, inB, W, mode_wrap, scA_p, scA_k, scB_k, sc, P, outA, outB, out0);
        else if (r == 2) hipLaunchKernelGGL(k_gauss_pair<2>, grid, dim3(QD_BLOCK), 0, c->stream, G, inA, inB, W, mode_wrap, scA_p, scA_k, scB_k, sc, P, outA, outB, out0);
        else hipLaunchKernelGGL(k_gauss_pair<4>, grid, dim3(QD_BLOCK), 0, c->stream, G, inA, inB, W, mode_wrap, scA_p, scA_k, scB_k, sc, P, outA, outB, out0));
    return 0;
}

int qd_gaussian(qd_ctx* c, const double* in, double* out, double* tmp, double sigma, int mode_wrap, int m_out, int clip01,
                const double* scale_p, double scale_k) {
    const bool scaled = scale_p != nullptr || scale_k != 1.0;
    if (scaled && !(c->use_fused && out != in && sigma > 1e-15 && c->geo.nlon > 2 * qd_gauss_radius(sigma)))
        return qd_fail(c, "qd_gaussian: input scaling needs the fused blur");
    if (!(sigma > 1e-15)) {
        if (out != in) hipMemcpyAsync(out, in, c->geo.cells() * sizeof(double), hipMemcpyDeviceToDevice, c->stream);
        qd_mark(c, {out}, m_out);
        return 0;
    }
    QdGaussW W;
    if (!qd_gauss_weights(sigma, W)) return qd_fail(c, "gaussian radius too large");
    const int r = W.r;
    if (c->use_fused && out != in && c->geo.nlon > 2 * r && (r == 1 || r == 2 || r == 4)) {
        QdScope sc(c, r == 1 ? "k_gauss_rows1" : (r == 2 ? "k_gauss_rows2" : "k_gauss_rows4"));
        if (r == 1) qd_launch_gauss_rows<1>(c, in, out, W, mode_wrap, clip01, scale_p, scale_k, m_out);
        else if (r == 2) qd_launch_gauss_rows<2>(c, in, out, W, mode_wrap, clip01, scale_p, scale_k, m_out);
        else qd_launch_gauss_rows<4>(c, in, out, W, mode_wrap, clip01, scale_p, scale_k, m_out);
        qd_mark(c, {out}, m_out);
        return 0;
    }
    if (c->use_fused && out != in && c->geo.nlon > 2 * r) {
        QdScope sc(c, "k_gauss_fused");
        QD_ROWS(c, m_out, G, hipLaunchKernelGGL(k_gauss_fused, qd_grid2d(G), dim3(QD_BLOCK), 0, c->stream, G, in, out, W, mode_wrap, clip01, scale_p, scale_k));
        qd_mark(c, {out}, m_out);
        return 0;
    }
    QdScope sc(c, "k_gauss_axis");
    QD_ROWS(c, m_out, G, hipLaunchKernelGGL(k_gauss_axis, qd_grid2d(G), dim3(QD_BLOCK), 0, c->stream, G, in, tmp, W, 0, mode_wrap));
    QD_ROWS(c, m_out, G, hipLaunchKernelGGL(k_gauss_axis, qd_grid2d(G), dim3(QD_BLOCK), 0, c->stream, G, tmp, out, W, 1, mode_wrap));
    qd_mark(c, {tmp, out}, m_out);
    if (clip01) {
        QD_ROWS(c, m_out, G, hipLaunchKernelGGL(k_clip01_field, qd_grid2d(G), dim3(QD_BLOCK), 0, c->stream, G, out));
    }
    return 0;
}

bool qd_gauss_can_fuse(const qd_ctx* c, double sigma) { return c->use_fused && sigma > 1e-15 && c->geo.nlon > 2 * qd_gauss_radius(sigma); }

int qd_gaussian_swap(qd_ctx* c, double*& field, double*& tmp, double sigma, int mode_wrap, int m_out, int clip01,
                     const double* scale_p, double scale_k) {
    if (!(sigma > 1e-15)) {
        if (clip01) QD_ROWS(c, m_out, G, hipLaunchKernelGGL(k_clip01_field, qd_grid2d(G), dim3(QD_BLOCK), 0, c->stream, G, field));
        return 0;
    }
    if (c->use_fused && c->geo.nlon > 2 * qd_gauss_radius(sigma)) {
        if (qd_gaussian(c, field, tmp, nullptr, sigma, mode_wrap, m_out, clip01, scale_p, scale_k)) return -1;
        std::swap(field, tmp);
        return 0;
    }
    if (scale_p != nullptr || scale_k != 1.0) return qd_fail(c, "qd_gaussian_swap: input scaling needs the fused blur");
    return qd_gaussian(c, field, field, tmp, sigma, mode_wrap, m_out, clip01);
}


__global__ void __launch_bounds__(QD_BLOCK) k_scrub_field(QdGeom G, double* __restrict__ x) {
    const QdTile tl = qd_tile();
    const int j = tl.seg * QD_BLOCK + threadIdx.x;
    if (j >= G.nlon) return;
    const size_t o = (size_t)qd_lrow(G, G.row0 + tl.row) * G.nlon + j;
    x[o] = qd_nn(x[o]);
}

__global__ void __launch_bounds__(QD_BLOCK)
k_zonal_filter(QdGeom G, QdFieldList fl, const double* __restrict__ tw, int kcut, int kN, double one_minus_s) {
    extern __shared__ double zs[];
    const int n = G.nlon, nb = kN - kcut + 1;
    double* x = zs;
    double* tc = x + n;
    double* ts = tc + n;
    double* Xr = ts + n;
    double* Xi = Xr + nb;
    const int i = G.row0 + blockIdx.y, f = blockIdx.z;
    double* Frow = fl.out[f] + (size_t)qd_lrow(G, i) * n;
    for (int j = threadIdx.x; j < n; j += QD_BLOCK) { x[j] = qd_nn(Frow[j]); tc[j] = tw[j]; ts[j] = tw[n + j]; }
    __syncthreads();
    for (int b = threadIdx.x; b < nb; b += QD_BLOCK) {
        const int k = kcut + b;
        double ar = 0.0, ai = 0.0;
        int idx = 0;
        for (int j = 0; j < n; ++j) {
            const double v = x[j];
            ar += v * tc[idx];
            ai -= v * ts[idx];
            idx += k; if (idx >= n) idx -= n;
        }
        Xr[b] = ar; Xi[b] = ai;
    }
    __syncthreads();
    const bool even = (n & 1) == 0;
    const double inv_n = 1.0 / (double)n;
    for (int j = threadIdx.x; j < n; j += QD_BLOCK) {
        double hp = 0.0;
        int idx = (int)(((long long)j * kcut) % n);
        for (int b = 0; b < nb; ++b) {
            const bool nyq = even && (kcut + b == kN);
            const double t = Xr[b] * tc[idx] - (nyq ? 0.0 : Xi[b] * ts[idx]);
            hp += nyq ? t : 2.0 * t;
            idx += j; if (idx >= n) idx -= n;
        }
        Frow[j] = qd_nn(x[j] - one_minus_s * (hp * inv_n));
    }
}

int qd_zonal_filter_fields(qd_ctx* c, double** fields, int nf, double cutoff, double damp, int m) {
    const int n = c->geo.nlon;
    if (!(damp > 0.0) || !(cutoff > 0.0) || n / 2 + 1 <= 1) {
        QdScope sc(c, "k_scrub_field");
        for (int f = 0; f < nf; ++f)
            QD_ROWS(c, m, G, hipLaunchKernelGGL(k_scrub_field, qd_grid2d(G), dim3(QD_BLOCK), 0, c->stream, G, fields[f]));
        return 0;
    }
    const int kN = n / 2;
    const int kcut = std::max(1, std::min(kN, (int)(cutoff * (double)kN)));
    const double s = std::max(0.0, 1.0 - std::min(1.0, damp));
    if (!c->zonal_tw) {
        std::vector<double> tw(2 * (size_t)n);
        for (int k = 0; k < n; ++k) { const double a = 2.0 * M_PI * (double)k / (double)n; tw[k] = std::cos(a); tw[n + k] = std::sin(a); }
        if (hipMalloc(&c->zonal_tw, tw.size() * sizeof(double)) != hipSuccess) return qd_fail(c, "hipMalloc zonal twiddles");
        QD_HIP(c, hipMemcpy(c->zonal_tw, tw.data(), tw.size() * sizeof(double), hipMemcpyHostToDevice));
    }
    const int nb = kN - kcut + 1;
    const size_t lds = sizeof(double) * (3 * (size_t)n + 2 * (size_t)nb);
    if (lds > 150 * 1024) return qd_fail(c, "zonal filter: row too long for the LDS-staged DFT");
    static bool once[QD_MAX_DEVICES] = {false};
    const int dv = c->desc.device >= 0 && c->desc.device < QD_MAX_DEVICES ? c->desc.device : 0;
    if (!once[dv]) { hipFuncSetAttribute((const void*)k_zonal_filter, hipFuncAttributeMaxDynamicSharedMemorySize, 150 * 1024); once[dv] = c->desc.device == dv; }
    QdFieldList fl{}; fl.n = nf;
    for (int f = 0; f < nf; ++f) { fl.in[f] = fields[f]; fl.out[f] = fields[f]; }
    QdScope sc(c, "k_zonal_filter");
    QD_ROWS(c, m, G, hipLaunchKernelGGL(k_zonal_filter, dim3(1, G.nrows, nf), dim3(QD_BLOCK), lds, c->stream, G, fl, c->zonal_tw,
                                        kcut, kN, 1.0 - s));
    qd_mark(c, {fields[0], nf > 1 ? fields[1] : fields[0], nf > 2 ? fields[2] : fields[0]}, m);
    return 0;
}
```

Baseline: 5.121 planet-days/s.

## Split pointwise kernels into load/compute/store phases to hoist global loads

Restructures the column, snow-albedo-forcing, albedo, forcing, SST clamp, polar fill and Gaussian pair kernels so that all global loads are issued up front, then the arithmetic runs, then all stores happen. The goal is to expose memory-level parallelism, letting loads overlap instead of being serialized behind stores the compiler cannot reorder past due to possible aliasing. In the polar fill kernel, the eta update is also spread across all segments instead of running only in segment 0. The cost is higher register pressure from holding many values live, which could lower occupancy.

```diff
diff --git a/qingdai_amd/csrc/qd_atmos.hip b/qingdai_amd/csrc/qd_atmos.hip
--- a/qingdai_amd/csrc/qd_atmos.hip
+++ b/qingdai_amd/csrc/qd_atmos.hip
@@ -15,25 +15,41 @@
     unsigned long long* npos;
 };
 
-struct QdColIn { double cloud, isr, albedo, teq; };
+struct QdColVals { double u, v, h, Ts, hice, q, Teq, cloud, isr, albedo, pref, csmap; bool land; };
+struct QdColRes { QdHum Hm; double cloud_eff, olr, Ts, h, hice; bool hice_changed; };
 
 template <int PHASE, bool HAS_ALB>
-__device__ __forceinline__ void qd_column_cell(const QdColP& P, const QdColPtrs& A, size_t o, const QdColIn* IN, int i, int nlat) {
-    const double u = A.u[o], v = A.v[o], h = A.h[o], Ts = A.Ts[o];
-    const double hice = A.hice[o];
-    const bool land = (A.land[o] == 1);
+__device__ __forceinline__ QdColVals qd_column_load(const QdColP& P, const QdColPtrs& A, size_t o, bool staged) {
+    QdColVals c;
+    c.u = A.u[o]; c.v = A.v[o]; c.Ts = A.Ts[o]; c.q = A.q[o];
+    c.h = c.hice = c.Teq = c.cloud = c.isr = c.albedo = c.pref = c.csmap = 0.0; c.land = false;
+    if (!staged) { c.h = A.h[o]; c.hice = A.hice[o]; c.land = (A.land[o] == 1); }
+    if (PHASE == 1) return c;
+    if (!staged) c.Teq = A.Teq[o];
+    if (HAS_ALB) {
+        if (!staged) { c.cloud = A.cloud[o]; c.isr = A.isr[o]; c.albedo = A.albedo[o]; }
+        if (P.couple) c.pref = *A.pref;
+        if (!P.seaice && P.has_csmap) c.csmap = A.csmap[o];
+    }
+    return c;
+}
+
+template <int PHASE, bool HAS_ALB>
+__device__ __forceinline__ QdColRes qd_column_cell(const QdColP& P, const QdColVals& C, int i, int nlat) {
+    QdColRes R;
+    const double u = C.u, v = C.v, h = C.h, Ts = C.Ts;
+    const double hice = C.hice;
+    const bool land = C.land;
     const bool ocean = !land;
     const double T_a = 288.0 + P.ga * h;
     const double qsat_air = qd_qsat(T_a, P.p0);
 
-    const QdHum Hm = qd_humidity_column(P, u, v, Ts, A.q[o], qsat_air, land, hice);
-    const double q = Hm.q, E = Hm.E, Pc = Hm.Pc, LH = Hm.LH, LHrel = Hm.LHrel;
-    if (PHASE == 1) { A.Pcond[o] = Pc; return; }
-    A.q[o] = q; A.LH[o] = LH;
-    if (PHASE != 2) A.Pcond[o] = Pc;
-    if (P.write_diag) { A.E[o] = E; A.LHrel[o] = LHrel; }
-
-    const double Teq = IN ? IN->teq : A.Teq[o];
+    const QdHum Hm = qd_humidity_column(P, u, v, Ts, C.q, qsat_air, land, hice);
+    const double q = Hm.q, Pc = Hm.Pc, LH = Hm.LH, LHrel = Hm.LHrel;
+    R.Hm = Hm; R.cloud_eff = 0.0; R.olr = 0.0; R.Ts = Ts; R.h = h; R.hice = hice; R.hice_changed = false;
+    if (PHASE == 1) return R;
+
+    const double Teq = C.Teq;
     const double olr_old = P.sigma * qd_pow4(Ts);
     const double net_old = P.sigma * qd_pow4(Teq) + P.gfs * qd_pow4(T_a) - olr_old;
     const double Ts_newton = Ts + (net_old / P.c_sfc_safe) * P.dt;
@@ -41,17 +57,17 @@
     double Ts_new, h_new = h;
     QdFlux F;
     if (HAS_ALB) {
-        const double cloud = IN ? IN->cloud : A.cloud[o];
+        const double cloud = C.cloud;
         double cloud_eff;
         if (P.couple) {
             const double RH = qd_clip(q / qd_max(1e-12, qsat_air), 0.0, 1.5);
             const double rh_excess = qd_max(0.0, RH - P.rh0);
-            const double P_ref = *A.pref;
+            const double P_ref = C.pref;
             const double p_term = qd_tanh(P_ref > 0 ? Pc / P_ref : 0.0);
             cloud_eff = qd_clip(cloud + P.k_q * rh_excess + P.k_p * p_term, 0.0, 1.0);
         } else cloud_eff = cloud;
-        A.cloud_eff[o] = cloud_eff;
-        F = qd_surface_fluxes(P, IN ? IN->isr : A.isr[o], IN ? IN->albedo : A.albedo[o], cloud_eff, Ts, T_a, u, v, land, hice);
+        R.cloud_eff = cloud_eff;
+        F = qd_surface_fluxes(P, C.isr, C.albedo, cloud_eff, Ts, T_a, u, v, land, hice);
         double Ts_energy;
         if (P.seaice) {
             double Q = F.SW_sfc - F.LW_sfc - F.SH - LH;
@@ -76,21 +92,21 @@
             if (hi > 0.0 && ocean) Tn = qd_min(Tn, P.t_freeze);
             Tn = qd_max(P.t_floor, Tn);
             Ts_energy = qd_nn(Tn);
-            { const double hn_ = qd_nn(hi); if (__double_as_longlong(hn_) != __double_as_longlong(hice)) A.hice[o] = hn_; }
+            { const double hn_ = qd_nn(hi); R.hice = hn_; R.hice_changed = __double_as_longlong(hn_) != __double_as_longlong(hice); }
         } else {
             const double net = F.SW_sfc - F.LW_sfc - F.SH - LH;
             double Cs;
-            if (P.has_csmap) { const double cm = A.csmap[o]; Cs = (isfinite(cm) && cm > 1e3) ? cm : 1e3; }
+            if (P.has_csmap) { const double cm = C.csmap; Cs = (isfinite(cm) && cm > 1e3) ? cm : 1e3; }
             else Cs = P.c_sfc_safe;
             Ts_energy = qd_nn(qd_max(P.t_floor, Ts + (net / Cs) * P.dt));
         }
-        if (P.write_diag) A.olr[o] = F.OLR;
+        R.olr = F.OLR;
         Ts_new = (1.0 - P.w_energy) * Ts_newton + P.w_energy * Ts_energy;
     } else {
-        if (P.write_diag) A.olr[o] = olr_old;
+        R.olr = olr_old;
         Ts_new = Ts_newton;
     }
-    A.Ts[o] = Ts_new;
+    R.Ts = Ts_new;
 
     const double h_eq = P.h_eq_fac * Teq;
     h_new = h + ((h_eq - h) / P.tau_rad) * P.dt;
@@ -98,7 +114,23 @@
         const double F_atm = F.SW_atm + F.LW_atm + F.SH + LHrel;
         h_new = qd_nn(h_new + P.atm_w * (F_atm / P.atm_denom) * P.dt);
     }
-    A.h[o] = h_new;
+    R.h = h_new;
+    return R;
+}
+
+template <int PHASE, bool HAS_ALB>
+__device__ __forceinline__ void qd_column_store(const QdColP& P, const QdColPtrs& A, size_t o, const QdColRes& R) {
+    if (PHASE == 1) { A.Pcond[o] = R.Hm.Pc; return; }
+    A.q[o] = R.Hm.q; A.LH[o] = R.Hm.LH;
+    if (PHASE != 2) A.Pcond[o] = R.Hm.Pc;
+    if (P.write_diag) { A.E[o] = R.Hm.E; A.LHrel[o] = R.Hm.LHrel; }
+    if (HAS_ALB) {
+        A.cloud_eff[o] = R.cloud_eff;
+        if (P.seaice && R.hice_changed) A.hice[o] = R.hice;
+    }
+    if (P.write_diag) A.olr[o] = R.olr;
+    A.Ts[o] = R.Ts;
+    A.h[o] = R.h;
 }
 
 template <int PHASE, bool HAS_ALB>
@@ -108,7 +140,10 @@
     const int j = tl.seg * QD_BLOCK + threadIdx.x;
     if (j >= G.nlon) return;
     const int i = G.row0 + tl.row;
-    qd_column_cell<PHASE, HAS_ALB>(P, A, (size_t)qd_lrow(G, i) * G.nlon + j, nullptr, i, G.nlat);
+    const size_t o = (size_t)qd_lrow(G, i) * G.nlon + j;
+    const QdColVals C = qd_column_load<PHASE, HAS_ALB>(P, A, o, false);
+    const QdColRes R = qd_column_cell<PHASE, HAS_ALB>(P, C, i, G.nlat);
+    qd_column_store<PHASE, HAS_ALB>(P, A, o, R);
 }
 
 __global__ void __launch_bounds__(QD_BLOCK)
@@ -118,9 +153,14 @@
     if (j >= K.G.nlon) return;
     const int i = K.G.row0 + tl.row;
     const size_t o = (size_t)qd_lrow(K.G, i) * K.G.nlon + j;
-    const QdSafOut s = qd_saf_cell(K, i, j, o, K.write_diag != 0);
-    const QdColIn in{s.cloud, s.isr, s.albedo, s.teq};
-    qd_column_cell<2, true>(P, A, o, &in, i, K.G.nlat);
+    const QdSafIn s = qd_saf_load(K, i, j, o);
+    QdColVals C = qd_column_load<2, true>(P, A, o, true);
+    const QdSafOut S = qd_saf_cell(K, s);
+    C.h = s.h; C.hice = s.hice; C.land = (s.landv == 1);
+    C.Teq = S.f.teq; C.cloud = S.cloud; C.isr = S.f.tot; C.albedo = S.albedo;
+    qd_saf_store(K, o, s, S, K.write_diag != 0);
+    const QdColRes R = qd_column_cell<2, true>(P, C, i, K.G.nlat);
+    qd_column_store<2, true>(P, A, o, R);
 }
 
 struct QdMomP { double g, a, dt, dlat, dlon, f_min; int primitive; };
@@ -197,7 +237,9 @@
     if (j >= G.nlon) return;
     const int i = G.row0 + tl.row;
     const size_t o = (size_t)qd_lrow(G, i) * G.nlon + j;
-    qd_forcing_cell(T, P, i, j, o, P.with_teq ? albedo[o] : 0.0, isrA, isrB, isr, Teq, eday, eday_dt);
+    const double alb = P.with_teq ? albedo[o] : 0.0, eday0 = eday ? eday[o] : 0.0;
+    const double sl = T.sin_raw[i], cl = T.cos_raw[i], lon = T.lon_rad[j];
+    qd_forcing_store(P, o, qd_forcing_cell(P, sl, cl, lon, alb), eday0, isrA, isrB, isr, Teq, eday, eday_dt);
 }
 
 int qd_forcing_impl(qd_ctx* c, const double* sa, const double* sb, double theta, int with_teq) {
diff --git a/qingdai_amd/csrc/qd_ocean.hip b/qingdai_amd/csrc/qd_ocean.hip
--- a/qingdai_amd/csrc/qd_ocean.hip
+++ b/qingdai_amd/csrc/qd_ocean.hip
@@ -551,11 +551,14 @@
                                                   const uint8_t* __restrict__ land, const uint8_t* __restrict__ ice, int has_ice,
                                                   double* __restrict__ Ts_atm, double* __restrict__ eta, const double* __restrict__ eta_mean,
                                                   double eta_cap) {
-    if (eta) eta[o] = qd_clip(qd_nn(eta[o] - *eta_mean), -eta_cap, eta_cap);
+    const double e0 = eta ? eta[o] : 0.0, em = eta ? *eta_mean : 0.0;
     const double t0 = sst[o];
+    const int ld = land[o], ic = ice[o];
+    const double e1 = qd_clip(qd_nn(e0 - em), -eta_cap, eta_cap);
     const double t = qd_clip(t0, tmin, tmax);
+    if (eta) eta[o] = e1;
     if (__double_as_longlong(t) != __double_as_longlong(t0)) sst[o] = t;
-    if (inject && land[o] == 0 && !(has_ice && ice[o] != 0)) Ts_atm[o] = t;
+    if (inject && ld == 0 && !(has_ice && ic != 0)) Ts_atm[o] = t;
 }
 
 __global__ void __launch_bounds__(QD_BLOCK)
@@ -578,24 +581,37 @@
     const QdTile tl = qd_tile();
     const int i = G.row0 + tl.row;
     if (i == 0 || i == G.nlat - 1) {
-        if (tl.seg != 0) return;
         const bool north = i != 0;
         const size_t b = (size_t)qd_lrow(G, i) * G.nlon;
         if (G.nlon > QD_PF_CH * QD_BLOCK) {
+            if (tl.seg != 0) return;
             qd_polar_fill_row(G, T, land, sst, uo, vo, north, &sm[0][0]);
             __syncthreads();
             for (int j = threadIdx.x; j < G.nlon; j += QD_BLOCK)
                 qd_sst_clamp_cell(b + j, sst, tmin, tmax, inject, land, ice, has_ice, Ts_atm, eta, eta_mean, eta_cap);
             return;
         }
-        double t_[QD_PF_CH], u_[QD_PF_CH], v_[QD_PF_CH], sl_[QD_PF_CH], cl_[QD_PF_CH]; int ld_[QD_PF_CH];
+        const int js = tl.seg * QD_BLOCK + threadIdx.x;
+        const bool edo = eta != nullptr && js < G.nlon;
+        double e0 = 0.0, em = 0.0;
+        if (edo) { e0 = eta[b + js]; em = *eta_mean; }
+        if (tl.seg != 0) {
+            if (edo) eta[b + js] = qd_clip(qd_nn(e0 - em), -eta_cap, eta_cap);
+            return;
+        }
+        double t_[QD_PF_CH], u_[QD_PF_CH], v_[QD_PF_CH], sl_[QD_PF_CH], cl_[QD_PF_CH]; int ld_[QD_PF_CH], ic_[QD_PF_CH];
 #pragma unroll
         for (int k = 0; k < QD_PF_CH; ++k) {
             const int j = threadIdx.x + k * QD_BLOCK;
             const int jj = j < G.nlon ? j : G.nlon - 1;
-            ld_[k] = j < G.nlon ? (int)land[b + jj] : 1;
+            ld_[k] = (int)land[b + jj];
+            ic_[k] = (int)ice[b + jj];
             t_[k] = sst[b + jj]; u_[k] = uo[b + jj]; v_[k] = vo[b + jj]; sl_[k] = T.sin_lon[jj]; cl_[k] = T.cos_lon[jj];
         }
+        if (edo) eta[b + js] = qd_clip(qd_nn(e0 - em), -eta_cap, eta_cap);
+#pragma unroll
+        for (int k = 0; k < QD_PF_CH; ++k)
+            if (threadIdx.x + k * QD_BLOCK >= G.nlon) ld_[k] = 1;
         double cnt = 0, sT = 0, s0 = 0, s1 = 0;
 #pragma unroll
         for (int k = 0; k < QD_PF_CH; ++k) {
@@ -626,10 +642,9 @@
                 uo[o] = (-sl_[k]) * m0 + cl_[k] * m1;
                 vo[o] = nx * m0 + ny * m1;
             }
-            if (eta) eta[o] = qd_clip(qd_nn(eta[o] - *eta_mean), -eta_cap, eta_cap);
             const double t = qd_clip(tv, tmin, tmax);
             sst[o] = t;
-            if (inject && ld_[k] == 0 && !(has_ice && ice[o] != 0)) Ts_atm[o] = t;
+            if (inject && ld_[k] == 0 && !(has_ice && ic_[k] != 0)) Ts_atm[o] = t;
         }
         return;
     }
diff --git a/qingdai_amd/csrc/qd_physics.hip b/qingdai_amd/csrc/qd_physics.hip
--- a/qingdai_amd/csrc/qd_physics.hip
+++ b/qingdai_amd/csrc/qd_physics.hip
@@ -184,11 +184,16 @@
     if (j >= G.nlon) return;
     const size_t o = (size_t)qd_lrow(G, G.row0 + tl.row) * G.nlon + j;
     double c = cloud[o];
-    if (P.do_adv) { c = qd_clip((1.0 - P.alpha) * c + P.alpha * adv[o], 0.0, 1.0); cloud[o] = c; }
+    const double av = P.do_adv ? adv[o] : 0.0, hi = hice[o];
     const int landv = land[o];
-    const double cs = (P.snow && landv == 1) ? csnow[o] : 0.0;
-    const double gl = (P.eco && landv == 1) ? glacier[o] : 0.0;
-    albedo[o] = qd_albedo_cell(P, o, c, cloud_eff, hice, base, landv, cs, gl, eco_alpha, banded, water);
+    const double cs0 = P.snow ? csnow[o] : 0.0, gl0 = P.eco ? glacier[o] : 0.0;
+    const QdAlbIn in = qd_albedo_load(P, o, cloud_eff, base, eco_alpha, banded, water);
+    if (P.do_adv) c = qd_clip((1.0 - P.alpha) * c + P.alpha * av, 0.0, 1.0);
+    const double cs = (landv == 1) ? cs0 : 0.0;
+    const double gl = (landv == 1) ? gl0 : 0.0;
+    const double alb = qd_albedo_cell(P, in, c, hi, landv, cs, gl);
+    if (P.do_adv) cloud[o] = c;
+    albedo[o] = alb;
 }
 
 __global__ void k_precip_scalars_post(const double* raw, double wsum, double pq_min, double p_blend, int use_fb, double* out) {
@@ -225,7 +230,7 @@
     if (j >= G.nlon) return;
     const int i = G.row0 + tl.row;
     const size_t o = (size_t)qd_lrow(G, i) * G.nlon + j;
-    const QdSnowOut r = qd_snow_cell(T, P, i, land[o] == 1, h[o], S_snow[o], elev[o], precip[o]);
+    const QdSnowOut r = qd_snow_cell(P, T.lat_deg[i], land[o] == 1, h[o], S_snow[o], elev[o], precip[o]);
     P_rain[o] = r.Pr; S_next[o] = r.Sn; melt[o] = r.melt; C_snow[o] = r.Cs; glacier[o] = r.gl;
 }
 
@@ -235,7 +240,9 @@
     const int j = tl.seg * QD_BLOCK + threadIdx.x;
     if (j >= K.G.nlon) return;
     const int i = K.G.row0 + tl.row;
-    qd_saf_cell(K, i, j, (size_t)qd_lrow(K.G, i) * K.G.nlon + j, true);
+    const size_t o = (size_t)qd_lrow(K.G, i) * K.G.nlon + j;
+    const QdSafIn s = qd_saf_load(K, i, j, o);
+    qd_saf_store(K, o, s, qd_saf_cell(K, s), true);
 }
 int qd_saf_launch(qd_ctx* c, const QdSafArgs& K) {
     hipLaunchKernelGGL(k_snow_albedo_forcing, qd_grid2d(K.G), dim3(QD_BLOCK), 0, c->stream, K);
diff --git a/qingdai_amd/csrc/qd_pointwise.h b/qingdai_amd/csrc/qd_pointwise.h
--- a/qingdai_amd/csrc/qd_pointwise.h
+++ b/qingdai_amd/csrc/qd_pointwise.h
@@ -8,12 +8,12 @@
 };
 struct QdSnowOut { double Pr, Sn, melt, Cs, gl; };
 
-__device__ __forceinline__ QdSnowOut qd_snow_cell(const QdTabs& T, const QdSnowP& P, int i, bool is_land, double hval, double S0, double elev,
+__device__ __forceinline__ QdSnowOut qd_snow_cell(const QdSnowP& P, double lat_deg, bool is_land, double hval, double S0, double elev,
                                                   double Pf) {
     QdSnowOut r;
     const double T_a = 288.0 + P.ga * hval;
     const double h_snow = is_land ? qd_max(S0, 0.0) / P.rho_snow_safe : 0.0;
-    const bool polar = fabs(T.lat_deg[i]) >= P.polar_lat;
+    const bool polar = fabs(lat_deg) >= P.polar_lat;
     const double h_ice_eff = polar ? qd_min(h_snow, P.ice_max) : h_snow;
     const double H_eff = qd_min(elev + h_ice_eff, P.elev_max);
     const double T_hat = P.lapse ? T_a - P.gamma * (H_eff / 1000.0) : T_a;
@@ -43,26 +43,36 @@
 
 struct QdAlbP { double alpha, hice_ref_safe, alpha_ice, alpha_cloud, alpha_water, alpha_snow, w_lai; int do_adv, use_topo, snow, eco, banded, water, eco_f32; };
 
-__device__ __forceinline__ double qd_albedo_cell(const QdAlbP& P, size_t o, double c, const double* __restrict__ cloud_eff,
-                                                 const double* __restrict__ hice, const double* __restrict__ base, int landv, double cs, double gl,
-                                                 const double* __restrict__ eco_alpha, const double* __restrict__ banded,
-                                                 const double* __restrict__ water) {
-    const double crad = cloud_eff ? cloud_eff[o] : c;
+struct QdAlbIn { int has_ce; double crad, base, eco, banded, water; float eco32, banded32; };
+__device__ __forceinline__ QdAlbIn qd_albedo_load(const QdAlbP& P, size_t o, const double* __restrict__ cloud_eff, const double* __restrict__ base,
+                                                  const double* __restrict__ eco_alpha, const double* __restrict__ banded,
+                                                  const double* __restrict__ water) {
+    QdAlbIn r{cloud_eff != nullptr, 0.0, 0.0, 0.0, 0.0, 0.0, 0.0f, 0.0f};
+    if (cloud_eff) r.crad = cloud_eff[o];
+    if (P.use_topo) r.base = base[o];
+    if (P.eco) { if (P.eco_f32) r.eco32 = reinterpret_cast<const float*>(eco_alpha)[o]; else r.eco = eco_alpha[o]; }
+    if (P.banded) { if (P.eco_f32) r.banded32 = reinterpret_cast<const float*>(banded)[o]; else r.banded = banded[o]; }
+    if (P.water) r.water = water[o];
+    return r;
+}
+
+__device__ __forceinline__ double qd_albedo_cell(const QdAlbP& P, const QdAlbIn& in, double c, double hice, int landv, double cs, double gl) {
+    const double crad = in.has_ce ? in.crad : c;
     const double C = qd_clip(crad, 0.0, 1.0);
-    const double ice_frac = 1.0 - exp(-qd_max(hice[o], 0.0) / P.hice_ref_safe);
+    const double ice_frac = 1.0 - exp(-qd_max(hice, 0.0) / P.hice_ref_safe);
     double fi = qd_clip(ice_frac, 0.0, 1.0);
     fi = fi * ((landv == 0) ? 1.0 : 0.0);
-    double b0 = P.use_topo ? base[o] : P.alpha_water;
+    double b0 = P.use_topo ? in.base : P.alpha_water;
     if (P.eco && landv == 1 && gl == 0.0) {
-        const double ae = P.eco_f32 ? (double)reinterpret_cast<const float*>(eco_alpha)[o] : eco_alpha[o];
+        const double ae = P.eco_f32 ? (double)in.eco32 : in.eco;
         if (fabs(ae) <= DBL_MAX) b0 = (1.0 - P.w_lai) * b0 + P.w_lai * ae;
     }
     if (P.banded && landv == 1) {
-        const double ab = P.eco_f32 ? (double)reinterpret_cast<const float*>(banded)[o] : banded[o];
+        const double ab = P.eco_f32 ? (double)in.banded32 : in.banded;
         if (fabs(ab) <= DBL_MAX) b0 = qd_clip(ab, 0.0, 1.0);
     }
     if (P.water && landv == 0) {
-        const double aw = water[o];
+        const double aw = in.water;
         if (fabs(aw) <= DBL_MAX) b0 = qd_clip(aw, 0.0, 1.0);
     }
     if (P.snow && landv == 1) b0 = qd_clip((1.0 - cs) * b0 + cs * P.alpha_snow, 0.0, 1.0);
@@ -73,32 +83,37 @@
 struct QdStar { double flux, sin_d, cos_d, alpha; };
 struct QdForcingP { QdStar A, B; double theta, sigma; int with_teq; };
 
-__device__ __forceinline__ void qd_star_insolation(const QdTabs& T, const QdStar& A, const QdStar& B, double theta, int i, int j,
-                                                   double& a_, double& b_) {
-    const double sl = T.sin_raw[i], cl = T.cos_raw[i], lon = T.lon_rad[j];
+__device__ __forceinline__ void qd_star_insolation_v(const QdStar& A, const QdStar& B, double theta, double sl, double cl, double lon,
+                                                     double& a_, double& b_) {
     const double hA = theta + lon - A.alpha;
     const double hB = theta + lon - B.alpha;
     const double czA = qd_max(0.0, sl * A.sin_d + cl * A.cos_d * cos(hA));
     const double czB = qd_max(0.0, sl * B.sin_d + cl * B.cos_d * cos(hB));
     a_ = A.flux * czA; b_ = B.flux * czB;
 }
+__device__ __forceinline__ void qd_star_insolation(const QdTabs& T, const QdStar& A, const QdStar& B, double theta, int i, int j,
+                                                   double& a_, double& b_) {
+    qd_star_insolation_v(A, B, theta, T.sin_raw[i], T.cos_raw[i], T.lon_rad[j], a_, b_);
+}
 
-struct QdForcingOut { double tot, teq; };
-__device__ __forceinline__ QdForcingOut qd_forcing_cell(const QdTabs& T, const QdForcingP& P, int i, int j, size_t o, double alb,
-                                                        double* __restrict__ isrA, double* __restrict__ isrB, double* __restrict__ isr,
-                                                        double* __restrict__ Teq, double* __restrict__ eday, double eday_dt) {
-    double a_, b_;
-    qd_star_insolation(T, P.A, P.B, P.theta, i, j, a_, b_);
-    const double tot = a_ + b_;
-    if (isrA) { isrA[o] = a_; isrB[o] = b_; }
-    isr[o] = tot;
-    if (eday) eday[o] += qd_nn(tot) * eday_dt;
-    QdForcingOut r{tot, 0.0};
+struct QdForcingOut { double a, b, tot, teq; };
+__device__ __forceinline__ QdForcingOut qd_forcing_cell(const QdForcingP& P, double sl, double cl, double lon, double alb) {
+    QdForcingOut r;
+    qd_star_insolation_v(P.A, P.B, P.theta, sl, cl, lon, r.a, r.b);
+    r.tot = r.a + r.b;
+    r.teq = 0.0;
     if (P.with_teq) {
-        double num = tot * (1 - alb);
+        double num = r.tot * (1 - alb);
         if (num < 0) num = 0;
         r.teq = sqrt(sqrt(num / P.sigma));
-        if (Teq) Teq[o] = r.teq;
     }
     return r;
 }
+__device__ __forceinline__ void qd_forcing_store(const QdForcingP& P, size_t o, const QdForcingOut& f, double eday0, double* __restrict__ isrA,
+                                                 double* __restrict__ isrB, double* __restrict__ isr, double* __restrict__ Teq,
+                                                 double* __restrict__ eday, double eday_dt) {
+    if (isrA) { isrA[o] = f.a; isrB[o] = f.b; }
+    isr[o] = f.tot;
+    if (eday) eday[o] = eday0 + qd_nn(f.tot) * eday_dt;
+    if (P.with_teq && Teq) Teq[o] = f.teq;
+}
diff --git a/qingdai_amd/csrc/qd_saf.h b/qingdai_amd/csrc/qd_saf.h
--- a/qingdai_amd/csrc/qd_saf.h
+++ b/qingdai_amd/csrc/qd_saf.h
@@ -11,23 +11,42 @@
     double *albedo, *isrA, *isrB, *isr, *Teq, *eday; double eday_dt;
     int write_diag, col1; QdColP P; const double *u, *v, *Ts, *q; double* Pcond;
 };
-struct QdSafOut { double cloud, albedo, isr, teq; };
+struct QdSafIn { int landv; double h, hice, S_snow, elev, precip, cloud, adv, eday, lat_deg, sl, cl, lon, u, v, Ts, q; QdAlbIn al; };
+struct QdSafOut { QdSnowOut r; double Pc, cloud, albedo; QdForcingOut f; };
 
-__device__ __forceinline__ QdSafOut qd_saf_cell(const QdSafArgs& K, int i, int j, size_t o, bool store_teq) {
-    const int landv = K.land[o];
-    const double hh = K.h[o];
+__device__ __forceinline__ QdSafIn qd_saf_load(const QdSafArgs& K, int i, int j, size_t o) {
+    QdSafIn s;
+    s.landv = K.land[o];
+    s.h = K.h[o]; s.hice = K.hice[o]; s.S_snow = K.S_snow[o]; s.elev = K.elev[o]; s.precip = K.precip[o]; s.cloud = K.cloud[o];
+    s.adv = K.A.do_adv ? K.adv[o] : 0.0;
+    s.eday = K.eday ? K.eday[o] : 0.0;
+    s.lat_deg = K.T.lat_deg[i]; s.sl = K.T.sin_raw[i]; s.cl = K.T.cos_raw[i]; s.lon = K.T.lon_rad[j];
+    s.u = s.v = s.Ts = s.q = 0.0;
+    if (K.col1) { s.u = K.u[o]; s.v = K.v[o]; s.Ts = K.Ts[o]; s.q = K.q[o]; }
+    s.al = qd_albedo_load(K.A, o, K.cloud_eff, K.base, K.eco_alpha, K.banded, K.water);
+    return s;
+}
+
+__device__ __forceinline__ QdSafOut qd_saf_cell(const QdSafArgs& K, const QdSafIn& s) {
+    QdSafOut R;
+    R.Pc = 0.0;
     if (K.col1) {
-        const double hi = K.hice[o];
-        const double qsat_air = qd_qsat(288.0 + K.P.ga * hh, K.P.p0);
-        K.Pcond[o] = qd_humidity_column(K.P, K.u[o], K.v[o], K.Ts[o], K.q[o], qsat_air, landv == 1, hi).Pc;
+        const double qsat_air = qd_qsat(288.0 + K.P.ga * s.h, K.P.p0);
+        R.Pc = qd_humidity_column(K.P, s.u, s.v, s.Ts, s.q, qsat_air, s.landv == 1, s.hice).Pc;
     }
-    const QdSnowOut r = qd_snow_cell(K.T, K.S, i, landv == 1, hh, K.S_snow[o], K.elev[o], K.precip[o]);
-    if (K.write_diag) { K.P_rain[o] = r.Pr; K.S_next[o] = r.Sn; K.melt[o] = r.melt; K.C_snow[o] = r.Cs; K.glacier[o] = r.gl; }
-    double c = K.cloud[o];
-    if (K.A.do_adv) { c = qd_clip((1.0 - K.A.alpha) * c + K.A.alpha * K.adv[o], 0.0, 1.0); K.cloud[o] = c; }
-    const double alb = qd_albedo_cell(K.A, o, c, K.cloud_eff, K.hice, K.base, landv, r.Cs, r.gl, K.eco_alpha, K.banded, K.water);
-    K.albedo[o] = alb;
-    const QdForcingOut f = qd_forcing_cell(K.T, K.Fo, i, j, o, alb, K.write_diag ? K.isrA : nullptr, K.isrB, K.isr, store_teq ? K.Teq : nullptr,
-                                           K.eday, K.eday_dt);
-    return QdSafOut{c, alb, f.tot, f.teq};
+    R.r = qd_snow_cell(K.S, s.lat_deg, s.landv == 1, s.h, s.S_snow, s.elev, s.precip);
+    double c = s.cloud;
+    if (K.A.do_adv) c = qd_clip((1.0 - K.A.alpha) * c + K.A.alpha * s.adv, 0.0, 1.0);
+    R.cloud = c;
+    R.albedo = qd_albedo_cell(K.A, s.al, c, s.hice, s.landv, R.r.Cs, R.r.gl);
+    R.f = qd_forcing_cell(K.Fo, s.sl, s.cl, s.lon, R.albedo);
+    return R;
 }
+
+__device__ __forceinline__ void qd_saf_store(const QdSafArgs& K, size_t o, const QdSafIn& s, const QdSafOut& R, bool store_teq) {
+    if (K.col1) K.Pcond[o] = R.Pc;
+    if (K.write_diag) { K.P_rain[o] = R.r.Pr; K.S_next[o] = R.r.Sn; K.melt[o] = R.r.melt; K.C_snow[o] = R.r.Cs; K.glacier[o] = R.r.gl; }
+    if (K.A.do_adv) K.cloud[o] = R.cloud;
+    K.albedo[o] = R.albedo;
+    qd_forcing_store(K.Fo, o, R.f, s.eday, K.write_diag ? K.isrA : nullptr, K.isrB, K.isr, store_teq ? K.Teq : nullptr, K.eday, K.eday_dt);
+}
diff --git a/qingdai_amd/csrc/qd_stencil.hip b/qingdai_amd/csrc/qd_stencil.hip
--- a/qingdai_amd/csrc/qd_stencil.hip
+++ b/qingdai_amd/csrc/qd_stencil.hip
@@ -424,22 +424,28 @@
     int op; double w_mem, w_p, w_src, tend, c_floor;
     int fold, fold_n, use_fb; const double* partial; double wsum, pq_min, p_blend, dcrit; double* scal_out;
 };
+template <int RR>
+__device__ __forceinline__ void qd_gauss_rows_load(const QdGeom& G, const double* __restrict__ in, int mode_wrap, int i0, int nvalid, int jbase,
+                                                   double (&x)[QD_GB + 2 * RR]) {
+    const int jj = jbase - RR + (int)threadIdx.x;
+    if (jj < G.nlon + RR) {
+        const int j = qd_ext(jj, G.nlon, mode_wrap);
+#pragma unroll
+        for (int q = 0; q < QD_GB + 2 * RR; ++q) {
+            const int qq = q < nvalid + 2 * RR ? q : nvalid + 2 * RR - 1;
+            x[q] = in[(size_t)qd_lrow(G, qd_ext(i0 - RR + qq, G.nlat, mode_wrap)) * G.nlon + j];
+        }
+    }
+}
 template <int RR, bool POS>
-__device__ __forceinline__ void qd_gauss_rows_pass(const QdGeom& G, const double* __restrict__ in, double sc, const double (&w)[RR + 1],
-                                                   int mode_wrap, int i0, int nvalid, int jbase, double (*sm)[QD_BLOCK], double (&acc)[QD_GB],
-                                                   double dcrit = 0.0) {
+__device__ __forceinline__ void qd_gauss_rows_pass(const QdGeom& G, double (&x)[QD_GB + 2 * RR], double sc, const double (&w)[RR + 1],
+                                                   int jbase, double (*sm)[QD_BLOCK], double (&acc)[QD_GB], double dcrit = 0.0) {
     {
         const int s = threadIdx.x;
         const int jj = jbase - RR + s;
         if (jj < G.nlon + RR) {
-            const int j = qd_ext(jj, G.nlon, mode_wrap);
-            double x[QD_GB + 2 * RR];
-#pragma unroll
-            for (int q = 0; q < QD_GB + 2 * RR; ++q) {
-                const int qq = q < nvalid + 2 * RR ? q : nvalid + 2 * RR - 1;
-                const double v = in[(size_t)qd_lrow(G, qd_ext(i0 - RR + qq, G.nlat, mode_wrap)) * G.nlon + j];
-                x[q] = (POS ? qd_max(0.0, -(v - dcrit)) : v) * sc;
-            }
+#pragma unroll
+            for (int q = 0; q < QD_GB + 2 * RR; ++q) x[q] = (POS ? qd_max(0.0, -(x[q] - dcrit)) : x[q]) * sc;
 #pragma unroll
             for (int k = 0; k < QD_GB; ++k) {
                 double tmp = x[k + RR] * w[0];
@@ -476,6 +482,10 @@
     double w[RR + 1];
 #pragma unroll
     for (int k = 0; k <= RR; ++k) w[k] = W.w[k];
+    double xa[QD_GB + 2 * RR], xb[QD_GB + 2 * RR], cv[QD_GB];
+#pragma unroll
+    for (int q = 0; q < QD_GB + 2 * RR; ++q) { xa[q] = 0.0; xb[q] = 0.0; }
+    qd_gauss_rows_load<RR>(G, inA, mode_wrap, i0, nvalid, jbase, xa);
     double scA, al;
     if (P.fold) {
         __shared__ double s_sc[2];
@@ -486,15 +496,22 @@
         scA = scA_p ? *scA_p : scA_k;
         al = (P.op == 1) ? sc[1] : 0.0;
     }
-    double a[QD_GB], b[QD_GB];
-#pragma unroll
-    for (int k = 0; k < QD_GB; ++k) { a[k] = 0.0; b[k] = 0.0; }
-    qd_gauss_rows_pass<RR, false>(G, inA, scA, w, mode_wrap, i0, nvalid, jbase, sm, a);
-    if (P.fold) { if (al != 0.0) qd_gauss_rows_pass<RR, true>(G, inB, scB_k, w, mode_wrap, i0, nvalid, jbase, sm, b, P.dcrit); }
-    else if (P.op != 1 || al != 0.0) qd_gauss_rows_pass<RR, false>(G, inB, scB_k, w, mode_wrap, i0, nvalid, jbase, sm, b);
+    const bool readB = P.fold ? (al != 0.0) : (P.op != 1 || al != 0.0);
+    if (readB) qd_gauss_rows_load<RR>(G, inB, mode_wrap, i0, nvalid, jbase, xb);
     const int c0 = threadIdx.x;
     const int j = jbase + c0 - RR;
-    if (c0 < RR || c0 >= QD_BLOCK - RR || j >= G.nlon) return;
+    const bool own = !(c0 < RR || c0 >= QD_BLOCK - RR || j >= G.nlon);
+#pragma unroll
+    for (int k = 0; k < QD_GB; ++k) cv[k] = (P.op != 1 && own && k < nvalid) ? out0[(size_t)qd_lrow(G, i0 + k) * G.nlon + j] : 0.0;
+    double a[QD_GB], b[QD_GB];
+#pragma unroll
+    for (int k = 0; k < QD_GB; ++k) { a[k] = 0.0; b[k] = 0.0; }
+    qd_gauss_rows_pass<RR, false>(G, xa, scA, w, jbase, sm, a);
+    if (readB) {
+        if (P.fold) qd_gauss_rows_pass<RR, true>(G, xb, scB_k, w, jbase, sm, b, P.dcrit);
+        else qd_gauss_rows_pass<RR, false>(G, xb, scB_k, w, jbase, sm, b);
+    }
+    if (!own) return;
 #pragma unroll
     for (int k = 0; k < QD_GB; ++k) {
         if (k >= nvalid) break;
@@ -506,7 +523,7 @@
         } else {
             const double cp = qd_clip(a[k], 0.0, 1.0), sr = qd_clip(b[k], 0.0, 1.0);
             outA[o] = cp; outB[o] = sr;
-            const double c0v = out0[o];
+            const double c0v = cv[k];
             const double tendency = sr * P.tend;
             double c = (P.w_mem * c0v + P.w_p * cp + P.w_src * qd_clip(c0v + tendency, 0.0, 1.0));
             if (P.c_floor > 0.0) c = qd_max(c, qd_clip(P.c_floor * cp, 0.0, 1.0));
```

Result: no change. 5.112 planet-days/s (-0.2%).
